# the-professor510/RSMCRT

Hardware: AMD Instinct MI355X
Metric: photon packets/sec (128^3 jmean grid, path-length deposition) (higher is better)
Workload: dtype f64

## Files before the change

### include/smcrt.h

```cpp
#ifndef SMCRT_H
#define SMCRT_H

#include <stddef.h>
#include <stdint.h>

#ifdef __cplusplus
extern "C" {
#endif

#define SMCRT_ABI_VERSION 5

typedef enum smcrt_status {
  SMCRT_OK = 0,
  SMCRT_ERR_INVALID_ARG = -1,
  SMCRT_ERR_HIP = -2,
  SMCRT_ERR_RCCL = -3,
  SMCRT_ERR_DEVICE_FAULT = -4,
  SMCRT_ERR_NO_DEVICE = -5,
  SMCRT_ERR_OOM = -6,
  SMCRT_ERR_UNSUPPORTED = -7
} smcrt_status;

typedef enum smcrt_sdf_kind {
  SMCRT_SDF_SPHERE = 1,
// ... 124 lines not shown

enum {
  SMCRT_FLAG_PATHLENGTH = 1u << 0,
  SMCRT_FLAG_SURVIVAL_BIAS = 1u << 1,
  SMCRT_FLAG_RENDER_SOURCE = 1u << 2,
  SMCRT_FLAG_TEST_KERNEL = 1u << 3,
  SMCRT_FLAG_END_EARLY = 1u << 4,
  SMCRT_FLAG_RECORD_PHOTONS = 1u << 5,
  SMCRT_FLAG_ASYNC_FOLD = 1u << 6,
  SMCRT_FLAG_OVERLAP = 1u << 7
};

typedef struct smcrt_run_config {
  uint64_t n_photons;
  uint64_t first_photon;
  uint64_t seed;
  uint32_t flags;
  int32_t reserved;
} smcrt_run_config;

enum {
  SMCRT_CTR_PHOTONS = 0,
  SMCRT_CTR_EMIT_RETRIES,
  SMCRT_CTR_SCATTERS,
  SMCRT_CTR_ABSORBED,
  SMCRT_CTR_SDF_EVALS,
  SMCRT_CTR_DEPOSITS,
  SMCRT_CTR_GRID_UPDATES,
  SMCRT_CTR_TAUINT,
  SMCRT_CTR_FRESNEL,
  SMCRT_CTR_REFLECTIONS,
  SMCRT_CTR_BOUNCE_ABORTS,
  SMCRT_CTR_FAULTS,
  SMCRT_CTR_RNG_DRAWS,
  SMCRT_CTR_DETECTOR_HITS,
  SMCRT_CTR_ESCAPED,
  SMCRT_CTR_WAVE_ITERS,
  SMCRT_NCOUNTERS = 16
};

typedef struct smcrt_photon_record {
  double pos[3];
  double dir[3];
  double weight;
  int32_t cell[3];
  int32_t layer;
  uint32_t nscatt;
  uint32_t bounces;
  uint32_t draws;
  uint32_t status;
} smcrt_photon_record;

typedef struct smcrt_tallies {
  float* jmean;
  float* absorb;
  float* emission;
  double* jmean_f64;
  double* absorb_f64;
  double* emission_f64;
  double* det_bins;
  double* nscatt;
  double* moments;
  uint64_t* counters;
  smcrt_photon_record* records;
} smcrt_tallies;

typedef struct smcrt_scene smcrt_scene;

int smcrt_abi_version(void);
int smcrt_device_count(int32_t* count);
const char* smcrt_last_error(void);

int smcrt_scene_create(const smcrt_sdf_node* nodes, int32_t n_nodes,
                       const int32_t* top, int32_t n_top,
                       const smcrt_grid* grid,
                       const smcrt_detector* dets, int32_t n_dets,
                       int32_t device, smcrt_scene** out);
void smcrt_scene_destroy(smcrt_scene* scene);

int smcrt_scene_info(const smcrt_scene* scene, smcrt_grid* grid, int32_t* n_top, int32_t* n_dets);

int smcrt_scene_det_bins(const smcrt_scene* scene, int64_t* n_doubles);

int smcrt_scene_set_optprops(smcrt_scene* scene, int32_t top_index,
                             double mus, double mua, double hgg, double n);

typedef struct smcrt_spectral {
  int64_t n_mus, n_mua, n_hgg, n_n, n_flux;
  const double* mus;
  const double* mua;
  const double* hgg;
  const double* n;
  const double* flux;
} smcrt_spectral;

typedef enum smcrt_spectral_mode {
  SMCRT_SPECTRAL_INIT = 0,
  SMCRT_SPECTRAL_UPDATE = 1,
  SMCRT_SPECTRAL_INIT_AS_WRITTEN = 2
} smcrt_spectral_mode;

typedef struct smcrt_optprops {
  double mus, mua, hgg, g2, n, kappa, albedo;
  double wavelength;
  int32_t node_flags;
  int32_t reserved;
} smcrt_optprops;

int smcrt_spectral_sample(const smcrt_spectral* sp, int32_t mode, uint64_t seed, uint64_t* draw,
                          smcrt_optprops* out);

int smcrt_scene_set_spectral(smcrt_scene* scene, int32_t top_index, const smcrt_spectral* sp, int32_t mode,
                             uint64_t seed, uint64_t* draw, smcrt_optprops* out);

int smcrt_run(smcrt_scene* scene, const smcrt_source* src, const smcrt_run_config* cfg,
              smcrt_tallies* io);

typedef struct smcrt_device_tallies {
  double* jmean;
  double* absorb;
  double* emission;
  double* det_bins;
  double* nscatt;
  double* moments;
  uint64_t* counters;
  smcrt_photon_record* records;
} smcrt_device_tallies;

int smcrt_run_device(smcrt_scene* scene, const smcrt_source* src, const smcrt_run_config* cfg,
                     smcrt_device_tallies* dev, void* stream);

int smcrt_run_origins(smcrt_scene* scene, const smcrt_source* src, const double* origins, int64_t n_origins,
                      const smcrt_run_config* cfg, double* det_totals, smcrt_tallies* io);

int smcrt_scene_classify(smcrt_scene* scene, const double* points, int64_t n, int32_t* layer, double* kappa);

int smcrt_scene_fence(smcrt_scene* scene, void* stream);

int smcrt_scene_check(smcrt_scene* scene);

typedef struct smcrt_kernel_times {
  double transport_ms;
  double deposit_ms;
  int64_t launches;
  int64_t lean_launches;
  int64_t far_steps;
  double fold_cu_ms;
  int64_t lean_hazards;
} smcrt_kernel_times;

int smcrt_scene_set_timing(smcrt_scene* scene, int32_t enable);
int smcrt_scene_kernel_times(smcrt_scene* scene, smcrt_kernel_times* out);

int smcrt_normalise_fluence(float* grid, const smcrt_grid* g, uint64_t nphotons);

typedef enum smcrt_symmetry {
  SMCRT_SYM_NONE = 0,
  SMCRT_SYM_PRISM = 1,
  SMCRT_SYM_FLIPPED = 2,
  SMCRT_SYM_UNIFORM_SLAB = 3,
  SMCRT_SYM_NONE_ROTATIONAL = 4,
  SMCRT_SYM_ROTATIONAL_360 = 5
} smcrt_symmetry;

typedef struct smcrt_escape_config {
  int32_t symmetry;
  int32_t n[3];
  double max[3];
  double pos[3];
  double dir[3];
  double rotation;
} smcrt_escape_config;

int smcrt_escape_sym_dims(const smcrt_escape_config* cfg, int32_t dims[3]);

int smcrt_escape_cells(const smcrt_escape_config* cfg, int64_t* n_cells, int32_t* cells, double* positions);

int smcrt_escape_map(const smcrt_escape_config* cfg, const smcrt_grid* grid, int32_t n_dets, const float* escape_sym,
                     float* escape);

int smcrt_escape_run(smcrt_scene* scene, const smcrt_source* src, const smcrt_escape_config* cfg,
                     const smcrt_run_config* run, float* escape_sym, float* escape, smcrt_tallies* io);

enum {
  SMCRT_INVERSE_FIND_MUS = 1u << 0,
  SMCRT_INVERSE_FIND_MUA = 1u << 1,
  SMCRT_INVERSE_FIND_G = 1u << 2,
  SMCRT_INVERSE_FIND_N = 1u << 3,
  SMCRT_INVERSE_APPLY_TRIAL = 1u << 4
};

typedef struct smcrt_inverse_config {
  int32_t layer;
  int32_t flags;
  int32_t max_steps;
  int32_t reserved;
  double max_step_size, grad_step_size, accuracy;
  uint64_t seed;
} smcrt_inverse_config;

int smcrt_scene_get_optprops(const smcrt_scene* scene, int32_t top_index, int32_t* layer, double* mus, double* mua,
                             double* hgg, double* n);

int smcrt_inverse_run(smcrt_scene* scene, const smcrt_source* src, const smcrt_inverse_config* cfg,
                      const smcrt_run_config* run, const double* targets, double* steps, smcrt_tallies* io);

enum {
  SMCRT_PACK_JMEAN = 1u << 0,
  SMCRT_PACK_ABSORB = 1u << 1,
  SMCRT_PACK_EMISSION = 1u << 2,
  SMCRT_PACK_DET_BINS = 1u << 3
};
typedef struct smcrt_pack_layout {
  int64_t n_voxels;
  int64_t n_det_bins;
  uint32_t fields;
  int32_t reserved;
} smcrt_pack_layout;

int smcrt_pack_size(const smcrt_pack_layout* layout, int64_t* n_doubles);
int smcrt_pack_host(const smcrt_pack_layout* layout, const smcrt_tallies* t, double* buf);
int smcrt_unpack_host(const smcrt_pack_layout* layout, const double* buf, smcrt_tallies* t);

#define SMCRT_UNIQUE_ID_BYTES 128
typedef struct smcrt_comm smcrt_comm;
int smcrt_comm_unique_id(uint8_t* id );
int smcrt_comm_init_rank(const uint8_t* id, int32_t n_ranks, int32_t rank, int32_t device, smcrt_comm** out);
void smcrt_comm_destroy(smcrt_comm* comm);
int smcrt_comm_info(const smcrt_comm* comm, int32_t* n_ranks, int32_t* rank, int32_t* device);
int smcrt_reduce_device_tallies(smcrt_scene* scene, smcrt_comm* comm, smcrt_device_tallies* dev, int32_t root,
                                void* stream);

typedef struct smcrt_multi smcrt_multi;
int smcrt_multi_create(const smcrt_sdf_node* nodes, int32_t n_nodes, const int32_t* top, int32_t n_top,
                       const smcrt_grid* grid, const smcrt_detector* dets, int32_t n_dets,
                       const int32_t* devices, int32_t n_devices, smcrt_multi** out);
int smcrt_multi_info(const smcrt_multi* multi, int32_t* n_devices);
smcrt_scene* smcrt_multi_scene(smcrt_multi* multi, int32_t i);
int smcrt_multi_run(smcrt_multi* multi, const smcrt_source* src, const smcrt_run_config* cfg, smcrt_tallies* io);
int smcrt_multi_accumulate(smcrt_multi* multi, const smcrt_source* src, const smcrt_run_config* cfg);
int smcrt_multi_collect(smcrt_multi* multi, smcrt_tallies* io);
int smcrt_multi_device_photons(const smcrt_multi* multi, uint64_t* photons);
void smcrt_multi_destroy(smcrt_multi* multi);


int smcrt_write_data_f32(const char* filename, const float* array, int32_t nx, int32_t ny, int32_t nz,
                         const char* metadata, const char* dect_id, int32_t overwrite,
                         char* written_path, int32_t path_cap);
int smcrt_write_data_f64(const char* filename, const double* array, int32_t nx, int32_t ny, int32_t nz,
                         const char* metadata, const char* dect_id, int32_t overwrite,
                         char* written_path, int32_t path_cap);

int smcrt_write_detector(const char* filename, const smcrt_detector* d, const double* data,
                         const char* id, int64_t nphotons);

int smcrt_write_checkpoint(const char* filename, const char* toml_filename, int64_t photons_run,
                           const float* jmean, const smcrt_grid* g, int32_t overwrite,
                           char* written_path, int32_t path_cap);

typedef struct smcrt_job smcrt_job;

typedef struct smcrt_job_desc {
  int64_t n_photons;
  int64_t seed;
  int32_t flags;
  int32_t n_nodes, n_top, n_dets;
  int32_t overwrite;
  smcrt_grid grid;
  smcrt_source source;
  char experiment[64];
  char source_name[32];
} smcrt_job_desc;

int smcrt_job_load(const char* toml_path, smcrt_job** out);
enum { SMCRT_JOB_DEFAULT = 0, SMCRT_JOB_ESCAPE = 1, SMCRT_JOB_INVERSE = 2 };
int smcrt_job_load_mode(const char* toml_path, int32_t mode, smcrt_job** out);
void smcrt_job_destroy(smcrt_job* job);
int smcrt_job_info(const smcrt_job* job, smcrt_job_desc* desc);
int smcrt_job_scene(const smcrt_job* job, smcrt_sdf_node* nodes, int32_t* top, smcrt_detector* dets);
int smcrt_job_metadata(const smcrt_job* job, char* buf, int32_t cap);
#define SMCRT_ALL_DEVICES (-1)
int smcrt_job_run(smcrt_job* job, int32_t device, const char* outdir, double* nscatt);
int smcrt_job_run_devices(smcrt_job* job, const int32_t* devices, int32_t n_devices, const char* outdir,
                          double* nscatt);

int smcrt_job_escape_config(const smcrt_job* job, smcrt_escape_config* out);
int smcrt_job_inverse_config(const smcrt_job* job, smcrt_inverse_config* out);
int smcrt_job_targets(const smcrt_job* job, double* targets);
int smcrt_job_run_escape(smcrt_job* job, int32_t device, const char* outdir);
int smcrt_job_run_inverse(smcrt_job* job, int32_t device, int32_t apply_trial, double* steps);

#ifdef __cplusplus
}
#endif
#endif
```

### rsmcrt_amd/abi.py

```python
import ctypes as C

SMCRT_ABI_VERSION = 5

OK = 0
ERR_INVALID_ARG = -1
ERR_HIP = -2
ERR_RCCL = -3
ERR_DEVICE_FAULT = -4
ERR_NO_DEVICE = -5
ERR_OOM = -6
ERR_UNSUPPORTED = -7

STATUS_NAMES = {
    OK: "OK", ERR_INVALID_ARG: "INVALID_ARG", ERR_HIP: "HIP_ERROR", ERR_RCCL: "RCCL_ERROR",
    ERR_DEVICE_FAULT: "DEVICE_FAULT", ERR_NO_DEVICE: "NO_DEVICE", ERR_OOM: "OUT_OF_MEMORY",
    ERR_UNSUPPORTED: "UNSUPPORTED",
}

SDF_SPHERE, SDF_BOX, SDF_TORUS, SDF_CYLINDER, SDF_TRIPRISM = 1, 2, 3, 4, 5
SDF_SEGMENT, SDF_CAPSULE, SDF_CONE, SDF_EGG, SDF_PLANE, SDF_MODEL = 6, 7, 8, 9, 10, 11
SDF_REVOLUTION, SDF_EXTRUDE, SDF_ONION, SDF_TWIST, SDF_BEND, SDF_ELONGATE, SDF_DISPLACEMENT = 12, 13, 14, 15, 16, 17, 18
DISP_SINE = 1

OP_UNION, OP_SMOOTH_UNION, OP_SUBTRACTION, OP_INTERSECTION = 0, 1, 2, 3
# ... 37 lines not shown
        ("first_child", C.c_int32), ("n_children", C.c_int32), ("flags", C.c_int32), ("reserved", C.c_int32 * 2),
        ("transform", C.c_double * 16), ("param", C.c_double * 12), ("k", C.c_double),
        ("mus", C.c_double), ("mua", C.c_double), ("hgg", C.c_double), ("n", C.c_double),
    ]


NODE_ALBEDO_UNGUARDED = 1

SPECTRAL_INIT = 0
SPECTRAL_UPDATE = 1
SPECTRAL_INIT_AS_WRITTEN = 2


class Spectral(C.Structure):
    _fields_ = [("n_mus", C.c_int64), ("n_mua", C.c_int64), ("n_hgg", C.c_int64), ("n_n", C.c_int64),
                ("n_flux", C.c_int64), ("mus", C.POINTER(C.c_double)), ("mua", C.POINTER(C.c_double)),
                ("hgg", C.POINTER(C.c_double)), ("n", C.POINTER(C.c_double)), ("flux", C.POINTER(C.c_double))]


class OptProps(C.Structure):
    _fields_ = [("mus", C.c_double), ("mua", C.c_double), ("hgg", C.c_double), ("g2", C.c_double),
                ("n", C.c_double), ("kappa", C.c_double), ("albedo", C.c_double), ("wavelength", C.c_double),
                ("node_flags", C.c_int32), ("reserved", C.c_int32)]


class Grid(C.Structure):
    _fields_ = [("nx", C.c_int32), ("ny", C.c_int32), ("nz", C.c_int32), ("reserved", C.c_int32),
                ("xmax", C.c_double), ("ymax", C.c_double), ("zmax", C.c_double)]


class Spectrum(C.Structure):
    _fields_ = [("kind", C.c_int32), ("reserved", C.c_int32), ("wavelength", C.c_double),
                ("n", C.c_int64), ("array", C.POINTER(C.c_double)),
                ("width", C.c_int32), ("height", C.c_int32), ("image", C.POINTER(C.c_double)),
                ("cell_width", C.c_double), ("cell_height", C.c_double)]


class Source(C.Structure):
    _fields_ = [("kind", C.c_int32), ("reserved", C.c_int32),
                ("pos", C.c_double * 3), ("dir", C.c_double * 3),
                ("p1", C.c_double * 3), ("p2", C.c_double * 3), ("p3", C.c_double * 3),
                ("beam", C.c_int32), ("reserved2", C.c_int32),
                ("radius", C.c_double), ("beam_size", C.c_double), ("focal_length", C.c_double),
                ("rlo", C.c_double), ("rhi", C.c_double), ("sigma", C.c_double),
                ("rotation", C.c_double * 3), ("spectrum", C.POINTER(Spectrum))]


class Detector(C.Structure):
    _fields_ = [
        ("kind", C.c_int32), ("nbins", C.c_int32), ("layer", C.c_int32), ("reserved", C.c_int32),
        ("pos", C.c_double * 3), ("dir", C.c_double * 3), ("e1", C.c_double * 3), ("e2", C.c_double * 3),
        ("radius", C.c_double), ("r1", C.c_double), ("r2", C.c_double),
        ("width", C.c_double), ("height", C.c_double),
        ("bin_wid", C.c_double), ("bin_wid_y", C.c_double), ("fibre", C.c_double * 11),
    ]


class RunConfig(C.Structure):
    _fields_ = [("n_photons", C.c_uint64), ("first_photon", C.c_uint64), ("seed", C.c_uint64),
                ("flags", C.c_uint32), ("reserved", C.c_int32)]


class PhotonRecord(C.Structure):
    _fields_ = [("pos", C.c_double * 3), ("dir", C.c_double * 3), ("weight", C.c_double),
                ("cell", C.c_int32 * 3), ("layer", C.c_int32), ("nscatt", C.c_uint32),
                ("bounces", C.c_uint32), ("draws", C.c_uint32), ("status", C.c_uint32)]


class Tallies(C.Structure):
    _fields_ = [
        ("jmean", C.POINTER(C.c_float)), ("absorb", C.POINTER(C.c_float)),
        ("emission", C.POINTER(C.c_float)),
        ("jmean_f64", C.POINTER(C.c_double)), ("absorb_f64", C.POINTER(C.c_double)),
        ("emission_f64", C.POINTER(C.c_double)),
        ("det_bins", C.POINTER(C.c_double)), ("nscatt", C.POINTER(C.c_double)),
        ("moments", C.POINTER(C.c_double)), ("counters", C.POINTER(C.c_uint64)),
        ("records", C.POINTER(PhotonRecord)),
    ]


class DeviceTallies(C.Structure):
    _fields_ = [
        ("jmean", C.c_void_p), ("absorb", C.c_void_p), ("emission", C.c_void_p),
        ("det_bins", C.c_void_p), ("nscatt", C.c_void_p), ("moments", C.c_void_p),
        ("counters", C.c_void_p), ("records", C.c_void_p),
    ]


def record_dtype():
    import numpy as np
    return np.dtype([("pos", "<f8", 3), ("dir", "<f8", 3), ("weight", "<f8"), ("cell", "<i4", 3),
                     ("layer", "<i4"), ("nscatt", "<u4"), ("bounces", "<u4"), ("draws", "<u4"),
                     ("status", "<u4")])


SYM_NONE, SYM_PRISM, SYM_FLIPPED, SYM_UNIFORM_SLAB, SYM_NONE_ROTATIONAL, SYM_ROTATIONAL_360 = 0, 1, 2, 3, 4, 5
SYMMETRY_KINDS = {"none": SYM_NONE, "prism": SYM_PRISM, "flipped": SYM_FLIPPED, "uniformSlab": SYM_UNIFORM_SLAB,
                  "noneRotational": SYM_NONE_ROTATIONAL, "360rotational": SYM_ROTATIONAL_360}


class EscapeConfig(C.Structure):
    _fields_ = [("symmetry", C.c_int32), ("n", C.c_int32 * 3), ("max", C.c_double * 3), ("pos", C.c_double * 3),
                ("dir", C.c_double * 3), ("rotation", C.c_double)]


INVERSE_FIND_MUS, INVERSE_FIND_MUA, INVERSE_FIND_G, INVERSE_FIND_N, INVERSE_APPLY_TRIAL = 1, 2, 4, 8, 16


class InverseConfig(C.Structure):
    _fields_ = [("layer", C.c_int32), ("flags", C.c_int32), ("max_steps", C.c_int32), ("reserved", C.c_int32),
                ("max_step_size", C.c_double), ("grad_step_size", C.c_double), ("accuracy", C.c_double),
                ("seed", C.c_uint64)]


JOB_DEFAULT, JOB_ESCAPE, JOB_INVERSE = 0, 1, 2


class JobDesc(C.Structure):
    _fields_ = [("n_photons", C.c_int64), ("seed", C.c_int64), ("flags", C.c_int32), ("n_nodes", C.c_int32),
                ("n_top", C.c_int32), ("n_dets", C.c_int32), ("overwrite", C.c_int32), ("grid", Grid),
                ("source", Source), ("experiment", C.c_char * 64), ("source_name", C.c_char * 32)]


PACK_JMEAN, PACK_ABSORB, PACK_EMISSION, PACK_DET_BINS = 1, 2, 4, 8
UNIQUE_ID_BYTES = 128
ALL_DEVICES = -1


class PackLayout(C.Structure):
    _fields_ = [("n_voxels", C.c_int64), ("n_det_bins", C.c_int64), ("fields", C.c_uint32), ("reserved", C.c_int32)]


class KernelTimes(C.Structure):
    _fields_ = [("transport_ms", C.c_double), ("deposit_ms", C.c_double), ("launches", C.c_int64),
                ("lean_launches", C.c_int64), ("far_steps", C.c_int64), ("fold_cu_ms", C.c_double),
                ("lean_hazards", C.c_int64)]


EXPORTED_SYMBOLS = [
    "smcrt_abi_version", "smcrt_device_count", "smcrt_last_error", "smcrt_scene_create",
    "smcrt_scene_destroy", "smcrt_scene_det_bins", "smcrt_scene_set_optprops", "smcrt_run",
    "smcrt_run_device", "smcrt_normalise_fluence", "smcrt_scene_set_timing", "smcrt_scene_kernel_times",
    "smcrt_write_data_f32", "smcrt_write_data_f64", "smcrt_write_detector", "smcrt_write_checkpoint",
    "smcrt_job_load", "smcrt_job_destroy", "smcrt_job_info", "smcrt_job_scene", "smcrt_job_metadata", "smcrt_job_run",
    "smcrt_scene_info", "smcrt_run_origins", "smcrt_scene_classify", "smcrt_escape_sym_dims", "smcrt_escape_cells",
    "smcrt_escape_map", "smcrt_escape_run", "smcrt_scene_get_optprops", "smcrt_inverse_run", "smcrt_job_load_mode",
    "smcrt_job_escape_config", "smcrt_job_inverse_config", "smcrt_job_targets", "smcrt_job_run_escape",
    "smcrt_job_run_inverse", "smcrt_scene_fence",
    "smcrt_pack_size", "smcrt_pack_host", "smcrt_unpack_host", "smcrt_comm_unique_id", "smcrt_comm_init_rank",
    "smcrt_comm_info", "smcrt_comm_destroy", "smcrt_reduce_device_tallies", "smcrt_multi_create", "smcrt_multi_info",
    "smcrt_multi_scene", "smcrt_multi_run", "smcrt_multi_accumulate", "smcrt_multi_collect",
    "smcrt_multi_device_photons", "smcrt_multi_destroy", "smcrt_job_run_devices",
    "smcrt_spectral_sample", "smcrt_scene_set_spectral", "smcrt_scene_check",
]
```

### rsmcrt_amd/csrc/kernel_ptrs.h

```cpp
#pragma once
#include <stddef.h>

namespace smcrt {

size_t kinst_ws_shared_bytes(int slots);
int kinst_ws_threads();
int kinst_ws_photon_lanes();
size_t kinst_ws_scratch_bytes(size_t lanes);

#define SMCRT_KINST_DECL(F, G)                                                               \
  const void* kinst_transport_##F##_##G(int xsrc, int coop);                                 \
  const void* kinst_ws_##F##_##G(int xf, int slots);                                         \
  const void* kinst_wsp_##F##_##G(int slots);                                                \
  void kinst_diag_##F##_##G(unsigned long long* d72, unsigned long long* t9, unsigned long long* c6); \
  void kinst_diagp_##F##_##G(unsigned long long* d72, unsigned long long* t9, unsigned long long* c6);
SMCRT_KINST_DECL(0, 0)
SMCRT_KINST_DECL(0, 1)
SMCRT_KINST_DECL(0, 2)
SMCRT_KINST_DECL(1, 0)
SMCRT_KINST_DECL(1, 1)
SMCRT_KINST_DECL(1, 2)
#undef SMCRT_KINST_DECL

inline const void* transport_kernel_ptr(bool lds_faces, int gm, bool xsrc, bool coop) {
  if (xsrc && coop) lds_faces = false;
  const int x = xsrc ? 1 : 0, c = coop ? 1 : 0;
  switch ((lds_faces ? 3 : 0) + gm) {
    case 0: return kinst_transport_0_0(x, c);
    case 1: return kinst_transport_0_1(x, c);
    case 2: return kinst_transport_0_2(x, c);
    case 3: return kinst_transport_1_0(x, c);
    case 4: return kinst_transport_1_1(x, c);
    default: return kinst_transport_1_2(x, c);
  }
}
inline const void* ws_kernel_ptr(bool lds_faces, int gm, bool xf, int slots) {
  const int x = xf ? 1 : 0;
  switch ((lds_faces ? 3 : 0) + gm) {
    case 0: return kinst_ws_0_0(x, slots);
    case 1: return kinst_ws_0_1(x, slots);
    case 2: return kinst_ws_0_2(x, slots);
    case 3: return kinst_ws_1_0(x, slots);
    case 4: return kinst_ws_1_1(x, slots);
    default: return kinst_ws_1_2(x, slots);
  }
}
inline void kinst_diag_gather(unsigned long long* d72, unsigned long long* t9, unsigned long long* c6) {
  for (int i = 0; i < 72; ++i) d72[i] = 0;
  for (int i = 0; i < 9; ++i) t9[i] = 0;
  for (int i = 0; i < 6; ++i) c6[i] = 0;
  kinst_diag_0_0(d72, t9, c6); kinst_diag_0_1(d72, t9, c6); kinst_diag_0_2(d72, t9, c6);
  kinst_diag_1_0(d72, t9, c6); kinst_diag_1_1(d72, t9, c6); kinst_diag_1_2(d72, t9, c6);
  kinst_diagp_0_0(d72, t9, c6); kinst_diagp_0_1(d72, t9, c6); kinst_diagp_0_2(d72, t9, c6);
  kinst_diagp_1_0(d72, t9, c6); kinst_diagp_1_1(d72, t9, c6); kinst_diagp_1_2(d72, t9, c6);
}

}
```

### rsmcrt_amd/csrc/kinst.hip

```cpp
#include "kernels.h"
#include "kernel_ptrs.h"

#if !defined(KI_F) || !defined(KI_G) || !defined(KI_P)
#error "kinst.hip is compiled with -DKI_F=<0|1> -DKI_G=<0|1|2> -DKI_P=<0|1> (rsmcrt_amd/build.py)"
#endif
#define KI_NAME3(a, f, g) a##_##f##_##g
#define KI_NAME2(a, f, g) KI_NAME3(a, f, g)
#define KI_NAME(a) KI_NAME2(a, KI_F, KI_G)

namespace smcrt {

#if KI_P == 1
const void* KI_NAME(kinst_wsp)(int slots) {
  return slots == 3 ? (const void*)ws_kernel<KI_F != 0, KI_G, false, 3> : (const void*)ws_kernel<KI_F != 0, KI_G, false, 2>;
}
#define KI_DIAG_NAME KI_NAME(kinst_diagp)
#else
const void* KI_NAME(kinst_transport)(int xsrc, int coop) {
  constexpr bool F = KI_F != 0;
  if (xsrc && coop) {
    if constexpr (!F) return (const void*)transport_kernel<false, KI_G, true, true>;
    return nullptr;
  }
  if (xsrc) return (const void*)transport_kernel<F, KI_G, true, false>;
  if (coop) return (const void*)transport_kernel<F, KI_G, false, true>;
  return (const void*)transport_kernel<F, KI_G, false, false>;
}

#if KI_F == 0 && KI_G == 0
size_t kinst_ws_shared_bytes(int slots) { return slots == 3 ? sizeof(WsSharedT<3>) : sizeof(WsSharedT<2>); }
int kinst_ws_threads() { return WS_THREADS; }
int kinst_ws_photon_lanes() { return (int)WS_NPL; }
size_t kinst_ws_scratch_bytes(size_t lanes) { return ws_scratch_bytes(lanes); }
#endif

const void* KI_NAME(kinst_ws)(int xf, int slots) {
  if (xf) return slots == 3 ? (const void*)ws_kernel<KI_F != 0, KI_G, true, 3> : (const void*)ws_kernel<KI_F != 0, KI_G, true, 2>;
  return KI_NAME(kinst_wsp)(slots);
}
#define KI_DIAG_NAME KI_NAME(kinst_diag)
#endif


void KI_DIAG_NAME(unsigned long long* d72, unsigned long long* t9, unsigned long long* c6) {
#ifdef SMCRT_DIAG
  unsigned long long h[72] = {0}, z[72] = {0};
  if (hipDeviceSynchronize() != hipSuccess) return;
  if (hipMemcpyFromSymbol(h, HIP_SYMBOL(g_diag), sizeof(h)) == hipSuccess)
    for (int i = 0; i < 72; ++i) d72[i] += (i >= 68 && i <= 69) ? 0 : h[i];
  for (int i = 68; i <= 69; ++i) d72[i] = h[i] > d72[i] ? h[i] : d72[i];
  (void)hipMemcpyToSymbol(HIP_SYMBOL(g_diag), z, sizeof(z));
  if (hipMemcpyFromSymbol(h, HIP_SYMBOL(g_diag_t), sizeof(unsigned long long) * 9) == hipSuccess)
    for (int i = 0; i < 9; ++i) t9[i] += h[i];
  (void)hipMemcpyToSymbol(HIP_SYMBOL(g_diag_t), z, sizeof(unsigned long long) * 9);
  if (hipMemcpyFromSymbol(h, HIP_SYMBOL(g_cull_diag), sizeof(unsigned long long) * 6) == hipSuccess)
    for (int i = 0; i < 6; ++i) c6[i] += h[i];
  (void)hipMemcpyToSymbol(HIP_SYMBOL(g_cull_diag), z, sizeof(unsigned long long) * 6);
#else
  (void)d72; (void)t9; (void)c6;
#endif
}

}
```

### rsmcrt_amd/csrc/sceneplan.cpp

```cpp
#include "sceneplan.h"

#include <algorithm>
#include <cmath>
#include <cstdlib>
#include <cstring>
#include <functional>
#include <string>

#include "hosterr.h"

namespace smcrt {
namespace {

int fail(int code, const std::string& msg) { return set_error(code, msg); }
bool is(const char* v, const char* s) { return v && std::strcmp(v, s) == 0; }

}

Knobs read_knobs() {
  Knobs k;
  auto num = [](const char* v, double d) { return v ? std::atof(v) : d; };
  if (const char* cm = std::getenv("SMCRT_COOP_MIN_TOPS")) k.coop_min_tops = std::max(1, std::atoi(cm));
  if (const char* cl = std::getenv("SMCRT_COOP_LANES")) k.coop_lanes = std::max(1, std::min(64, std::atoi(cl)));
  k.coop_tab = !is(std::getenv("SMCRT_COOP_TAB"), "0");
  k.cull = !is(std::getenv("SMCRT_CULL"), "0");
  k.cull_grid.cells_per_top = num(std::getenv("SMCRT_CULL_CPT"), 512.0);
  k.cull_grid.max_cells = num(std::getenv("SMCRT_CULL_MAX_CELLS"), 1 << 18);
  k.cull_grid.max_list = (int32_t)num(std::getenv("SMCRT_CULL_MAX_LIST"), 64);
  k.cull_grid.k_nearest = (int32_t)num(std::getenv("SMCRT_CULL_K"), 8);
  k.cull_grid.u_frac = num(std::getenv("SMCRT_CULL_UFRAC"), 1.0);
  k.cull_log = std::getenv("SMCRT_CULL_LOG") != nullptr;
  k.far_march = !is(std::getenv("SMCRT_FAR_MARCH"), "0");
  const char* dm = std::getenv("SMCRT_DEPOSIT");
  k.deposit_atomic = is(dm, "atomic");
  k.deposit_sorted = is(dm, "sorted");
  if (const char* pc = std::getenv("SMCRT_POOL_CAP"))
    k.pool_cap_chunks = std::max<uint64_t>(1, std::strtoull(pc, nullptr, 10) / CHUNK_RECORDS);
  const char* fp = std::getenv("SMCRT_FOLD_PRIO");
  k.fold_prio = !(fp && fp[0] == '0');
  k.fused_hist = !is(std::getenv("SMCRT_FUSED_HIST"), "0");
  const char* wsl = std::getenv("SMCRT_WS_SLOTS");
  k.ws_two_slots = wsl && wsl[0] == '2';
  const char* le = std::getenv("SMCRT_LEAN");
  k.lean_mode = le ? (is(le, "0") ? 0 : 1) : -1;
  const char* lm = std::getenv("SMCRT_DEBUG_LEAN_MARGIN");
  k.lean_debug = is(lm, "all") ? 2u : (is(lm, "0") ? 1u : 0u);
  k.verbose = std::getenv("SMCRT_VERBOSE") != nullptr;
  return k;
}

LaunchKnobs read_launch_knobs() {
  LaunchKnobs k;
#ifdef SMCRT_DIAG
  const char* dd = std::getenv("SMCRT_DIAG_DONE");
  k.diag_done = dd && dd[0] == '1';
#endif
  if (const char* wm = std::getenv("SMCRT_WATCHDOG_MS")) k.watchdog_ms = std::strtod(wm, nullptr);
  if (const char* cd = std::getenv("SMCRT_DEBUG_CLAIM_DELAY")) k.claim_delay = (uint32_t)std::strtoul(cd, nullptr, 10);
  const char* de = std::getenv("SMCRT_DEBUG_DROP_EVENT");
  k.drop_event = de && de[0] == '1';
  return k;
}

PoolKnobs read_pool_knobs() {
  PoolKnobs k;
  if (const char* ns = std::getenv("SMCRT_SLOTS")) k.slots = std::max(2, std::min(MAX_SLOTS, std::atoi(ns)));
  if (const char* dg = std::getenv("SMCRT_DEEP_SLOT_GIB")) {
    k.deep_set = true;
    k.deep_bytes = (uint64_t)std::strtoull(dg, nullptr, 10) << 30;
  }
  return k;
}

bool pool_log_knob() {
  static const bool on = std::getenv("SMCRT_POOL_LOG") != nullptr;
  return on;
}

TopProps make_props(const smcrt_sdf_node& nd) {
  TopProps p;
  p.kappa = nd.mus + nd.mua;
  if (nd.flags & SMCRT_NODE_ALBEDO_UNGUARDED) p.albedo = nd.mus / p.kappa;
  else p.albedo = (nd.mua < 1e-9) ? 1.0 : nd.mus / p.kappa;
  p.hgg = nd.hgg;
  p.n = nd.n;
  return p;
}

namespace {

int validate(const smcrt_sdf_node* nodes, int32_t n_nodes, const int32_t* top, int32_t n_top, const smcrt_grid* grid,
             const smcrt_detector* dets, int32_t n_dets) {
  if (!nodes || n_nodes < 1 || !top || n_top < 1 || !grid || n_dets < 0 || (n_dets > 0 && !dets))
    return fail(SMCRT_ERR_INVALID_ARG, "bad scene arguments");
  if (grid->nx < 1 || grid->ny < 1 || grid->nz < 1 || !(grid->xmax > 0) || !(grid->ymax > 0) ||
      !(grid->zmax > 0))
    return fail(SMCRT_ERR_INVALID_ARG, "grid dimensions must be positive");
  if ((uint64_t)grid->nx * (uint64_t)grid->ny * (uint64_t)grid->nz >= (1ull << 32))
    return fail(SMCRT_ERR_UNSUPPORTED, "grids of 2^32 or more voxels are not supported");
  for (int32_t i = 0; i < n_nodes; ++i) {
    const smcrt_sdf_node& nd = nodes[i];
    if (nd.kind < SMCRT_SDF_SPHERE || nd.kind > SMCRT_SDF_DISPLACEMENT)
      return fail(SMCRT_ERR_INVALID_ARG, "node " + std::to_string(i) + ": unknown SDF kind");
    if (nd.kind == SMCRT_SDF_MODEL) {
      if (nd.n_children < 1 || nd.first_child < 0 || nd.first_child + nd.n_children > n_nodes)
        return fail(SMCRT_ERR_INVALID_ARG, "model node " + std::to_string(i) + ": bad child range");
      if (nd.op < SMCRT_OP_UNION || nd.op > SMCRT_OP_INTERSECTION)
        return fail(SMCRT_ERR_INVALID_ARG, "model node " + std::to_string(i) + ": bad CSG op");
    } else if (composite_kind(nd.kind)) {
      if (nd.n_children != 1 || nd.first_child < 0 || nd.first_child >= n_nodes)
        return fail(SMCRT_ERR_INVALID_ARG, "modifier node " + std::to_string(i) + ": needs exactly one child");
      if (nd.kind == SMCRT_SDF_DISPLACEMENT && nd.param[0] != (double)SMCRT_DISP_SINE)
        return fail(SMCRT_ERR_INVALID_ARG, "displacement node " + std::to_string(i) + ": unknown function");
    }
  }
  std::function<int(int32_t, int)> depth_ok = [&](int32_t idx, int lvl) -> int {
    const smcrt_sdf_node& nd = nodes[idx];
    if (!composite_kind(nd.kind)) return 1;
    if (lvl >= PROG_MAX_DEPTH) return 0;
    for (int32_t c = 0; c < nd.n_children; ++c)
      if (!depth_ok(nd.first_child + c, lvl + 1)) return 0;
    return 1;
  };
  for (int32_t i = 0; i < n_top; ++i)
    if (top[i] >= 0 && top[i] < n_nodes && !depth_ok(top[i], 0))
      return fail(SMCRT_ERR_UNSUPPORTED, "top " + std::to_string(i) + ": models/modifiers nested more than " +
                                             std::to_string(PROG_MAX_DEPTH) + " levels deep are not supported");
  for (int32_t i = 0; i < n_top; ++i)
    if (top[i] < 0 || top[i] >= n_nodes) return fail(SMCRT_ERR_INVALID_ARG, "top index out of range");
  for (int32_t i = 0; i < n_dets; ++i) {
    if (dets[i].kind < SMCRT_DET_CIRCLE || dets[i].kind > SMCRT_DET_FIBRE || dets[i].nbins < 1)
      return fail(SMCRT_ERR_INVALID_ARG, "bad detector " + std::to_string(i));
  }
  return SMCRT_OK;
}

bool translate_only(const smcrt_sdf_node& nd) {
  const double* t = nd.transform;
  return t[0] == 1.0 && t[1] == 0.0 && t[2] == 0.0 && t[4] == 0.0 && t[5] == 1.0 && t[6] == 0.0 &&
         t[8] == 0.0 && t[9] == 0.0 && t[10] == 1.0;
}

void flatten(const smcrt_sdf_node* nodes, const int32_t* top, int32_t n_top, ScenePlan& p) {
  std::vector<ProgOp>& prog = p.prog;
  p.top_first.assign((size_t)n_top + 1, 0);
  for (int32_t i = 0; i < n_top; ++i) {
    const smcrt_sdf_node& nd = nodes[top[i]];
    p.top_first[i] = (int32_t)prog.size();
    if (!composite_kind(nd.kind)) {
      prog.push_back(ProgOp{top[i], PROG_TOP, i + 1, 0, 0.0, translate_only(nd), 0});
    } else if (nd.kind != SMCRT_SDF_MODEL) {
      prog.push_back(ProgOp{top[i], PROG_TOP | PROG_SUB, i + 1, 0, 0.0, 0, 0});
    } else {
      for (int32_t c = 0; c < nd.n_children; ++c) {
        const int32_t ci = nd.first_child + c;
        const bool sub = composite_kind(nodes[ci].kind);
        prog.push_back(ProgOp{ci, (c == 0 ? PROG_CHILD_FIRST : PROG_CHILD) | (sub ? PROG_SUB : 0),
                              c == nd.n_children - 1 ? i + 1 : 0, nd.op, nd.k, sub ? 0 : translate_only(nodes[ci]), 0});
      }
    }
  }
  p.n_prog = (int)prog.size();
  p.top_first[n_top] = p.n_prog;
  for (int32_t i = 0; i <= n_top; ++i)
    prog.push_back(ProgOp{p.top_first[i], PROG_TOP, 0, 0, 0.0, 0, 0});
  for (const ProgOp& op : prog) p.nested = p.nested || (op.action & PROG_SUB) != 0;
}

void plan_far_march(const smcrt_sdf_node* nodes, const int32_t* top, int32_t n_top, const smcrt_grid* grid, bool fm,
                    ScenePlan& p) {
  double ext = grid->xmax + grid->ymax + grid->zmax + 1.0;
  double scale = 0.0;
  std::function<bool(int32_t, int, double&)> far_ok = [&](int32_t idx, int lvl, double& m) -> bool {
    const smcrt_sdf_node& nd = nodes[idx];
    if (nd.kind == SMCRT_SDF_MODEL) {
      const bool op_ok = nd.op == SMCRT_OP_UNION || nd.op == SMCRT_OP_INTERSECTION || nd.op == SMCRT_OP_SUBTRACTION ||
                         (nd.op == SMCRT_OP_SMOOTH_UNION && nd.k > 0.0 && std::isfinite(nd.k));
      if (lvl >= 4 || !op_ok || nd.n_children < 1) return false;
      if (nd.op == SMCRT_OP_SMOOTH_UNION) m = std::max(m, nd.k);
      for (int32_t c = 0; c < nd.n_children; ++c)
        if (!far_ok(nd.first_child + c, lvl + 1, m)) return false;
      return true;
    }
    const int32_t kd = nd.kind;
    if (!translate_only(nd) || !(kd == SMCRT_SDF_SPHERE || kd == SMCRT_SDF_BOX || kd == SMCRT_SDF_TORUS ||
                                 kd == SMCRT_SDF_SEGMENT || kd == SMCRT_SDF_CAPSULE))
      return false;
    double mm = std::fabs(nd.transform[3]) + std::fabs(nd.transform[7]) + std::fabs(nd.transform[11]);
    for (int r = 0; r < 8; ++r) mm += std::fabs(nd.param[r]);
    if (!std::isfinite(mm)) return false;
    m = std::max(m, mm);
    return true;
  };
  for (int32_t i = 0; fm && i < n_top; ++i) {
    double m = 0.0;
    fm = far_ok(top[i], 0, m);
    scale = std::max(scale, m);
  }
  fm = fm && std::isfinite(ext);
  if (fm) {
    p.fm_err = std::ldexp(scale + ext, -44);
    p.fm_step = std::ldexp(scale + ext, -48);
  }
}

}

int plan_scene(const smcrt_sdf_node* nodes, int32_t n_nodes, const int32_t* top, int32_t n_top, const smcrt_grid* grid,
               const smcrt_detector* dets, int32_t n_dets, const Knobs& knobs, const PlanLimits& lim, ScenePlan* out) {
  if (const int st = validate(nodes, n_nodes, top, n_top, grid, dets, n_dets)) return st;
  ScenePlan& p = *out;
  p.n_nodes = n_nodes;
  p.n_top = n_top;
  p.n_dets = n_dets;
  p.grid = *grid;
  p.h_nodes.assign(nodes, nodes + n_nodes);
  p.h_top.assign(top, top + n_top);
  for (int32_t i = 0; i < n_top; ++i) p.h_props.push_back(make_props(nodes[top[i]]));
  p.h_dets.assign(dets, dets + n_dets);
  p.h_det_off.assign((size_t)n_dets + 1, 0);
  for (int32_t i = 0; i < n_dets; ++i) {
    const int64_t nb = dets[i].nbins;
    p.h_det_off[i + 1] = p.h_det_off[i] + (dets[i].kind == SMCRT_DET_CAMERA ? nb * nb : nb);
  }
  p.det_total = p.h_det_off[n_dets];
  for (int32_t i = 0; i < grid->nx + 1; ++i) p.faces.push_back((double)i * 2.0 * grid->xmax / (double)grid->nx);
  for (int32_t i = 0; i < grid->ny + 1; ++i) p.faces.push_back((double)i * 2.0 * grid->ymax / (double)grid->ny);
  for (int32_t i = 0; i < grid->nz + 2; ++i) p.faces.push_back((double)i * 2.0 * grid->zmax / (double)grid->nz);
  flatten(nodes, top, n_top, p);
  p.coop_lanes = n_top >= knobs.coop_min_tops ? std::max(1, std::min(16, n_top / ((n_top + 63) / 64 + 3))) : 0;
  if (knobs.coop_lanes && p.coop_lanes > 0) p.coop_lanes = knobs.coop_lanes;
  {
    bool ok = p.coop_lanes > 0 && n_top <= 64 && knobs.coop_tab;
    for (int32_t i = 0; ok && i < n_top; ++i) ok = !composite_kind(nodes[top[i]].kind);
    if (ok) {
      p.ctab.assign(CTAB_DOUBLES, 0.0);
      for (int32_t i = 0; i < n_top; ++i) {
        const smcrt_sdf_node& nd = nodes[top[i]];
        for (int r = 0; r < 12; ++r) p.ctab[r * 64 + i] = nd.transform[r];
        for (int r = 0; r < 8; ++r) p.ctab[(12 + r) * 64 + i] = nd.param[r];
        p.ctab[20 * 64 + i] = (double)nd.kind + (translate_only(nd) ? 16.0 : 0.0);
      }
    }
  }
  const double maxes[3] = {grid->xmax, grid->ymax, grid->zmax};
  if (p.coop_lanes > 0 && knobs.cull) p.cull = build_cull(nodes, n_nodes, top, n_top, maxes, knobs.cull_grid);
  if (!p.ctab.empty() || p.cull.enabled) plan_far_march(nodes, top, n_top, grid, knobs.far_march, p);
  for (int a = 0; a < 3; ++a) {
    int ex = 0;
    const double m = std::frexp(2.0 * maxes[a], &ex);
    p.inv2[a] = (m == 0.5 && std::isfinite(1.0 / (2.0 * maxes[a]))) ? 1.0 / (2.0 * maxes[a]) : 0.0;
  }
  {
    const bool p2 = p.inv2[0] != 0.0 && p.inv2[1] != 0.0 && p.inv2[2] != 0.0;
    const int32_t ns[3] = {grid->nx, grid->ny, grid->nz};
    bool f2 = p2;
    for (int a = 0; a < 3; ++a) {
      if ((ns[a] & (ns[a] - 1)) != 0) { f2 = false; continue; }
      int e2m = 0, en = 0;
      (void)std::frexp(2.0 * maxes[a], &e2m);
      (void)std::frexp((double)ns[a], &en);
      p.fe[a] = e2m - en;
    }
    p.grid_mode = f2 ? 2 : (p2 ? 1 : 0);
  }
  {
    const uint64_t nv = (uint64_t)grid->nx * grid->ny * grid->nz;
    const uint64_t tiles = (nv + TILE_VOXELS - 1) / TILE_VOXELS;
    p.n_tiles = (tiles <= MAX_TILES && nv < 0xFFFFFFFFull) ? (uint32_t)tiles : 0;
    p.force_atomic = knobs.deposit_atomic;
    p.pool_cap_chunks = knobs.pool_cap_chunks;
    const bool sorted = knobs.deposit_sorted || !knobs.fused_hist;
    p.bucketed = !sorted && p.n_tiles > 0 && p.n_tiles <= MAX_DIRECT_TILES;
    p.hist_tiles = (!p.bucketed && knobs.fused_hist && p.n_tiles > 0 && p.n_tiles <= MAX_FUSED_HIST_TILES) ? p.n_tiles : 0;
  }
  p.face_bytes = p.faces.size() * sizeof(double) + sizeof(TopProps) * (size_t)n_top;
  p.lds_faces = p.face_bytes <= MAX_FACE_BYTES;
  for (int32_t i = 1; i < n_top; ++i) p.fresnel = p.fresnel || p.h_props[i].n != p.h_props[0].n;
  {
    bool ok = p.bucketed && p.coop_lanes == 0 && grid->nx < (1 << 20) - 2 && grid->ny < (1 << 20) - 2 &&
              grid->nz < (1 << 20) - 2;
    p.ws_slots = (!knobs.ws_two_slots && lean_lds(p) + lim.ws_shared3 <= LDS_BYTES) ? 3 : 2;
    ok = ok && lean_lds(p) + (p.ws_slots == 3 ? lim.ws_shared3 : lim.ws_shared2) <= LDS_BYTES;
    p.lean_mode = knobs.lean_mode;
    p.lean_candidate = ok && !p.nested && (p.lean_mode == 1 || (p.lean_mode != 0 && n_dets == 0));
    p.lean_debug = knobs.lean_debug;
  }
  p.fold_prio = knobs.fold_prio;
  p.cull_log = knobs.cull_log;
  p.verbose = knobs.verbose;
  return SMCRT_OK;
}

}
```

### rsmcrt_amd/csrc/sceneplan.h

```cpp
#pragma once
#include <stdint.h>

#include <algorithm>
#include <vector>

#include "../../include/smcrt.h"
#include "transport.h"
#include "cull.h"
#include "deposit.h"

namespace smcrt {

constexpr int MAX_SLOTS = 4;
#ifndef SMCRT_DEEP_SLOT_GIB
#define SMCRT_DEEP_SLOT_GIB 24
#endif
constexpr uint64_t DEEP_SLOT_BYTES = (uint64_t)SMCRT_DEEP_SLOT_GIB << 30;

enum QueueWord : int {
  Q_STREAM0 = 0,
  Q_CALLER = MAX_SLOTS,
  Q_FAR_STEPS,
  Q_FOLD_TICKS,
  Q_LEAN_HAZARDS,
  Q_WATCHDOG,
  Q_COUNT
};
constexpr int N_QUEUES = Q_CALLER + 1;

constexpr size_t LDS_BYTES = 163840;
constexpr size_t MAX_FACE_BYTES = 40960;
constexpr uint32_t MAX_FUSED_HIST_TILES = 512;
constexpr uint64_t MAX_POOL_RECORDS = (1ull << 32) - (1ull << 28);
constexpr double POOL_SLACK = 1.15;
constexpr double DEFAULT_WATCHDOG_MS = 2000.0;

struct Knobs {
  int32_t coop_min_tops = 8;
  int32_t coop_lanes = 0;
  bool coop_tab = true;
  bool cull = true;
  CullKnobs cull_grid;
  bool cull_log = false;
  bool far_march = true;
  bool deposit_atomic = false, deposit_sorted = false;
  uint64_t pool_cap_chunks = 0;
  bool fold_prio = true;
  bool fused_hist = true;
  bool ws_two_slots = false;
  int lean_mode = -1;
  uint32_t lean_debug = 0;
  bool verbose = false;
};
struct LaunchKnobs {
  double watchdog_ms = DEFAULT_WATCHDOG_MS;
  uint32_t claim_delay = 0;
  bool drop_event = false;
  bool diag_done = false;
};
struct PoolKnobs {
  int slots = 0;
  bool deep_set = false;
  uint64_t deep_bytes = 0;
};
Knobs read_knobs();
LaunchKnobs read_launch_knobs();
PoolKnobs read_pool_knobs();
bool pool_log_knob();

struct PlanLimits {
  size_t ws_shared2 = 0, ws_shared3 = 0;
};

struct ScenePlan {
  int n_nodes = 0, n_top = 0, n_dets = 0;
  smcrt_grid grid{};
  int64_t det_total = 0;
  std::vector<smcrt_sdf_node> h_nodes;
  std::vector<int32_t> h_top;
  std::vector<TopProps> h_props;
  std::vector<smcrt_detector> h_dets;
  std::vector<int64_t> h_det_off;
  std::vector<double> faces;
  std::vector<ProgOp> prog;
  std::vector<int32_t> top_first;
  int n_prog = 0;
  bool nested = false;
  int coop_lanes = 0;
  std::vector<double> ctab;
  CullHost cull;
  double fm_err = 0.0, fm_step = 0.0;
  double inv2[3] = {0.0, 0.0, 0.0};
  int grid_mode = 0;
  int32_t fe[3] = {0, 0, 0};
  uint32_t n_tiles = 0;
  bool force_atomic = false;
  uint64_t pool_cap_chunks = 0;
  bool bucketed = false;
  uint32_t hist_tiles = 0;
  size_t face_bytes = 0;
  bool lds_faces = false;
  bool fresnel = false;
  int ws_slots = 3;
  int lean_mode = -1;
  uint32_t lean_debug = 0;
  bool lean_candidate = false;
  bool fold_prio = true, cull_log = false, verbose = false;
};

int plan_scene(const smcrt_sdf_node* nodes, int32_t n_nodes, const int32_t* top, int32_t n_top, const smcrt_grid* grid,
               const smcrt_detector* dets, int32_t n_dets, const Knobs& knobs, const PlanLimits& lim, ScenePlan* out);

TopProps make_props(const smcrt_sdf_node& nd);

inline size_t lean_lds(const ScenePlan& p) {
  return (p.lds_faces ? p.face_bytes : 0) + (size_t)2 * p.n_tiles * sizeof(uint32_t);
}
inline uint32_t dep_words(const ScenePlan& p) { return p.bucketed ? 2 * p.n_tiles : 4 * p.hist_tiles; }
inline size_t transport_lds(const ScenePlan& p, uint32_t dep_words, bool xsrc) {
  const bool ctab = !p.ctab.empty() && p.coop_lanes > 0;
  const bool faces = p.lds_faces && !(xsrc && p.coop_lanes > 0);
  return (faces ? p.face_bytes : 0) + (p.n_dets ? 3 * 256 * sizeof(double) : 0) +
         (size_t)dep_words * sizeof(uint32_t) + (ctab ? CTAB_DOUBLES * sizeof(double) : 0);
}
inline double pool_slack_records(const ScenePlan& p, int blocks) {
  const double waves = (double)blocks * 4.0;
  return p.bucketed ? (waves / 4.0 * 2.0 * p.n_tiles + waves * BUCKET_BATCH) * BUCKET_RECORDS
                    : waves * CHUNK_RECORDS;
}
inline uint64_t pool_records_for(const ScenePlan& p, int blocks, uint64_t n, double rpp) {
  const double want = (double)n * rpp * POOL_SLACK + pool_slack_records(p, blocks);
  return (uint64_t)std::min(want, (double)MAX_POOL_RECORDS);
}
inline int slot_depth(const PoolKnobs& k, bool lean_or_far, uint64_t cap_bytes, uint64_t total_mem) {
  const int want = k.slots ? k.slots : (lean_or_far ? 2 : MAX_SLOTS);
  uint64_t deep = std::max<uint64_t>(DEEP_SLOT_BYTES, (uint64_t)(0.6 * (double)total_mem) / MAX_SLOTS);
  if (k.deep_set) deep = k.deep_bytes;
  return cap_bytes <= deep ? want : 2;
}
inline bool launch_binned(const ScenePlan& p, bool has_jmean, uint32_t flags) {
  return has_jmean && (flags & SMCRT_FLAG_PATHLENGTH) && !(flags & SMCRT_FLAG_SURVIVAL_BIAS) && p.n_tiles > 0 &&
         !p.force_atomic;
}
inline bool launch_lean(bool lean_ok, bool xsrc, uint32_t bucket_tiles, uint32_t flags) {
  return !xsrc && lean_ok && bucket_tiles && (flags & SMCRT_FLAG_PATHLENGTH) && !(flags & SMCRT_FLAG_SURVIVAL_BIAS);
}
inline void lean_margins(uint32_t lean_debug, const smcrt_grid& g, double lo[3], double hi[3]) {
  const double eps = 1e-8, mf = (lean_debug & 3u) ? 0.0 : 2.0 * eps;
  const double mx = mf * (double)(g.nx + 2), my = mf * (double)(g.ny + 2), mz = mf * (double)(g.nz + 2);
  lo[0] = mx; lo[1] = my; lo[2] = mz;
  hi[0] = 2.0 * g.xmax - mx; hi[1] = 2.0 * g.ymax - my; hi[2] = 2.0 * g.zmax - mz;
}

}
```

### rsmcrt_amd/csrc/smcrt.hip

```cpp
#include <hip/hip_runtime.h>

#include <algorithm>
#include <cmath>
#include <cstdio>
#include <cstring>
#include <memory>
#include <mutex>
#include <string>
#include <vector>

#define SMCRT_FOLD_KERNELS
#include "../../include/smcrt.h"
#include "scene_internal.h"
#include "transport.h"
#include "deposit.h"
#include "devmem.h"
#include "hosterr.h"
#include "sceneplan.h"

using namespace smcrt;

#include "kernel_ptrs.h"


// ... 125 lines not shown
    float a = 0.f, b = 0.f;
    if ((err = hipEventElapsedTime(&a, e[0], e[1])) != hipSuccess) return err;
    if ((err = hipEventElapsedTime(&b, e[2], e[3])) != hipSuccess) return err;
    s->t_transport += a; s->t_deposit += b; s->t_launches += 1;
  }
  s->tev_used = 0;
  return hipSuccess;
}

static const void* transport_fn(const smcrt_scene* s, bool xsrc) {
  return transport_kernel_ptr(s->lds_faces, s->grid_mode, xsrc, s->coop_lanes > 0);
}

static uint32_t* watchdog_word(smcrt_scene* s) { return (uint32_t*)(s->d_queue + Q_WATCHDOG); }
static const char* watchdog_site(uint32_t site) {
  switch (site) {
    case WDOG_PHOTON_WAVE: return "ws_kernel photon wave (every live lane waited for an event, a segment or a slot)";
    case WDOG_RING: return "ws_kernel ring producer (the token word's previous lap was never consumed)";
    case WDOG_EVENT_QUEUE: return "ws_kernel event-queue producer (the entry's previous lap was never consumed)";
    case WDOG_BUCKET: return "bucket wait (deposit.h: the pending claim never rebased the tile word)";
    default: return "unknown site";
  }
}
static int take_watchdog(smcrt_scene* s) {
  uint32_t w = 0;
  HIPCHK(hipMemcpy(&w, watchdog_word(s), sizeof w, hipMemcpyDeviceToHost));
  if (!w) return SMCRT_OK;
  HIPCHK(hipMemset(watchdog_word(s), 0, sizeof w));
  return fail(SMCRT_ERR_DEVICE_FAULT, std::string("watchdog: a wait exceeded SMCRT_WATCHDOG_MS at ") +
                                          watchdog_site(w & 0xFFu) + " in block " + std::to_string((w >> 8) - 1u) +
                                          "; the run's tallies are incomplete");
}

extern "C" {

int smcrt_abi_version(void) { return SMCRT_ABI_VERSION; }

const char* smcrt_last_error(void) { return g_last_error.c_str(); }

int smcrt_device_count(int32_t* count) {
  if (!count) return fail(SMCRT_ERR_INVALID_ARG, "count is NULL");
  int n = 0;
  hipError_t e = hipGetDeviceCount(&n);
  if (e == hipErrorNoDevice) n = 0;
  else if (e != hipSuccess) return fail(SMCRT_ERR_HIP, hipGetErrorString(e));
  *count = n;
  return SMCRT_OK;
}

void smcrt_scene_destroy(smcrt_scene* s) {
  if (!s) return;
  (void)hipSetDevice(s->device);
  if (s->stream) (void)hipStreamSynchronize(s->stream);
  if (s->fstream) (void)hipStreamSynchronize(s->fstream);
  for (int i = 0; i < MAX_SLOTS; ++i)
    if (s->lstream[i]) (void)hipStreamSynchronize(s->lstream[i]);
  delete s;
}

static int upload_plan(smcrt_scene* s) {
  int st;
  if ((st = upload(s->d_nodes, s->h_nodes.data(), s->h_nodes.size(), "scene upload")) ||
      (st = upload(s->d_prog, s->prog.data(), s->prog.size(), "scene upload")) ||
      (st = upload(s->d_props, s->h_props.data(), s->h_props.size(), "scene upload")) ||
      (st = upload(s->d_faces, s->faces.data(), s->faces.size(), "scene upload")) ||
      (st = upload(s->d_dets, s->h_dets.data(), s->h_dets.size(), "scene upload")) ||
      (st = upload(s->d_det_off, s->h_det_off.data(), s->h_det_off.size(), "scene upload")) ||
      (!s->ctab.empty() && (st = upload(s->d_ctab, s->ctab.data(), s->ctab.size(), "scene upload"))) ||
      (st = dalloc(s->d_queue, Q_COUNT)) || (st = dalloc(s->d_cold, COLD_SLOTS)) ||
      (st = dalloc(s->d_counters, SMCRT_NCOUNTERS)) || (st = dalloc(s->d_small, (size_t)s->det_total + 1 + 24)))
    return st;
  hipError_t e = hipMemset(s->d_queue, 0, Q_COUNT * sizeof(unsigned long long));
  if (e == hipSuccess) e = hipStreamCreateWithFlags(s->stream.out(), hipStreamNonBlocking);
  for (int i = 0; i < MAX_SLOTS && e == hipSuccess; ++i) {
    e = hipStreamCreateWithFlags(s->lstream[i].out(), hipStreamNonBlocking);
    if (e == hipSuccess) e = hipEventCreateWithFlags(s->lev[i].out(), hipEventDisableTiming);
  }
  if (e == hipSuccess) e = hipEventCreateWithFlags(s->ev_in.out(), hipEventDisableTiming);
  if (e != hipSuccess) return fail(SMCRT_ERR_HIP, std::string("scene upload: ") + hipGetErrorString(e));
  return SMCRT_OK;
}

static int upload_cull(smcrt_scene* s) {
  const CullHost& cull = s->cull;
  std::vector<ProgOp> pa;
  for (int32_t t : cull.always)
    for (int32_t ip = s->top_first[t]; ip < s->top_first[t + 1]; ++ip) pa.push_back(s->prog[ip]);
  auto al = [](size_t b) { return (b + 15) & ~(size_t)15; };
  const size_t b_pa = al(pa.size() * sizeof(ProgOp)), b_off = al(cull.off.size() * 4),
               b_list = al(std::max<size_t>(1, cull.list.size()) * 4), b_lb = al(cull.lb.size() * 8),
               b_elb = al(std::max<size_t>(1, cull.elb.size()) * 4);
  std::vector<unsigned char> blob(b_pa + b_off + b_list + b_lb + b_elb, 0);
  std::memcpy(blob.data(), pa.data(), pa.size() * sizeof(ProgOp));
  std::memcpy(blob.data() + b_pa, cull.off.data(), cull.off.size() * 4);
  std::memcpy(blob.data() + b_pa + b_off, cull.list.data(), cull.list.size() * 4);
  std::memcpy(blob.data() + b_pa + b_off + b_list, cull.lb.data(), cull.lb.size() * 8);
  std::memcpy(blob.data() + b_pa + b_off + b_list + b_lb, cull.elb.data(), cull.elb.size() * 4);
  int st;
  if ((st = upload(s->d_cull_data, blob.data(), blob.size(), "cull upload"))) return st;
  const unsigned char* base = s->d_cull_data;
  CullGrid G;
  for (int a = 0; a < 3; ++a) { G.lo[a] = cull.lo[a]; G.n[a] = cull.n[a]; }
  G.cell = cull.cell;
  G.inv_cell = 1.0 / cull.cell;
  G.n_prog_always = (int32_t)pa.size();
  G.prog_always = base;
  G.off = (const uint32_t*)(base + b_pa);
  G.list = (const uint32_t*)(base + b_pa + b_off);
  G.lb = (const double*)(base + b_pa + b_off + b_list);
  G.elb = (const float*)(base + b_pa + b_off + b_list + b_lb);
  if ((st = upload(s->d_cull, &G, 1, "cull upload"))) return st;
  if (s->cull_log)
    std::fprintf(stderr, "[cull] %d tops, %zu always, %d x %d x %d cells of %.4g, %.1f tops per cell\n",
                 s->n_top, cull.always.size(), cull.n[0], cull.n[1], cull.n[2], cull.cell, cull.mean_list);
  s->cull.off = {}; s->cull.list = {}; s->cull.elb = {}; s->cull.lb = {};
  return SMCRT_OK;
}

static int create_fold_state(smcrt_scene* s) {
  int st;
  if ((st = dalloc(s->d_tile_count, s->n_tiles)) || (st = dalloc(s->d_tile_start, s->n_tiles))) return st;
  for (int i = 0; i < MAX_SLOTS; ++i)
    if ((st = dalloc(s->d_dep_ctl[i], 8)) || (st = dalloc(s->d_bin_counts[i], (size_t)s->n_tiles * BIN_BLOCKS))) return st;
  s->scatter_lds = scatter_lds_bytes(s->n_tiles);
  if (hipFuncSetAttribute((const void*)bin_scatter, hipFuncAttributeMaxDynamicSharedMemorySize,
                          (int)s->scatter_lds) != hipSuccess)
    return fail(SMCRT_ERR_HIP, "bin_scatter LDS attribute");
  int prio_least = 0, prio_greatest = 0;
  const bool fold_prio = s->fold_prio &&
                         hipDeviceGetStreamPriorityRange(&prio_least, &prio_greatest) == hipSuccess &&
                         prio_greatest != prio_least;
  bool ok = s->h_ctl.alloc(8 * MAX_SLOTS) == hipSuccess &&
            hipEventCreateWithFlags(s->ev_t.out(), hipEventDisableTiming) == hipSuccess &&
            (fold_prio ? hipStreamCreateWithPriority(s->fstream.out(), hipStreamNonBlocking, prio_greatest)
                       : hipStreamCreateWithFlags(s->fstream.out(), hipStreamNonBlocking)) == hipSuccess;
  for (int i = 0; ok && i < MAX_SLOTS; ++i)
    ok = hipEventCreateWithFlags(s->ctl_ev[i].out(), hipEventDisableTiming) == hipSuccess &&
         hipEventCreateWithFlags(s->ev_f[i].out(), hipEventDisableTiming) == hipSuccess;
  if (!ok) return fail(SMCRT_ERR_HIP, "pinned/event/stream allocation failed");
  std::memset(s->h_ctl, 0, 8 * MAX_SLOTS * sizeof(uint32_t));
  return SMCRT_OK;
}

static void size_grids(smcrt_scene* s) {
  int per_cu = 0, cus = 0;
  if (hipDeviceGetAttribute(&cus, hipDeviceAttributeMultiprocessorCount, s->device) != hipSuccess || cus < 1) cus = 256;
  s->n_cus = cus;
  int khz = 0;
  if (hipDeviceGetAttribute(&khz, hipDeviceAttributeWallClockRate, s->device) == hipSuccess && khz > 0) s->wall_khz = khz;
  s->lean_ok = s->lean_candidate;
  const bool xf = s->fresnel || s->n_dets > 0;
  if (s->lean_ok) {
    hipError_t oe = hipOccupancyMaxActiveBlocksPerMultiprocessor(
        &per_cu, ws_kernel_ptr(s->lds_faces, s->grid_mode, xf, s->ws_slots), kinst_ws_threads(), lean_lds(*s));
    if (oe != hipSuccess || per_cu < 1) per_cu = 1;
    s->grid_blocks_ws = cus * per_cu;
    if (xf) {
      s->lscratch_stride = (kinst_ws_scratch_bytes((size_t)s->grid_blocks_ws * kinst_ws_photon_lanes()) + 255) & ~(size_t)255;
      if (s->d_lscratch.alloc(s->lscratch_stride * N_QUEUES) != hipSuccess) {
        (void)hipGetLastError();
        s->lean_ok = false;
      }
    }
  }
  if (s->verbose)
    std::fprintf(stderr, "[smcrt] scene: lean %d (ws slots %d, blocks/CU %d, static LDS %zu + dynamic %zu B), transport grid %d\n",
                 (int)s->lean_ok, s->ws_slots, s->grid_blocks_ws / std::max(1, cus), kinst_ws_shared_bytes(s->ws_slots), lean_lds(*s),
                 s->grid_blocks);
  for (int x = 0; x < 2; ++x) {
    hipError_t oe = hipOccupancyMaxActiveBlocksPerMultiprocessor(&per_cu, transport_fn(s, x == 1), 256,
                                                                 transport_lds(*s, dep_words(*s), x == 1));
    if (oe != hipSuccess || per_cu < 1) per_cu = 1;
    (x ? s->grid_blocks_x : s->grid_blocks) = cus * per_cu;
  }
}

int smcrt_scene_create(const smcrt_sdf_node* nodes, int32_t n_nodes, const int32_t* top, int32_t n_top,
                       const smcrt_grid* grid, const smcrt_detector* dets, int32_t n_dets, int32_t device,
                       smcrt_scene** out) {
  g_last_error.clear();
  if (!out) return fail(SMCRT_ERR_INVALID_ARG, "out is NULL");
  *out = nullptr;
  const PlanLimits lim{kinst_ws_shared_bytes(2), kinst_ws_shared_bytes(3)};
  ScenePlan plan;
  int st = plan_scene(nodes, n_nodes, top, n_top, grid, dets, n_dets, read_knobs(), lim, &plan);
  if (st) return st;
  int ndev = 0;
  if (hipGetDeviceCount(&ndev) != hipSuccess || ndev == 0) return fail(SMCRT_ERR_NO_DEVICE, "no HIP device");
  if (device < 0 || device >= ndev) return fail(SMCRT_ERR_INVALID_ARG, "device ordinal out of range");
  std::unique_ptr<smcrt_scene, void (*)(smcrt_scene*)> s(new smcrt_scene(), smcrt_scene_destroy);
  static_cast<ScenePlan&>(*s) = std::move(plan);
  s->device = device;
  if (hipSetDevice(device) != hipSuccess) return fail(SMCRT_ERR_HIP, "hipSetDevice failed");
  if ((st = upload_plan(s.get())) || (s->cull.enabled && (st = upload_cull(s.get()))) ||
      (s->n_tiles && (st = create_fold_state(s.get()))))
    return st;
  size_grids(s.get());
  *out = s.release();
  return SMCRT_OK;
}

int smcrt_scene_det_bins(const smcrt_scene* s, int64_t* n) {
  if (!s || !n) return fail(SMCRT_ERR_INVALID_ARG, "NULL argument");
  *n = s->det_total;
  return SMCRT_OK;
}

int smcrt_scene_set_optprops(smcrt_scene* s, int32_t i, double mus, double mua, double hgg, double n) {
  return smcrt::scene_set_node_props(s, i, mus, mua, hgg, n, 0);
}

int smcrt_scene_get_optprops(const smcrt_scene* s, int32_t i, int32_t* layer, double* mus, double* mua, double* hgg,
                             double* n) {
  if (!s || i < 0 || i >= s->n_top) return fail(SMCRT_ERR_INVALID_ARG, "bad scene or index");
  const smcrt_sdf_node& nd = s->h_nodes[s->h_top[i]];
  if (layer) *layer = nd.layer;
  if (mua) *mua = nd.mua;
  if (mus) *mus = s->h_props[i].kappa - nd.mua;
  if (hgg) *hgg = nd.hgg;
  if (n) *n = nd.n;
  return SMCRT_OK;
}

}

int smcrt::scene_node_optprops(const smcrt_scene* s, int32_t i, double out[4]) {
  if (!s || i < 0 || i >= s->n_top) return fail(SMCRT_ERR_INVALID_ARG, "bad scene or index");
  const smcrt_sdf_node& nd = s->h_nodes[s->h_top[i]];
  out[0] = nd.mus; out[1] = nd.mua; out[2] = nd.hgg; out[3] = nd.n;
  return SMCRT_OK;
}

int smcrt::scene_set_node_props(smcrt_scene* s, int32_t i, double mus, double mua, double hgg, double n,
                                int32_t flags) {
  if (!s || i < 0 || i >= s->n_top) return fail(SMCRT_ERR_INVALID_ARG, "bad scene or index");
  std::lock_guard<std::mutex> g(s->mu);
  smcrt_sdf_node& nd = s->h_nodes[s->h_top[i]];
  nd.mus = mus; nd.mua = mua; nd.hgg = hgg; nd.n = n;
  nd.flags = flags;
  s->h_props[i] = make_props(nd);
  HIPCHK(hipSetDevice(s->device));
  HIPCHK(hipMemcpyAsync(s->d_props + i, &s->h_props[i], sizeof(TopProps), hipMemcpyHostToDevice, s->stream));
  HIPCHK(hipStreamSynchronize(s->stream));
  return SMCRT_OK;
}

int smcrt::scene_node_flags(const smcrt_scene* s, int32_t i, int32_t* flags) {
  if (!s || i < 0 || i >= s->n_top) return fail(SMCRT_ERR_INVALID_ARG, "bad scene or index");
  *flags = s->h_nodes[s->h_top[i]].flags;
  return SMCRT_OK;
}

int smcrt::scene_device(const smcrt_scene* s) { return s->device; }
void* smcrt::scene_stream(const smcrt_scene* s) { return (void*)s->stream; }

int smcrt::scene_inflight(smcrt_scene* s) {
  std::lock_guard<std::mutex> g(s->mu);
  int n = 0;
  for (int i = 0; i < MAX_SLOTS; ++i) {
    if (s->lpending[i] && hipEventQuery(s->lev[i]) == hipSuccess) s->lpending[i] = false;
    n += s->lpending[i] ? 1 : 0;
  }
  return n;
}
int smcrt::scene_depth(const smcrt_scene* s) { return s->n_slots; }

int smcrt::scene_det_size(const smcrt_scene* s, int32_t d, int64_t* n) {
  if (!s || d < 0 || d >= s->n_dets) return fail(SMCRT_ERR_INVALID_ARG, "bad scene or detector");
  *n = (d + 1 < s->n_dets ? s->h_det_off[d + 1] : s->det_total) - s->h_det_off[d];
  return SMCRT_OK;
}

extern "C" {

static void refine_rpp(smcrt_scene* s) {
  for (int i = 0; i < s->n_slots; ++i) {
    const int sl = s->last_slot < 0 ? i : (s->last_slot + 1 + i) % s->n_slots;
    if (s->ctl_pending[sl] && hipEventQuery(s->ctl_ev[sl]) == hipSuccess) {
      s->ctl_pending[sl] = false;
      const uint32_t* h = s->h_ctl + 8 * sl;
      if (pool_log_knob())
        std::fprintf(stderr, "[pool] slot %d: %u photons, %u records, %u overflowed, %u of %llu chunks\n", sl, h[4],
                     h[3], h[1], h[0], (unsigned long long)s->pool_chunks);
      if (h[4] > 0) {
        const double rpp = (double)(h[3] + h[1]) / (double)h[4];
        s->rpp_est = std::max(1.0, rpp);
        s->rpp_measured = true;
      }
    }
  }
}

static hipError_t drain_folds(smcrt_scene* s) {
  if (!s->fstream) return hipSuccess;
  const hipError_t e = hipStreamSynchronize(s->fstream);
  for (bool& f : s->f_pending) f = false;
  return e;
}

static int transport_blocks(const smcrt_scene* s) { return std::max(s->grid_blocks, s->grid_blocks_x); }

static bool ensure_pool(smcrt_scene* s, uint64_t records) {
  uint64_t chunks = (records + CHUNK_RECORDS - 1) / CHUNK_RECORDS;
  if (s->pool_cap_chunks) chunks = std::min(chunks, s->pool_cap_chunks);
  if (chunks <= s->pool_chunks) return true;
  chunks = std::min<uint64_t>(chunks + chunks / 4, MAX_POOL_RECORDS / CHUNK_RECORDS);
  if (s->pool_cap_chunks) chunks = std::min(chunks, s->pool_cap_chunks);
  (void)hipDeviceSynchronize();
  (void)drain_folds(s);
  auto release = [&]() {
    s->d_sorted.reset(); s->d_pieces.reset(); s->d_order.reset();
    for (int i = 0; i < MAX_SLOTS; ++i) { s->d_pool[i].reset(); s->d_chunk_fill[i].reset(); s->d_bucket_tile[i].reset(); }
    s->pool_chunks = 0;
  };
  release();
  const uint64_t cap = chunks * CHUNK_RECORDS;
  size_t mfree = 0, mtotal = 0;
  if (hipMemGetInfo(&mfree, &mtotal) != hipSuccess) mtotal = 0;
  s->n_slots = slot_depth(read_pool_knobs(), s->lean_ok || s->fm_err > 0.0, cap * 8, mtotal);
  s->slot = 0;
  s->lturn = 0;
  s->last_slot = -1;
  const uint64_t pieces = std::min<uint64_t>(cap / MIN_PIECE_RECORDS, REDUCE_PIECES + 1) + s->n_tiles + 1;
  const uint64_t buckets = cap / BUCKET_RECORDS;
  bool ok = s->d_pieces.alloc(pieces) == hipSuccess;
  for (int i = 0; ok && i < s->n_slots; ++i) {
    ok = s->d_pool[i].alloc(cap) == hipSuccess;
    if (ok && s->bucketed)
      ok = s->d_chunk_fill[i].alloc(buckets) == hipSuccess && s->d_bucket_tile[i].alloc(buckets) == hipSuccess;
    else if (ok)
      ok = s->d_chunk_fill[i].alloc(chunks) == hipSuccess;
  }
  if (ok && s->bucketed)
    ok = s->d_order.alloc(buckets) == hipSuccess;
  else if (ok)
    ok = s->d_sorted.alloc(cap) == hipSuccess;
  if (!ok) {
    (void)hipGetLastError();
    release();
    return false;
  }
  s->pool_chunks = chunks;
  s->max_pieces = pieces;
  return true;
}


static int next_timing_events(smcrt_scene* s, Event** ev) {
  *ev = nullptr;
  if (!s->timing) return SMCRT_OK;
  if (s->tev_used == MAX_TIMED) HIPCHK(harvest_times(s));
  while (4 * (s->tev_used + 1) > s->tev.size()) {
    Event e;
    HIPCHK(hipEventCreate(e.out()));
    s->tev.push_back(std::move(e));
  }
  *ev = &s->tev[4 * s->tev_used++];
  return SMCRT_OK;
}

static int enqueue_transport(smcrt_scene* s, const KParams& K, KCold Ch, bool xsrc, bool lean, hipStream_t stream,
                             int sl, int qi, Event** ev_out) {
  const bool binned = K.rec_pool != nullptr;
  if (binned && s->f_pending[sl]) HIPCHK(hipStreamWaitEvent(stream, s->ev_f[sl], 0));
  Ch.queue = s->d_queue + qi;
  Ch.lane_scratch = s->d_lscratch ? (double*)(s->d_lscratch + (size_t)qi * s->lscratch_stride) : nullptr;
  HIPCHK(hipMemsetAsync(Ch.queue, 0, sizeof(unsigned long long), stream));
  const KCold* C = s->d_cold + (size_t)qi * COLD_PER_STREAM + (s->cold_seq[qi]++ % COLD_PER_STREAM);
  HIPCHK(hipMemcpyAsync((void*)C, &Ch, sizeof(KCold), hipMemcpyHostToDevice, stream));
  if (binned) {
    HIPCHK(hipMemsetAsync(s->d_dep_ctl[sl], 0, 8 * sizeof(uint32_t), stream));
    if (K.bucket_tiles)
      HIPCHK(hipMemsetAsync(s->d_bin_counts[sl], 0, (size_t)s->n_tiles * sizeof(uint32_t), stream));
    else if (K.hist_tiles)
      HIPCHK(hipMemsetAsync(s->d_bin_counts[sl], 0, (size_t)s->n_tiles * BIN_BLOCKS * sizeof(uint32_t), stream));
  }
  if (const int st = next_timing_events(s, ev_out)) return st;
  Event* ev = *ev_out;
  if (ev) HIPCHK(hipEventRecord(ev[0], stream));
  const uint64_t waves_needed = (Ch.n_photons + 63) / 64;
  const uint64_t blocks_needed = (waves_needed + 3) / 4;
  const uint64_t ws_needed = (Ch.n_photons + kinst_ws_photon_lanes() - 1) / kinst_ws_photon_lanes();
  const int blocks = (int)std::min<uint64_t>(
      (uint64_t)(lean ? s->grid_blocks_ws : (xsrc ? s->grid_blocks_x : s->grid_blocks)),
      std::max<uint64_t>(1, lean ? ws_needed : blocks_needed));
  const smcrt_sdf_node* a_nodes = K.nodes;
  const ProgOp* a_prog = K.prog;
  if (lean) {
    ++s->lean_launches;
    void* args[] = {(void*)&K, (void*)&a_nodes, (void*)&a_prog, (void*)&C};
    HIPCHK(hipLaunchKernel(ws_kernel_ptr(s->lds_faces, s->grid_mode, s->d_lscratch != nullptr, s->ws_slots), dim3(blocks),
                           dim3(kinst_ws_threads()), args, lean_lds(*s), stream));
  } else {
    const smcrt_detector* a_dets = K.dets;
    const int64_t* a_off = K.det_off;
    void* args[] = {(void*)&K, (void*)&a_nodes, (void*)&a_prog, (void*)&a_dets, (void*)&a_off, (void*)&C};
    HIPCHK(hipLaunchKernel(transport_fn(s, xsrc), dim3(blocks), dim3(256), args, transport_lds(*s, dep_words(*s), xsrc), stream));
  }
  HIPCHK(hipGetLastError());
  if (ev) HIPCHK(hipEventRecord(ev[1], stream));
  return SMCRT_OK;
}

static int enqueue_fold(smcrt_scene* s, const KParams& K, double* jmean, hipStream_t stream, int sl, Event* ev) {
  if (!K.rec_pool) {
    if (ev) {
      HIPCHK(hipEventRecord(ev[2], stream));
      HIPCHK(hipEventRecord(ev[3], stream));
    }
    return SMCRT_OK;
  }
  hipStream_t fs = s->fstream;
  HIPCHK(hipEventRecord(s->ev_t, stream));
  HIPCHK(hipStreamWaitEvent(fs, s->ev_t, 0));
  if (ev) HIPCHK(hipEventRecord(ev[2], fs));
  const uint32_t nch = (uint32_t)s->pool_chunks;
  const uint64_t nv = (uint64_t)s->grid.nx * s->grid.ny * s->grid.nz;
  if (K.bucket_tiles) {
    hipLaunchKernelGGL(bk_scan, dim3(1), dim3(1024), 0, fs, s->d_bin_counts[sl], s->n_tiles, s->d_tile_start,
                       s->d_tile_count, s->d_pieces, s->d_dep_ctl[sl]);
    hipLaunchKernelGGL(bk_place, dim3(BIN_BLOCKS), dim3(BIN_THREADS), 0, fs, s->d_bucket_tile[sl], s->d_dep_ctl[sl],
                       K.n_buckets, s->n_tiles, s->d_tile_count, s->d_order);
#ifndef SMCRT_ABL_NO_FOLD
    hipLaunchKernelGGL(bk_reduce, dim3(1024), dim3(RED_THREADS), 0, fs, s->d_pool[sl], s->d_order, s->d_chunk_fill[sl],
                       s->d_pieces, s->d_dep_ctl[sl], nv, jmean, s->d_queue + Q_FOLD_TICKS);
#endif
  } else {
    if (!K.hist_tiles)
      hipLaunchKernelGGL(bin_hist, dim3(BIN_BLOCKS), dim3(BIN_THREADS), 0, fs, s->d_pool[sl], s->d_chunk_fill[sl],
                         s->d_dep_ctl[sl], nch, s->n_tiles, s->d_bin_counts[sl]);
    hipLaunchKernelGGL(bin_rowscan, dim3(s->n_tiles), dim3(BIN_BLOCKS), 0, fs, s->d_bin_counts[sl],
                       s->d_tile_count);
    hipLaunchKernelGGL(bin_scan, dim3(1), dim3(1024), 0, fs, s->d_tile_count, s->n_tiles, s->d_tile_start,
                       s->d_pieces, s->d_dep_ctl[sl]);
    hipLaunchKernelGGL(bin_scatter, dim3(BIN_BLOCKS), dim3(BIN_THREADS), s->scatter_lds, fs, s->d_pool[sl],
                       s->d_chunk_fill[sl], s->d_dep_ctl[sl], nch, s->n_tiles, s->d_tile_start, s->d_bin_counts[sl],
                       s->d_sorted, (uint64_t)s->pool_chunks * CHUNK_RECORDS);
    hipLaunchKernelGGL(bin_reduce, dim3(1024), dim3(1024), 0, fs, s->d_sorted, s->d_pieces, s->d_dep_ctl[sl], nv,
                       jmean);
  }
  HIPCHK(hipGetLastError());
  HIPCHK(hipMemcpyAsync(s->h_ctl + 8 * sl, s->d_dep_ctl[sl], 4 * sizeof(uint32_t), hipMemcpyDeviceToHost, fs));
  HIPCHK(hipMemcpyAsync(s->h_ctl + 8 * sl + 5, s->d_dep_ctl[sl] + 5, 2 * sizeof(uint32_t), hipMemcpyDeviceToHost, fs));
  HIPCHK(hipEventRecord(s->ctl_ev[sl], fs));
  s->ctl_pending[sl] = true;
  if (ev) HIPCHK(hipEventRecord(ev[3], fs));
  HIPCHK(hipEventRecord(s->ev_f[sl], fs));
  s->f_pending[sl] = true;
  s->last_slot = sl;
  return SMCRT_OK;
}

#ifdef SMCRT_DIAG
static int diag_report(hipStream_t stream, bool lean) {
  unsigned long long h[72], ht[9], hc[6];
  HIPCHK(hipStreamSynchronize(stream));
  kinst_diag_gather(h, ht, hc);
  if (lean) {
    const double wi = (double)std::max(1ull, h[20]), pt = (double)std::max(1ull, h[24]);
    std::fprintf(stderr, "[diag-ws] walker iters %llu: idle %.3f, busy lanes/iter %.1f, pending lanes/iter %.1f | "
                 "photon trips %llu: sleep %.3f, idle lanes %.1f, sync-waiting %.2f, slot-blocked %.2f, EVAL lanes "
                 "%.1f, pushes %.2f, P7 runs %.3f (lanes/run %.1f), event-waiting %.2f | producer waits %llu | event "
                 "iters %llu, lanes/iter %.1f\n",
                 h[20], h[21] / wi, h[22] / wi, h[23] / wi, h[24], h[25] / pt, h[30] / pt, h[27] / pt, h[26] / pt,
                 h[31] / pt, h[32] / pt, h[28] / pt, (double)h[29] / (double)std::max(1ull, h[28]), h[36] / pt, h[33],
                 h[34], (double)h[35] / (double)std::max(1ull, h[34]));
    const char* np[8] = {"fetch", "poll", "eval", "p3p4", "handout", "p5p6", "p7", "p8"};
    double tp = 0, tw = 0, te = 0;
    for (int i = 0; i < 8; ++i) tp += (double)h[37 + i];
    for (int i = 0; i < 4; ++i) tw += (double)h[45 + i];
    te = (double)h[49] + (double)h[50];
    std::fprintf(stderr, "[diag-ws-time] photon:");
    for (int i = 0; i < 8; ++i) std::fprintf(stderr, " %s=%.3f", np[i], (double)h[37 + i] / std::max(1.0, tp));
    std::fprintf(stderr, " | walker: claim=%.3f idle=%.3f walk=%.3f finish=%.3f | event: run=%.3f idle=%.3f | "
                 "ticks photon/walker/event %.3g/%.3g/%.3g\n", h[45] / std::max(1.0, tw), h[46] / std::max(1.0, tw),
                 h[47] / std::max(1.0, tw), h[48] / std::max(1.0, tw), h[49] / std::max(1.0, te),
                 h[50] / std::max(1.0, te), tp, tw, te);
  }
  unsigned long long lt = 0;
  for (int i = 0; i < 64; ++i) lt += h[i];
  std::fprintf(stderr, "[diag] waves %llu, longest wave %llu trips %llu ticks\n", h[70], h[68], h[69]);
  std::fprintf(stderr, "[diag] trips %llu dda %llu eval %llu p7 %llu | lane-trips %llu:", h[64], h[65], h[66],
               h[67], lt);
  for (int i = 0; i < 64; ++i)
    if (h[i]) std::fprintf(stderr, " %s%d=%.3f", i >= 32 ? "seg:" : "", i & 31, (double)h[i] / (double)lt);
  std::fprintf(stderr, "\n");

  double tt = 0;
  for (int i = 1; i < 9; ++i) tt += (double)ht[i];
  const char* nm_t[9] = {"", "fetch", "eval", "p3", "p4", "dda", "p5p6", "p7", "p8"};
  const char* nm_l[9] = {"", "fetch", "eval", "p3p4", "push", "walk", "p5p6", "p7", "p8"};
  const char* const* nm = lean ? nm_l : nm_t;
  std::fprintf(stderr, "[diag-time]");
  for (int i = 1; i < 9; ++i) std::fprintf(stderr, " %s=%.3f", nm[i], (double)ht[i] / tt);
  std::fprintf(stderr, "\n");

  if (hc[0] + hc[2])
    std::fprintf(stderr, "[diag-cull] culled lane-EVALs %llu, bound fallbacks %llu (%.4f), capture/outside %llu, "
                 "mean list %.1f, wave-EVALs %llu with a full fallback %.3f\n", hc[0], hc[1],
                 (double)hc[1] / (double)std::max(1ull, hc[0]), hc[2], (double)hc[3] / (double)std::max(1ull, hc[0]),
                 hc[4], (double)hc[5] / (double)std::max(1ull, hc[4]));
  return SMCRT_OK;
}
#endif

static int launch_one(smcrt_scene* s, const KParams& K, const KCold& Ch, bool xsrc, hipStream_t stream, int sl, int qi) {
  const bool lean = launch_lean(s->lean_ok, xsrc, K.bucket_tiles, K.flags);
  Event* ev = nullptr;
  int st = enqueue_transport(s, K, Ch, xsrc, lean, stream, sl, qi, &ev);
  if (!st) st = enqueue_fold(s, K, Ch.jmean, stream, sl, ev);
#ifdef SMCRT_DIAG
  if (!st) st = diag_report(stream, lean);
#endif
  return st;
}

struct OriginRun {
  const double* d_origins;
  double* d_totals;
  uint64_t per_origin, first;
};

static int fill_params(smcrt_scene* s, const smcrt_source* src, const smcrt_run_config* cfg,
                       const smcrt_device_tallies& dt, const SrcPlan& plan, hipStream_t stream, bool diag_done_ok,
                       KParams& K, KCold& Ch) {
  const LaunchKnobs knobs = read_launch_knobs();
  K.nodes = s->d_nodes;
  K.prog = s->d_prog;
  K.n_prog = s->n_prog;
  K.coop_lanes = s->coop_lanes;
  K.cull = s->d_cull;
  K.ctab = s->d_ctab;
  const bool far = s->fm_err > 0.0 && (cfg->flags & SMCRT_FLAG_PATHLENGTH);
  K.fm_err = far ? s->fm_err : 0.0;
  K.fm_step = s->fm_step;
  K.inv2x = s->inv2[0]; K.inv2y = s->inv2[1]; K.inv2z = s->inv2[2];
  K.fex = s->fe[0]; K.fey = s->fe[1]; K.fez = s->fe[2];
  K.props = s->d_props;
  K.xface = s->d_faces;
  K.yface = s->d_faces + (s->grid.nx + 1);
  K.zface = s->d_faces + (s->grid.nx + 1) + (s->grid.ny + 1);
  K.dets = s->d_dets;
  K.det_off = s->d_det_off;
  K.n_top = s->n_top;
  K.n_dets = s->n_dets;
  K.nx = s->grid.nx; K.ny = s->grid.ny; K.nz = s->grid.nz;
  K.xmax = s->grid.xmax; K.ymax = s->grid.ymax; K.zmax = s->grid.zmax;
  K.flags = cfg->flags;
  Ch.src = *src;
  Ch.plan = plan;
  K.key0 = (uint32_t)cfg->seed;
  K.key1 = (uint32_t)(cfg->seed >> 32);
  Ch.jmean = dt.jmean; Ch.absorb = dt.absorb; Ch.emission = dt.emission;
  Ch.chunk_fill = nullptr; Ch.dep_ctl = nullptr; Ch.bin_counts = nullptr;
  Ch.bucket_tile = nullptr; Ch.bucket_fill = nullptr; Ch.tile_nb = nullptr;
  Ch.det_bins = dt.det_bins; Ch.nscatt = dt.nscatt; Ch.moments = dt.moments;
  Ch.counters = (unsigned long long*)dt.counters;
  Ch.queue = nullptr;
  Ch.far_steps = s->d_queue + Q_FAR_STEPS;
  Ch.lean_hazards = s->d_queue + Q_LEAN_HAZARDS;
  Ch.lane_scratch = nullptr;
  Ch.watchdog = watchdog_word(s);
#ifdef SMCRT_DIAG
  Ch.done_time = nullptr;
  Ch.done_base = cfg->first_photon;
  if (knobs.diag_done && diag_done_ok) {
    s->n_done = cfg->n_photons;
    HIPCHK(s->d_done.alloc(s->n_done));
    HIPCHK(hipMemsetAsync(s->d_done, 0, sizeof(unsigned long long) * s->n_done, stream));
    Ch.done_time = s->d_done;
  }
#else
  (void)stream; (void)diag_done_ok;
#endif
  Ch.watchdog_ticks = knobs.watchdog_ms > 0.0 ? (uint64_t)(knobs.watchdog_ms * (double)s->wall_khz) : 0ull;
  K.rec_pool = nullptr; K.n_chunks = 0; K.hist_tiles = 0; K.bucket_tiles = 0; K.n_buckets = 0;
  K.claim_delay = knobs.claim_delay;
  K.lean_debug = s->lean_debug | (knobs.drop_event ? 4u : 0u);
  lean_margins(K.lean_debug, s->grid, K.lean_lo, K.lean_hi);
  return SMCRT_OK;
}

static int launch(smcrt_scene* s, const smcrt_source* src, const smcrt_run_config* cfg,
                  const smcrt_device_tallies& dt, hipStream_t stream, const OriginRun* orun = nullptr) {
  if (src->kind < SMCRT_SRC_POINT || src->kind > SMCRT_SRC_APERTURE) return fail(SMCRT_ERR_INVALID_ARG, "bad source kind");
  if (cfg->n_photons == 0) return SMCRT_OK;
  const bool xsrc = src_needs_plan(src) || orun || s->nested;
  SrcPlan plan;
  std::memset(&plan, 0, sizeof plan);
  if (xsrc) {
    std::vector<double> px, py, pc;
    const char* perr = "";
    const int pst = build_src_plan(src, &s->grid, &plan, px, py, pc, &perr);
    if (pst) return fail(pst, perr);
    std::vector<double> tab;
    tab.reserve(px.size() + py.size() + pc.size());
    tab.insert(tab.end(), px.begin(), px.end());
    tab.insert(tab.end(), py.begin(), py.end());
    tab.insert(tab.end(), pc.begin(), pc.end());
    if (!tab.empty()) {
      if (tab != s->h_spec) {
        HIPCHK(hipStreamSynchronize(stream));
        if (s->stream != stream) HIPCHK(hipStreamSynchronize(s->stream));
        if (tab.size() > s->spec_cap) {
          s->spec_cap = 0;
          HIPCHK(s->d_spec.alloc(tab.size()));
          s->spec_cap = tab.size();
        }
        HIPCHK(hipMemcpy(s->d_spec, tab.data(), tab.size() * sizeof(double), hipMemcpyHostToDevice));
        s->h_spec = tab;
      }
      plan.spec_x = px.empty() ? nullptr : s->d_spec;
      plan.spec_y = py.empty() ? nullptr : s->d_spec + px.size();
      plan.cdf = s->d_spec + px.size() + py.size();
    }
    if (orun) {
      plan.origins = orun->d_origins;
      plan.det_totals = orun->d_totals;
      plan.per_origin = orun->per_origin;
      plan.first = orun->first;
    }
  }
  KParams K;
  KCold Ch;
  if (const int st = fill_params(s, src, cfg, dt, plan, stream, !orun, K, Ch)) return st;
  const bool binned = launch_binned(*s, dt.jmean != nullptr, cfg->flags);
  const bool overlap = (cfg->flags & SMCRT_FLAG_OVERLAP) != 0;
  if (overlap) {
    HIPCHK(hipEventRecord(s->ev_in, stream));
    for (int i = 0; i < MAX_SLOTS; ++i) HIPCHK(hipStreamWaitEvent(s->lstream[i], s->ev_in, 0));
  } else {
    for (int i = 0; i < MAX_SLOTS; ++i)
      if (s->lpending[i]) HIPCHK(hipStreamWaitEvent(stream, s->lev[i], 0));
  }
  for (int i = 0; i < MAX_SLOTS; ++i)
    if (s->lpending[i] && hipEventQuery(s->lev[i]) == hipSuccess) s->lpending[i] = false;
  for (uint64_t done = 0; done < cfg->n_photons;) {
    refine_rpp(s);
    uint64_t n = cfg->n_photons - done;
    K.rec_pool = nullptr; K.n_chunks = 0; K.hist_tiles = 0; K.bucket_tiles = 0; K.n_buckets = 0;
    bool calibrate = false;
    if (binned) {
      if (!s->rpp_measured && n > CALIB_PHOTONS) { n = CALIB_PHOTONS; calibrate = true; }
      const uint64_t want = pool_records_for(*s, transport_blocks(s), n, s->rpp_est);
      if (!ensure_pool(s, want)) (void)ensure_pool(s, want / 4);
      if (s->pool_chunks) {
        const double usable = (double)(s->pool_chunks * CHUNK_RECORDS) - pool_slack_records(*s, transport_blocks(s));
        n = std::min<uint64_t>(n, (uint64_t)std::max(65536.0, usable / (s->rpp_est * POOL_SLACK)));
        K.rec_pool = s->d_pool[s->slot];
        Ch.chunk_fill = s->d_chunk_fill[s->slot];
        Ch.dep_ctl = s->d_dep_ctl[s->slot];
        Ch.bin_counts = s->d_bin_counts[s->slot];
        K.n_chunks = (uint32_t)s->pool_chunks;
        K.hist_tiles = s->hist_tiles;
        if (s->bucketed) {
          Ch.bucket_fill = s->d_chunk_fill[s->slot];
          Ch.bucket_tile = s->d_bucket_tile[s->slot];
          Ch.tile_nb = s->d_bin_counts[s->slot];
          K.bucket_tiles = s->n_tiles;
          K.n_buckets = (uint32_t)(s->pool_chunks * (CHUNK_RECORDS / BUCKET_RECORDS));
        }
      }
    }
    Ch.n_photons = n;
    Ch.first_photon = orun ? done : cfg->first_photon + done;
    Ch.records = dt.records ? dt.records + done : nullptr;
    const int sl = s->slot;
    if (K.rec_pool) {
      if (s->ctl_pending[sl]) { HIPCHK(hipEventSynchronize(s->ctl_ev[sl])); refine_rpp(s); }
      s->h_ctl[8 * sl + 4] = (uint32_t)std::min<uint64_t>(n, 0xFFFFFFFFull);
    }
    int st;
    if (overlap) {
      const int q = s->lturn;
      s->lturn = (s->lturn + 1) % s->n_slots;
      st = launch_one(s, K, Ch, xsrc, s->lstream[q], sl, q);
      if (!st && hipEventRecord(s->lev[q], s->lstream[q]) != hipSuccess) st = fail(SMCRT_ERR_HIP, "event record failed");
      s->lpending[q] = true;
    } else {
      st = launch_one(s, K, Ch, xsrc, stream, sl, Q_CALLER);
    }
    if (st) return st;
    if (K.rec_pool) s->slot = (s->slot + 1) % s->n_slots;
    if (calibrate && K.rec_pool) {
      HIPCHK(hipEventSynchronize(s->ctl_ev[sl]));
      refine_rpp(s);
    }
    done += n;
  }
  if (!(cfg->flags & (SMCRT_FLAG_ASYNC_FOLD | SMCRT_FLAG_OVERLAP)) && s->last_slot >= 0 && s->f_pending[s->last_slot])
    HIPCHK(hipStreamWaitEvent(stream, s->ev_f[s->last_slot], 0));
  return SMCRT_OK;
}

int smcrt_run_device(smcrt_scene* s, const smcrt_source* src, const smcrt_run_config* cfg,
                     smcrt_device_tallies* dev, void* stream) {
  g_last_error.clear();
  if (!s || !src || !cfg || !dev) return fail(SMCRT_ERR_INVALID_ARG, "NULL argument");
  std::lock_guard<std::mutex> g(s->mu);
  HIPCHK(hipSetDevice(s->device));
  return launch(s, src, cfg, *dev, (hipStream_t)stream);
}

}

static int run_sync(smcrt_scene* s, const smcrt_source* src, const smcrt_run_config* cfg_in, smcrt_tallies* io,
                    const OriginRun* orun) {
  smcrt_run_config cfg_local = *cfg_in;
  cfg_local.flags &= ~(uint32_t)(SMCRT_FLAG_ASYNC_FOLD | SMCRT_FLAG_OVERLAP);
  const smcrt_run_config* cfg = &cfg_local;
  const int64_t nv = (int64_t)s->grid.nx * s->grid.ny * s->grid.nz;
  const bool want[3] = {io->jmean || io->jmean_f64, io->absorb || io->absorb_f64, io->emission || io->emission_f64};
  if (!s->d_grids && (want[0] || want[1] || want[2])) {
    int st = dalloc(s->d_grids, (size_t)nv * 3);
    if (st) return st;
  }
  const bool rec = (cfg->flags & SMCRT_FLAG_RECORD_PHOTONS) && io->records;
  if (rec && s->records_cap < cfg->n_photons) {
    s->records_cap = 0;
    int st = dalloc(s->d_records, cfg->n_photons);
    if (st) return st;
    s->records_cap = cfg->n_photons;
  }
  smcrt_device_tallies dt{};
  for (int t = 0; t < 3; ++t) {
    if (!want[t]) continue;
    double* p = s->d_grids + (size_t)t * nv;
    HIPCHK(hipMemsetAsync(p, 0, sizeof(double) * nv, s->stream));
    if (t == 0) dt.jmean = p;
    if (t == 1) dt.absorb = p;
    if (t == 2) dt.emission = p;
// ... 51 lines not shown

int smcrt_run_origins(smcrt_scene* s, const smcrt_source* src, const double* origins, int64_t n_origins,
                      const smcrt_run_config* cfg, double* det_totals, smcrt_tallies* io) {
  g_last_error.clear();
  if (!s || !cfg || !io || (n_origins > 0 && !origins)) return fail(SMCRT_ERR_INVALID_ARG, "NULL argument");
  if (n_origins < 0) return fail(SMCRT_ERR_INVALID_ARG, "n_origins < 0");
  if (cfg->flags & SMCRT_FLAG_RECORD_PHOTONS) return fail(SMCRT_ERR_INVALID_ARG, "photon records are not kept for batched origins");
  if (n_origins > 0xFFFFFFFFll) return fail(SMCRT_ERR_INVALID_ARG, "more than 2^32 origins");
  if (n_origins == 0 || cfg->n_photons == 0) return SMCRT_OK;
  if (cfg->n_photons > UINT64_MAX / (uint64_t)n_origins) return fail(SMCRT_ERR_INVALID_ARG, "photon count overflows");
  std::lock_guard<std::mutex> g(s->mu);
  HIPCHK(hipSetDevice(s->device));
  smcrt_source p;
  if (src) p = *src;
  else std::memset(&p, 0, sizeof p);
  p.kind = SMCRT_SRC_POINT;
  const size_t nt = (size_t)n_origins * (size_t)std::max(s->n_dets, 1);
  DevBuf<double> d_org, d_tot;
  int st = dalloc(d_org, (size_t)n_origins * 3);
  if (!st) st = dalloc(d_tot, nt);
  if (!st) {
    OriginRun orun{d_org, s->n_dets ? d_tot : nullptr, cfg->n_photons, cfg->first_photon};
    smcrt_run_config c = *cfg;
    c.n_photons = cfg->n_photons * (uint64_t)n_origins;
    hipError_t e = hipMemcpy(d_org, origins, sizeof(double) * 3 * (size_t)n_origins, hipMemcpyHostToDevice);
    if (e == hipSuccess) e = hipMemset(d_tot, 0, sizeof(double) * nt);
    if (e != hipSuccess) st = fail(SMCRT_ERR_HIP, std::string("origin upload: ") + hipGetErrorString(e));
    if (!st) st = run_sync(s, &p, &c, io, &orun);
    if (!st && det_totals && s->n_dets) {
      std::vector<double> h(nt);
      e = hipMemcpy(h.data(), d_tot, sizeof(double) * nt, hipMemcpyDeviceToHost);
      if (e != hipSuccess) st = fail(SMCRT_ERR_HIP, std::string("totals: ") + hipGetErrorString(e));
      else for (size_t i = 0; i < nt; ++i) det_totals[i] += h[i];
    }
  }
  return st;
}

#ifdef SMCRT_DIAG
int smcrt_diag_read(unsigned long long* out) {
  HIPCHK(hipDeviceSynchronize());
  unsigned long long hc[6];
  kinst_diag_gather(out, out + 72, hc);
  return SMCRT_OK;
}
int smcrt_diag_done_times(smcrt_scene* s, unsigned long long* out, uint64_t n, int32_t* khz) {
  if (!s || !out || !s->d_done || n > s->n_done) return fail(SMCRT_ERR_INVALID_ARG, "no completion times");
  HIPCHK(hipDeviceSynchronize());
  HIPCHK(hipMemcpy(out, s->d_done, sizeof(unsigned long long) * n, hipMemcpyDeviceToHost));
  if (khz) *khz = s->wall_khz;
  return SMCRT_OK;
}
#endif

int smcrt_scene_info(const smcrt_scene* s, smcrt_grid* grid, int32_t* n_top, int32_t* n_dets) {
  if (!s) return fail(SMCRT_ERR_INVALID_ARG, "scene is NULL");
  if (grid) *grid = s->grid;
  if (n_top) *n_top = s->n_top;
  if (n_dets) *n_dets = s->n_dets;
  return SMCRT_OK;
}

int smcrt_scene_classify(smcrt_scene* s, const double* points, int64_t n, int32_t* layer, double* kappa) {
  g_last_error.clear();
  if (!s || (n > 0 && (!points || !layer))) return fail(SMCRT_ERR_INVALID_ARG, "NULL argument");
  if (n <= 0) return SMCRT_OK;
  std::lock_guard<std::mutex> g(s->mu);
  HIPCHK(hipSetDevice(s->device));
  DevBuf<double> d_pts;
  DevBuf<int32_t> d_lay;
  int st = dalloc(d_pts, (size_t)n * 3);
  if (!st) st = dalloc(d_lay, (size_t)n);
  if (!st) {
    hipError_t e = hipMemcpy(d_pts, points, sizeof(double) * 3 * (size_t)n, hipMemcpyHostToDevice);
    if (e == hipSuccess) {
      const int blocks = (int)std::min<int64_t>((n + 255) / 256, 65535);
      hipLaunchKernelGGL(classify_kernel, dim3(blocks), dim3(256), 0, s->stream, (const smcrt_sdf_node*)s->d_nodes,
                         (const ProgOp*)s->d_prog, (int32_t)s->n_prog, (const double*)d_pts, n, d_lay);
      e = hipGetLastError();
    }
    if (e == hipSuccess) e = hipStreamSynchronize(s->stream);
    if (e == hipSuccess) e = hipMemcpy(layer, d_lay, sizeof(int32_t) * (size_t)n, hipMemcpyDeviceToHost);
    if (e != hipSuccess) st = fail(SMCRT_ERR_HIP, std::string("classify: ") + hipGetErrorString(e));
  }
  if (!st && kappa)
    for (int64_t i = 0; i < n; ++i) kappa[i] = layer[i] > 0 ? s->h_props[layer[i] - 1].kappa : 0.0;
  return st;
}

int smcrt_scene_fence(smcrt_scene* s, void* stream) {
  g_last_error.clear();
  if (!s) return fail(SMCRT_ERR_INVALID_ARG, "scene is NULL");
  std::lock_guard<std::mutex> g(s->mu);
  HIPCHK(hipSetDevice(s->device));
  for (int i = 0; i < MAX_SLOTS; ++i)
    if (s->lpending[i]) HIPCHK(hipStreamWaitEvent((hipStream_t)stream, s->lev[i], 0));
  if (s->last_slot >= 0 && s->f_pending[s->last_slot])
    HIPCHK(hipStreamWaitEvent((hipStream_t)stream, s->ev_f[s->last_slot], 0));
  return SMCRT_OK;
}

int smcrt_scene_check(smcrt_scene* s) {
  g_last_error.clear();
  if (!s) return fail(SMCRT_ERR_INVALID_ARG, "scene is NULL");
  std::lock_guard<std::mutex> g(s->mu);
  HIPCHK(hipSetDevice(s->device));
  for (int i = 0; i < MAX_SLOTS; ++i)
    if (s->lstream[i]) {
      const hipError_t e = hipStreamSynchronize(s->lstream[i]);
      if (e != hipSuccess) return fail(SMCRT_ERR_DEVICE_FAULT, std::string("transport kernel: ") + hipGetErrorString(e));
    }
  for (hipStream_t st : {(hipStream_t)s->stream, (hipStream_t)s->fstream})
    if (st) {
      const hipError_t e = hipStreamSynchronize(st);
      if (e != hipSuccess) return fail(SMCRT_ERR_DEVICE_FAULT, std::string("transport kernel: ") + hipGetErrorString(e));
    }
  return take_watchdog(s);
}

int smcrt_scene_set_timing(smcrt_scene* s, int32_t enable) {
  if (!s) return fail(SMCRT_ERR_INVALID_ARG, "scene is NULL");
  std::lock_guard<std::mutex> g(s->mu);
  s->timing = enable != 0;
  return SMCRT_OK;
}

int smcrt_scene_kernel_times(smcrt_scene* s, smcrt_kernel_times* out) {
  if (!s || !out) return fail(SMCRT_ERR_INVALID_ARG, "NULL argument");
  std::lock_guard<std::mutex> g(s->mu);
  HIPCHK(hipSetDevice(s->device));
  HIPCHK(harvest_times(s));
  out->transport_ms = s->t_transport;
  out->deposit_ms = s->t_deposit;
  out->launches = s->t_launches;
  out->lean_launches = s->lean_launches;
  s->lean_launches = 0;
  unsigned long long far = 0;
  HIPCHK(hipMemcpy(&far, s->d_queue + Q_FAR_STEPS, sizeof(far), hipMemcpyDeviceToHost));
  out->far_steps = (int64_t)(far - s->far_reported);
  s->far_reported = far;
  unsigned long long ticks = 0;
  HIPCHK(hipMemcpy(&ticks, s->d_queue + Q_FOLD_TICKS, sizeof(ticks), hipMemcpyDeviceToHost));
  out->fold_cu_ms = (double)(ticks - s->fold_ticks_reported) / (double)s->wall_khz / (double)s->n_cus;
  s->fold_ticks_reported = ticks;
  unsigned long long hz = 0;
  HIPCHK(hipMemcpy(&hz, s->d_queue + Q_LEAN_HAZARDS, sizeof(hz), hipMemcpyDeviceToHost));
  out->lean_hazards = (int64_t)(hz - s->hazards_reported);
  s->hazards_reported = hz;
  s->t_transport = s->t_deposit = 0.0;
  s->t_launches = 0;
  return SMCRT_OK;
}

int smcrt_normalise_fluence(float* g, const smcrt_grid* grid, uint64_t nphotons) {
  if (!g || !grid || nphotons == 0) return fail(SMCRT_ERR_INVALID_ARG, "bad arguments");
  const double xmax = grid->xmax, ymax = grid->ymax, zmax = grid->zmax;
  const double f = (2.0 * xmax * 2.0 * ymax * 2.0 * zmax) /
                   ((double)nphotons * (2.0 * xmax / grid->nx) * (2.0 * ymax / grid->ny) * (2.0 * zmax / grid->nz));
  const int64_t nv = (int64_t)grid->nx * grid->ny * grid->nz;
  for (int64_t i = 0; i < nv; ++i) g[i] = (float)((double)g[i] * f);
  return SMCRT_OK;
}

}
```

### rsmcrt_amd/csrc/transport.h

```cpp
#pragma once
#include <hip/hip_runtime.h>
#include <stdint.h>

#include "../../include/smcrt.h"
#include "detmath.h"
#include "geometry.h"
#include "srcplan.h"
#include "cull.h"

namespace smcrt {

constexpr int64_t MAX_EMIT_TRIES = 100000;
constexpr int64_t MAX_HOP_ITERS = 1000000;
constexpr int64_t MAX_MARCH_ITERS = 10000000;
constexpr int64_t MAX_GLANCE_ITERS = 100000;
constexpr int64_t MAX_DDA_ITERS = 10000000;
constexpr int MAX_RENORM_ITERS = 64;
constexpr int64_t MAX_INTERACTIONS = 100000000;

#define SMCRT_DDA_PER_ITER 3
#define SMCRT_FETCH_CHUNK 64
#define SMCRT_EVENT_LANES 16

struct TopProps {
  double kappa, albedo, hgg, n;
};

struct KCold {
  smcrt_source src;
  uint64_t n_photons, first_photon;
  double* absorb;
  double* emission;
  double* det_bins;
  double* nscatt;
  double* moments;
  unsigned long long* counters;
  smcrt_photon_record* records;
  unsigned long long* queue;
  double* jmean;
  uint32_t* chunk_fill;
  uint32_t* dep_ctl;
  uint32_t* bin_counts;
  uint32_t* bucket_tile;
  uint32_t* bucket_fill;
  uint32_t* tile_nb;
  unsigned long long* far_steps;
  unsigned long long* lean_hazards;
  double* lane_scratch;
  uint32_t* watchdog;
  uint64_t watchdog_ticks;
#ifdef SMCRT_DIAG
  unsigned long long* done_time;
  uint64_t done_base;
#endif
  SrcPlan plan;
};

enum : uint32_t {
  WDOG_PHOTON_WAVE = 1,
  WDOG_RING = 2,
  WDOG_EVENT_QUEUE = 3,
  WDOG_BUCKET = 4
};
__device__ __forceinline__ bool watchdog_expired(const KCold* __restrict__ C, uint64_t t0, uint32_t site) {
  const uint64_t budget = C->watchdog_ticks;
  if (budget == 0 || __builtin_amdgcn_s_memrealtime() - t0 <= budget) return false;
  atomicCAS(C->watchdog, 0u, site | ((blockIdx.x + 1u) << 8));
  return true;
}

struct KParams {
  const smcrt_sdf_node* __restrict__ nodes;
  const ProgOp* __restrict__ prog;
  const TopProps* __restrict__ props;
  const double* __restrict__ xface;
  const double* __restrict__ yface;
  const double* __restrict__ zface;
  const smcrt_detector* __restrict__ dets;
  const int64_t* __restrict__ det_off;
  int32_t n_prog, n_top, n_dets;
  int32_t coop_lanes;
  int32_t nx, ny, nz;
  uint32_t flags;
  double xmax, ymax, zmax;
  double inv2x, inv2y, inv2z;
  int32_t fex, fey, fez;
  uint32_t key0, key1;
  unsigned long long* rec_pool;
  uint32_t n_chunks;
  uint32_t hist_tiles;
  uint32_t bucket_tiles, n_buckets;
  uint32_t claim_delay;
  uint32_t lean_debug;
  double lean_lo[3], lean_hi[3];
  const CullGrid* __restrict__ cull;
  const double* __restrict__ ctab;
  double fm_err, fm_step;
};

template <int GM>
__device__ __forceinline__ double cell_floor(double p, int32_t n, double max, double inv, int32_t fe) {
  if constexpr (GM == 2) return floor(ldexp(p, -fe));
  const double a = (double)n * p;
  return floor(GM >= 1 ? a * inv : (inv != 0.0 ? a * inv : a / (2.0 * max)));
}
__device__ __forceinline__ int32_t cvt_sat_i32(double f) {
  int32_t r;
  asm("v_cvt_i32_f64 %0, %1" : "=v"(r) : "v"(f));
  return r;
}
template <int GM>
__device__ __forceinline__ int32_t cell_of(double p, int32_t n, double max, double inv, int32_t fe) {
  const double f = cell_floor<GM>(p, n, max, inv, fe);
  if (!(f >= 0.0 && f < (double)n)) return -1;
  return (int32_t)f + 1;
}
template <int GM>
__device__ __forceinline__ int32_t vox_of(double p, int32_t n, double max, double inv, int32_t fe) {
  return cell_of<GM>(p + max, n, max, inv, fe);
}

template <int GM>
__device__ __forceinline__ double face(const double* __restrict__ f, int32_t k, int32_t ex) {
  if constexpr (GM == 2) return ldexp((double)k, ex);
  else return f[k];
}

__device__ __forceinline__ void atomic_add_nr(double* p, double v) {
  __hip_atomic_fetch_add(p, v, __ATOMIC_RELAXED, __HIP_MEMORY_SCOPE_AGENT);
}

__device__ __forceinline__ bool intersect_circle(V3 n, V3 p0, double radius, V3 l0, V3 l, double& t, double& d2) {
  t = 0.0;
  const double denom = dot(n, l);
  if (denom > 1e-6) {
    const V3 p0l0 = p0 - l0;
    double tt = dot(p0l0, n);
    tt = tt / denom;
    t = tt;
    if (tt > -1e-6) {
      const V3 p = l0 + mul(l, tt);
      const V3 v = p - p0;
      d2 = sqrt(dot(v, v));
      if (d2 <= radius) return true;
    }
  }
  return false;
}

__device__ __forceinline__ int64_t f_nint(double x) {
  if (!(fabs(x) < 4.0e18)) return x > 0 ? (int64_t)4e18 : -(int64_t)4e18;
  return (int64_t)round(x);
}
__device__ __forceinline__ int64_t f_int(double x) {
  if (!(fabs(x) < 4.0e18)) return x > 0 ? (int64_t)4e18 : -(int64_t)4e18;
  return (int64_t)x;
}

__device__ __forceinline__ uint32_t record_hits(const KParams& K, double* det_bins,
                                                const smcrt_detector* __restrict__ dets,
                                                const int64_t* __restrict__ det_off, V3 start, V3 dir,
                                                double pointSep, int32_t layer, double weight,
                                                double* totals = nullptr) {
  uint32_t hits = 0;
  double value1D = (double)layer;
  for (int32_t di = 0; di < K.n_dets; ++di) {
    const smcrt_detector* D = dets + di;
    const V3 dpos = v3(D->pos[0], D->pos[1], D->pos[2]);
    const V3 ddir = v3(D->dir[0], D->dir[1], D->dir[2]);
    double* data = det_bins ? det_bins + det_off[di] : nullptr;
    double t;
    int64_t bin = -1;
    double w = weight;
    if (D->kind == SMCRT_DET_CIRCLE || D->kind == SMCRT_DET_ANNULUS) {
      const double den = dot(ddir, dir);
      const double num = dot(dpos - start, ddir);
      if (!(den > 1e-6) || !(num > 0.0) || num > pointSep * den * (1.0 + 1e-9)) continue;
    }
    if (D->kind == SMCRT_DET_CIRCLE) {
      bool hit = intersect_circle(ddir, dpos, D->radius, start, dir, t, value1D);
      if (hit && (t <= 0.0 || t > pointSep)) hit = false;
      if (hit) {
        int64_t idx = f_nint(value1D / D->bin_wid) + 1;
        if (idx > D->nbins) idx = D->nbins;
        if (idx >= 1) bin = idx - 1;
      }
    } else if (D->kind == SMCRT_DET_ANNULUS) {
      const bool h1 = intersect_circle(ddir, dpos, D->r1, start, dir, t, value1D);
      const bool h2 = intersect_circle(ddir, dpos, D->r2, start, dir, t, value1D);
      bool hit = false;
      if (!h1 && h2) hit = !(t <= 0.0 || t > pointSep);
      value1D = value1D - D->r1;
      if (hit) {
        int64_t idx = f_nint(value1D / D->bin_wid) + 1;
        if (idx > D->nbins) idx = D->nbins;
        if (idx >= 1) bin = idx - 1;
      }
    } else if (D->kind == SMCRT_DET_CAMERA) {
      const V3 e1 = v3(D->e1[0], D->e1[1], D->e1[2]), e2 = v3(D->e2[0], D->e2[1], D->e2[2]);
      const double tt = dot(dpos - start, ddir) / dot(dir, ddir);
      if (tt >= 0.0) {
        const V3 v = (start + smul(tt, dir)) - dpos;
        const double proj1 = dot(v, e1) / D->width;
        const double proj2 = dot(v, e2) / D->height;
        if ((proj1 < D->width && proj1 > 0.0) && (proj2 < D->height && proj2 > 0.0)) {
          const double x = start.z + D->pos[0];
          const double y = start.y + D->pos[1];
          int64_t idx = f_int(x / D->bin_wid) + 1;
          int64_t idy = f_int(y / D->bin_wid_y) + 1;
          if (idx > D->nbins) idx = D->nbins;
          if (idy > D->nbins) idy = D->nbins;
          if (idx < 1) idx = D->nbins;
          if (idy < 1) idy = D->nbins;
          bin = (idx - 1) + (int64_t)D->nbins * (idy - 1);
          w = 1.0;
        }
      }
    } else if (D->kind == SMCRT_DET_FIBRE) {
      const double* F = D->fibre;
      bool hit = intersect_circle(ddir, dpos + mul(ddir, F[4]), F[2], start, dir, t, value1D);
      if (hit && (t <= 0.0 || t > pointSep)) hit = false;
      if (hit) {
        double costt = dot(ddir, dir);
        if (costt > 1.0) costt = 1.0;
        const double sintt = sqrt(1.0 - costt * costt);
        double gradient = sintt / costt;
        double radius = value1D;
        gradient = -radius / F[0] + gradient;
        radius = radius + gradient * F[6];
        if (radius > F[8]) {
          hit = false;
        } else {
          radius = radius + gradient * F[7];
          if (radius > F[3]) {
            hit = false;
          } else {
            gradient = -radius / F[1] + gradient;
            radius = radius + gradient * F[5];
            const double angle = fabs(det_atan(gradient)) * 360.0 / 6.283185307179586;
            if (angle > F[9] || radius > (F[10] / 2.0)) hit = false;
            value1D = fabs(radius);
          }
        }
      }
      if (hit) {
        int64_t idx = f_nint(value1D / D->bin_wid) + 1;
// ... 1108 lines not shown
```

### rsmcrt_amd/csrc/ws.h

```cpp
#pragma once
#include <hip/hip_runtime.h>
#include <stdint.h>

#include "lean.h"

namespace smcrt {

#ifndef SMCRT_WS_PHOTON_WAVES
#define SMCRT_WS_PHOTON_WAVES 8
#endif
#ifndef SMCRT_WS_EVENT_WAVES
#define SMCRT_WS_EVENT_WAVES 1
#endif
#ifndef SMCRT_WS_DDA
#define SMCRT_WS_DDA 2
#endif
#ifndef SMCRT_WS_WAVES
#define SMCRT_WS_WAVES 16
#endif
#ifndef SMCRT_WS_KBOUNDS_PLAIN
#define SMCRT_WS_KBOUNDS_PLAIN 0
#endif
#ifndef SMCRT_WS_START_CELLS
#define SMCRT_WS_START_CELLS 1
#endif
constexpr int WS_WAVES = SMCRT_WS_WAVES;
constexpr int WS_THREADS = 64 * WS_WAVES;
constexpr int WS_PW = SMCRT_WS_PHOTON_WAVES;
constexpr int WS_EW = SMCRT_WS_EVENT_WAVES;
static_assert(WS_PW >= 1 && WS_EW >= 1 && WS_PW + WS_EW < WS_WAVES, "a block needs all three roles");
constexpr uint32_t WS_NPL = 64u * WS_PW;
constexpr uint32_t ws_pow2(uint32_t v) { return v <= 1 ? 1 : 2 * ws_pow2((v + 1) / 2); }
constexpr uint32_t WS_EQ = ws_pow2(WS_NPL);
constexpr uint32_t WS_CONSUMED = 1u << 12;
constexpr uint32_t WS_SEQ_MASK = 0xFFFFF000u;
__device__ __forceinline__ uint32_t ws_tick(uint32_t t) { return ((t + 1u) & 0x7FFFFu) << 13; }

enum : int { SG_OX = 0, SG_OY, SG_OZ, SG_DX, SG_DY, SG_DZ, SG_LEN, SG_N };
template <uint32_t SL>
struct WsSharedT {
  static constexpr uint32_t SLOTS = SL;
  static constexpr uint32_t RING = ws_pow2(WS_NPL * SL);
  static_assert(SL >= 1 && SL <= 4, "two slot bits in a meta word");
  static_assert(RING >= WS_NPL * SL && RING < (1u << 18), "ring bound");
  double seg[SL][SG_N][WS_NPL];
  uint32_t meta[RING];
  unsigned long long pcell[WS_NPL][SL];
  uint32_t busy[WS_NPL];
  uint32_t lu[3][WS_NPL];
  uint32_t wctr[WS_WAVES][LC_N];
  double ev_dir[3][WS_NPL];
  double ev_cached[WS_NPL];
  double ev_tau[WS_NPL];
  uint32_t ev_pid[2][WS_NPL];
  uint32_t ev_draws[WS_NPL];
  uint32_t ev_code[WS_NPL];
  uint32_t evq[WS_EQ];
  uint32_t head, tail;
  uint32_t ev_head, ev_tail;
  uint32_t alive;
  uint32_t abort_;
};
constexpr uint32_t WS_EV_INTERACT = 1u, WS_EV_TAU = 2u, WS_EV_EMIT = 3u, WS_EV_FRESNEL = 4u;

enum : int { WX_ENTRY = 0, WX_START = 6, WX_SSP = 9, WX_ND = 12 };
enum : int { WXI_NEWL = 0, WXI_BOUNCES, WXI_N };
__host__ __device__ constexpr size_t ws_scratch_bytes(size_t lanes) {
  return lanes * (WX_ND * sizeof(double) + WXI_N * sizeof(uint32_t));
}

template <class S>
__device__ __forceinline__ void ws_count(S* sh, int c) {
  const uint64_t m = __ballot(1);
  if ((int)(threadIdx.x & 63) == __builtin_ctzll(m)) atomicAdd(&sh->wctr[threadIdx.x >> 6][c], (uint32_t)__popcll(m));
}

template <class S>
__device__ __forceinline__ uint32_t ws_busy(S* sh, uint32_t pl) {
  return __hip_atomic_load(&sh->busy[pl], __ATOMIC_ACQUIRE, __HIP_MEMORY_SCOPE_WORKGROUP);
}

__device__ __forceinline__ uint32_t ws_load(uint32_t* p) {
  return __hip_atomic_load(p, __ATOMIC_RELAXED, __HIP_MEMORY_SCOPE_WORKGROUP);
}


#ifdef SMCRT_ASM_MARKERS
#define WS_MARK(i) asm volatile("; @@LPHASE " #i)
#else
#define WS_MARK(i) do {} while (0)
#endif
#ifdef SMCRT_DIAG
enum : int { WD_WITERS = 20, WD_WIDLE, WD_WBUSY, WD_WPEND, WD_PTRIPS, WD_PSLEEP, WD_PBLOCKED, WD_PWAIT, WD_P7,
             WD_P7LANES, WD_PIDLE, WD_ELANES, WD_PUSH, WD_PRODWAIT, WD_EITERS, WD_ELANESRUN, WD_PEVQ,
             WD_TP_FETCH, WD_TP_POLL, WD_TP_EVAL, WD_TP_P34, WD_TP_HAND, WD_TP_P56, WD_TP_P7, WD_TP_P8,
             WD_TW_CLAIM, WD_TW_IDLE, WD_TW_WALK, WD_TW_FIN, WD_TE_RUN, WD_TE_IDLE, WD_N };
static_assert(WD_N <= 64, "g_diag[64..] belongs to transport_kernel");
#define WSDIAG(i, v) (wd[(i) - WD_WITERS] += (uint64_t)(v))
#define WST(i)                                                \
  do {                                                        \
    const uint64_t now_ = __builtin_amdgcn_s_memtime();       \
    wd[(i) - WD_WITERS] += now_ - tprev;                      \
    tprev = now_;                                             \
  } while (0)
#else
#define WSDIAG(i, v) do {} while (0)
#define WST(i) do {} while (0)
#endif

template <bool LDS_FACES, int GM, bool XF, uint32_t SL>
__global__ __launch_bounds__(WS_THREADS) __attribute__((amdgpu_waves_per_eu(4))) void ws_kernel(
    KParams K, const smcrt_sdf_node* __restrict__ nodes, const ProgOp* __restrict__ prog,
    const KCold* __restrict__ C) {
  using WsShared = WsSharedT<SL>;
  constexpr uint32_t WS_SLOTS = SL, WS_RING = WsShared::RING;
  __shared__ WsShared shm;
  WsShared* sh = &shm;
  const double eps = 1e-8;
  const int lane_id = threadIdx.x & 63;
  const int wv = threadIdx.x >> 6;

  extern __shared__ double sh_dyn[];
  const TopProps* props = K.props;
  const double* xf = K.xface;
  const double* yf = K.yface;
  const double* zf = K.zface;
  int dyn_off = 0;
  if constexpr (LDS_FACES) {
    const int np = 4 * K.n_top;
    const double* gp = (const double*)K.props;
    for (int i = threadIdx.x; i < np; i += blockDim.x) sh_dyn[i] = gp[i];
    const int nf = (K.nx + 1) + (K.ny + 1) + (K.nz + 2);
    double* sh_faces = sh_dyn + np;
    for (int i = threadIdx.x; i < nf; i += blockDim.x) sh_faces[i] = K.xface[i];
    props = (const TopProps*)sh_dyn;
    xf = sh_faces;
    yf = sh_faces + (K.nx + 1);
    zf = yf + (K.ny + 1);
    dyn_off = np + nf;
  }
  unsigned long long* const bstate = (unsigned long long*)(sh_dyn + dyn_off);
  init_buckets(K, C, bstate);
  for (int c = lane_id; c < LC_N; c += 64) sh->wctr[wv][c] = 0;
  for (uint32_t i = threadIdx.x; i < WS_NPL; i += WS_THREADS) {
    sh->busy[i] = 0;
    sh->lu[0][i] = sh->lu[1][i] = sh->lu[2][i] = 0;
  }
  for (uint32_t i = threadIdx.x; i < WS_RING; i += WS_THREADS) sh->meta[i] = 0;
  for (uint32_t i = threadIdx.x; i < WS_EQ; i += WS_THREADS) sh->evq[i] = 0;
  if (threadIdx.x == 0) {
    sh->head = sh->tail = 0;
    sh->ev_head = sh->ev_tail = 0;
    sh->alive = WS_PW;
    sh->abort_ = 0;
  }
  __syncthreads();

  uint32_t w_iters = 0, w_sdf = 0, w_dep = 0, hazards = 0;
  uint32_t r_upd = 0, r_scat = 0, r_tau = 0, r_abs = 0;
#ifdef SMCRT_DIAG
  uint64_t wd[WD_N - WD_WITERS] = {};
  uint64_t tprev = __builtin_amdgcn_s_memtime();
#endif
  if (wv < WS_PW) {
    WS_MARK(1);
    const bool test_kernel = (K.flags & SMCRT_FLAG_TEST_KERNEL) != 0;
    const bool records_on = (K.flags & SMCRT_FLAG_RECORD_PHOTONS) != 0 && C->records != nullptr;
    const uint32_t pl = threadIdx.x;
#define WLU(f) (sh->lu[(f)][pl])
    const double mf = (K.lean_debug & 3u) ? 0.0 : 2.0 * eps;
    const double mx0 = mf * (double)(K.nx + 2), my0 = mf * (double)(K.ny + 2), mz0 = mf * (double)(K.nz + 2);
    const double ex0 = 2.0 * K.xmax - mx0, ey0 = 2.0 * K.ymax - my0, ez0 = 2.0 * K.zmax - mz0;
    const bool defer_all = (K.lean_debug & 3u) == 2u;
    bool drop_event = (K.lean_debug & 4u) && blockIdx.x == 0 && pl == 0;
    uint64_t wait_t0 = 0;
    const size_t xs = (size_t)gridDim.x * WS_NPL;
    double* const X = XF ? C->lane_scratch + (size_t)blockIdx.x * WS_NPL + pl : nullptr;
    uint32_t* const XI = XF ? (uint32_t*)(C->lane_scratch + WX_ND * xs) + (size_t)blockIdx.x * WS_NPL + pl
                                         : nullptr;
    LeanPhoton P;
    P.st = ST_FETCH; P.f = LF_CELLS;
    P.pos = P.dir = v3(0.0, 0.0, 0.0);
    P.tau = P.taurun = P.d = P.minabs = 0.0;
    P.layer = P.xcell = P.ycell = P.zcell = 0;
    P.hop = P.loopc = P.seq = 0;
    P.rng.init(0);
    uint64_t chunk_base = 0;
    uint32_t chunk_left = 0;
    bool more = true;
    auto t2_entry = [&]() {
      if constexpr (XF) {
        X[(WX_ENTRY + 0) * xs] = P.pos.x; X[(WX_ENTRY + 1) * xs] = P.pos.y; X[(WX_ENTRY + 2) * xs] = P.pos.z;
        X[(WX_ENTRY + 3) * xs] = P.dir.x; X[(WX_ENTRY + 4) * xs] = P.dir.y; X[(WX_ENTRY + 5) * xs] = P.dir.z;
        X[(WX_START + 0) * xs] = P.pos.x; X[(WX_START + 1) * xs] = P.pos.y; X[(WX_START + 2) * xs] = P.pos.z;
      }
    };

    auto p8 = [&]() {
      if (!(P.f & (LF_REQ | LF_WAIT | LF_PEND)) && P.st == ST_H0) {
        if (!(P.taurun <= P.tau)) P.st = ST_T2END;
        else if (++P.hop > (uint32_t)MAX_HOP_ITERS) { P.set(LF_FAULT | LF_TFLAG); P.st = ST_T2END; }
        else P.set(LF_PEND);
      }
    };
    for (;; ++w_iters) {
      {
        uint64_t need = __ballot(P.st == ST_FETCH);
        while (need && more) {
          if (chunk_left == 0) {
            unsigned long long base = 0;
            if (lane_id == 0) base = atomicAdd(C->queue, (unsigned long long)SMCRT_FETCH_CHUNK);
            chunk_base = __shfl(base, 0, 64);
            const uint64_t n_photons = C->n_photons;
            chunk_left = (chunk_base < n_photons)
                             ? (uint32_t)((n_photons - chunk_base) < SMCRT_FETCH_CHUNK ? (n_photons - chunk_base)
                                                                                         : SMCRT_FETCH_CHUNK)
                             : 0u;
            if (chunk_left == 0) { more = false; break; }
          }
          const uint32_t n = __popcll(need);
          const uint32_t take = n < chunk_left ? n : chunk_left;
          const uint64_t rank = __popcll(need & ((1ull << lane_id) - 1ull));
          if (P.st == ST_FETCH && rank < take) {
            P.rng.init(C->first_photon + chunk_base + rank);
            sh->ev_pid[0][pl] = P.rng.pid_lo; sh->ev_pid[1][pl] = P.rng.pid_hi;
            P.st = ST_EMIT;
          }
          chunk_base += take;
          chunk_left -= take;
          need = __ballot(P.st == ST_FETCH);
        }
        if (!more && P.st == ST_FETCH) P.st = ST_IDLE;
        const uint64_t live = __ballot(P.st != ST_IDLE);
        if (live == 0) break;
      }
      WST(WD_TP_FETCH);
      if (P.has(LF_EVQ)) {
        const uint32_t code = __hip_atomic_load(&sh->ev_code[pl], __ATOMIC_ACQUIRE, __HIP_MEMORY_SCOPE_WORKGROUP);
        if (code & EV_DONE) {
          P.clr(LF_EVQ);
          P.rng.draws = sh->ev_draws[pl];
          P.rng.cached = sh->ev_cached[pl];
          if (P.st == ST_EMIT) {
            P.pos = v3(sh->seg[P.seq][SG_OX][pl], sh->seg[P.seq][SG_OY][pl], sh->seg[P.seq][SG_OZ][pl]);
            P.dir = v3(sh->ev_dir[0][pl], sh->ev_dir[1][pl], sh->ev_dir[2][pl]);
            P.clr(LF_TFLAG);
            P.layer = (int32_t)(code & 0xFFFFu);
            P.xcell = vox_of<GM>(P.pos.x, K.nx, K.xmax, K.inv2x, K.fex);
            P.ycell = vox_of<GM>(P.pos.y, K.ny, K.ymax, K.inv2y, K.fey);
            P.zcell = vox_of<GM>(P.pos.z, K.nz, K.zmax, K.inv2z, K.fez);
            P.set(LF_CELLS);
            if (code & EV_RUNAWAY) { P.set(LF_FAULT); P.st = ST_DONE; }
            else { P.st = ST_LAYER; P.set(LF_PEND); }
          } else if (XF && P.st == ST_F0) {
            if (code & EV_RUNAWAY) {
              P.set(LF_FAULT | LF_TFLAG); P.st = ST_T2END;
            } else if (code & EV_FR_REFLECT) {
              X[WX_START * xs] = P.pos.x; X[(WX_START + 1) * xs] = P.pos.y; X[(WX_START + 2) * xs] = P.pos.z;
              const uint32_t nb = XI[WXI_BOUNCES * xs] + 1u;
              XI[WXI_BOUNCES * xs] = nb;
              if (nb > 1000u) {
                ws_count(sh, LC_BABORT);
                P.pos = v3(X[WX_ENTRY * xs], X[(WX_ENTRY + 1) * xs], X[(WX_ENTRY + 2) * xs]);
                P.dir = v3(X[(WX_ENTRY + 3) * xs], X[(WX_ENTRY + 4) * xs], X[(WX_ENTRY + 5) * xs]);
                P.st = ST_INTERACT;
              } else {
                P.dir = v3(sh->ev_dir[0][pl], sh->ev_dir[1][pl], sh->ev_dir[2][pl]);
                P.st = ST_H0;
                p8();
              }
            } else {
              X[WX_SSP * xs] = sh->seg[P.seq][SG_DX][pl];
              X[(WX_SSP + 1) * xs] = sh->seg[P.seq][SG_DY][pl];
              X[(WX_SSP + 2) * xs] = sh->seg[P.seq][SG_DZ][pl];
              P.dir = v3(sh->ev_dir[0][pl], sh->ev_dir[1][pl], sh->ev_dir[2][pl]);
              P.layer = (int32_t)XI[WXI_NEWL * xs];
              P.st = ST_X1;
              P.set(LF_REQ | LF_SSP);
            }
          } else if (code & EV_ABSORB) {
            P.set(LF_TFLAG);
            P.st = ST_ABSORB;
          } else {
            if (code & EV_RUNAWAY) P.set(LF_FAULT | LF_TFLAG);
            P.dir = v3(sh->ev_dir[0][pl], sh->ev_dir[1][pl], sh->ev_dir[2][pl]);
            P.tau = sh->ev_tau[pl];
            P.taurun = 0.0;
            P.hop = 0;
            P.st = ST_H0;
            t2_entry();
            p8();
          }
        }
      }
      WSDIAG(WD_PTRIPS, 1);
      WSDIAG(WD_PIDLE, __popcll(__ballot(P.st == ST_IDLE)));
      WSDIAG(WD_PWAIT, __popcll(__ballot(P.has(LF_WAIT))));
      WSDIAG(WD_PEVQ, __popcll(__ballot(P.has(LF_EVQ))));

      WST(WD_TP_POLL);
      const bool have = (P.f & (LF_PEND | LF_REQ | LF_WAIT)) == LF_PEND;
      EvalOut R;
      R.minabs = R.minv = R.va = R.vb = 0.0; R.maxloc = 0;
      if (__ballot(have)) {
        const bool mask_le = test_kernel && P.st == ST_LAYER;
        const V3 q = (P.st == ST_H1 || P.st == ST_G0) ? P.pos + smul(P.d, P.dir) : P.pos;
        R = eval_sdfs(nodes, prog, K.n_prog, q, mask_le, 0, 0);
        const bool counted = P.st == ST_H0 || P.st == ST_H1 || P.st == ST_H3 || P.st == ST_M1 || P.st == ST_G0;
        w_sdf += __popcll(__ballot(have && counted)) * (uint32_t)K.n_top;
        WSDIAG(WD_ELANES, __popcll(__ballot(have)));
        if (have) P.clr(LF_PEND);
      }

      WST(WD_TP_EVAL);
      if (have && (P.st == ST_H0 || P.st == ST_H3 || P.st == ST_M1)) {
        const uint32_t st0 = P.st;
        P.minabs = R.minabs;
        const bool small = st0 == ST_H0 && R.minabs < eps;
        const bool out = st0 != ST_H0 && R.minv > 0.0;
        if (out) P.set(LF_TFLAG);
        if (st0 == ST_H0) P.loopc = 0;
        const bool done = P.taurun >= P.tau || P.has(LF_TFLAG);
        P.d = small ? R.minabs + 2.0 * eps : R.minabs;
        uint32_t ns = st0 == ST_M1 ? (out ? (uint32_t)ST_B0 : (uint32_t)ST_M0) : (done ? (uint32_t)ST_T2END : (uint32_t)ST_M0);
        if (small) { ns = ST_H1; P.set(LF_PEND); }
        P.st = ns;
      } else if (have) {
        switch (P.st) {
          case ST_LAYER:
            P.layer = R.maxloc;
            if (P.layer == 0) { P.set(LF_FAULT); P.st = ST_DONE; }
            else P.st = ST_T2;
            break;
          case ST_H1: {
            const double kap = props[P.layer - 1].kappa;
            const double t = P.d * kap;
            if (R.maxloc == P.layer) {
              if (P.taurun + t < P.tau) { P.set(LF_MOVE_FWD); P.taurun = P.taurun + t; }
              else { P.d = (P.tau - P.taurun) / kap; P.taurun = P.taurun + t; }
            } else {
              if (P.taurun + t < P.tau) { P.set(LF_MOVE_BACK); P.taurun = P.taurun + t; }
              else { P.d = (P.tau - P.taurun) / kap; P.set(LF_MOVE_BACK); }
            }
            P.st = ST_H2;
            P.set(LF_REQ);
            break;
          }
          case ST_G0: {
            const int32_t new_layer = R.maxloc;
            if (new_layer == P.layer && R.minabs < eps) {
              if (++P.loopc > (uint32_t)MAX_GLANCE_ITERS) { P.set(LF_FAULT | LF_TFLAG); P.st = ST_T2END; break; }
              P.d = P.d + eps;
              P.set(LF_PEND);
              break;
            }
            if (new_layer == 0) { P.set(LF_TFLAG); P.st = ST_T2END; break; }
            if (XF && props[P.layer - 1].n != props[new_layer - 1].n) {
              XI[WXI_NEWL * xs] = (uint32_t)new_layer;
              P.st = ST_F0;
              break;
            }
            P.layer = new_layer;
            P.st = ST_X1;
            P.set(LF_REQ);
            break;
          }
          default:
            break;
        }
      }

      if (!(P.f & (LF_REQ | LF_WAIT)) && P.st == ST_M0) {
        if (!(P.d >= eps)) {
          P.st = ST_B0;
        } else if (++P.loopc > (uint32_t)MAX_MARCH_ITERS) {
          P.set(LF_FAULT | LF_TFLAG); P.st = ST_B0;
        } else {
          const double kap = props[P.layer - 1].kappa;
          const double t = P.d * kap;
          if (P.taurun + t < P.tau) {
            P.taurun = P.taurun + t;
            P.st = ST_M1; P.set(LF_PEND);
          } else {
            P.d = (P.tau - P.taurun) / kap;
            P.taurun = P.tau;
            P.st = ST_B0;
          }
          P.set(LF_REQ | LF_MOVE_FWD);
        }
      }

      WST(WD_TP_P34);
      if (__ballot(P.has(LF_REQ))) {
        bool push = false, sync = false;
        V3 old = v3(0.0, 0.0, 0.0);
        const uint32_t slot = P.seq;
        if (P.has(LF_REQ) && !(ws_busy(sh, pl) & (1u << slot))) {
          ++r_upd;
          old = v3(P.pos.x + K.xmax, P.pos.y + K.ymax, P.pos.z + K.zmax);
          const int32_t ci = cell_of<GM>(old.x, K.nx, K.xmax, K.inv2x, K.fex),
                        cj = cell_of<GM>(old.y, K.ny, K.ymax, K.inv2y, K.fey),
                        ck = cell_of<GM>(old.z, K.nz, K.zmax, K.inv2z, K.fez);
          if (P.has(LF_MOVE_FWD)) P.pos = P.pos + smul(P.d, P.dir);
          else if (P.has(LF_MOVE_BACK)) P.pos = P.pos - smul(P.d, P.dir);
          P.clr(LF_REQ | LF_MOVE_FWD | LF_MOVE_BACK);
          if (ci == -1 || cj == -1 || ck == -1) {
            P.set(LF_TFLAG | LF_CELLS);
            P.xcell = ci; P.ycell = cj; P.zcell = ck;
          } else {
            const double len = P.d;
            const V3 e = v3(old.x + P.dir.x * len, old.y + P.dir.y * len, old.z + P.dir.z * len);
            constexpr bool KB = XF || SMCRT_WS_KBOUNDS_PLAIN;
            const double mx = KB ? K.lean_lo[0] : mx0, my = KB ? K.lean_lo[1] : my0, mz = KB ? K.lean_lo[2] : mz0;
            const double ex = KB ? K.lean_hi[0] : ex0, ey = KB ? K.lean_hi[1] : ey0, ez = KB ? K.lean_hi[2] : ez0;
            const bool inside = old.x >= mx && old.x <= ex && old.y >= my && old.y <= ey && old.z >= mz &&
                                old.z <= ez && e.x >= mx && e.x <= ex && e.y >= my && e.y <= ey && e.z >= mz &&
                                e.z <= ez;
            push = true;
            sync = !inside && !defer_all;
#if SMCRT_WS_START_CELLS
            sh->pcell[pl][slot] = lean_pack(ci, cj, ck);
#endif
            if constexpr (GM != 2) {
              const bool in_cell = face<GM>(xf, ci - 1, K.fex) <= old.x && old.x <= face<GM>(xf, ci, K.fex) &&
                                   face<GM>(yf, cj - 1, K.fey) <= old.y && old.y <= face<GM>(yf, cj, K.fey) &&
                                   face<GM>(zf, ck - 1, K.fez) <= old.z && old.z <= face<GM>(zf, ck, K.fez);
              if (!in_cell) sync = true;
            }
          }
        }
        const uint64_t pm = __ballot(push);
        WSDIAG(WD_PUSH, __popcll(pm));
        WSDIAG(WD_PBLOCKED, __popcll(__ballot(P.has(LF_REQ))));
        if (pm) {
          const int first = __builtin_ctzll(pm);
          uint32_t base = 0;
          if (lane_id == first) base = atomicAdd(&sh->tail, (uint32_t)__popcll(pm));
          base = __builtin_amdgcn_readlane(base, first);
          if (push) {
            const uint32_t rank = __builtin_amdgcn_mbcnt_hi((uint32_t)(pm >> 32), __builtin_amdgcn_mbcnt_lo((uint32_t)pm, 0u));
            const uint32_t t = base + rank;
            const uint32_t ix = t & (WS_RING - 1);
            double* const sg = &sh->seg[slot][0][pl];
            sg[SG_OX * WS_NPL] = old.x; sg[SG_OY * WS_NPL] = old.y; sg[SG_OZ * WS_NPL] = old.z;
            sg[SG_DX * WS_NPL] = P.dir.x; sg[SG_DY * WS_NPL] = P.dir.y; sg[SG_DZ * WS_NPL] = P.dir.z;
            sg[SG_LEN * WS_NPL] = P.d;
            atomicOr(&sh->busy[pl], 1u << slot);
            const uint32_t prev = t < WS_RING ? 0u : (ws_tick(t - WS_RING) | WS_CONSUMED);
            uint64_t t0 = 0;
            while (__hip_atomic_load(&sh->meta[ix], __ATOMIC_RELAXED, __HIP_MEMORY_SCOPE_WORKGROUP) != prev) {
              WSDIAG(WD_PRODWAIT, 1);
              __builtin_amdgcn_s_sleep(1);
              if (!t0) t0 = __builtin_amdgcn_s_memrealtime();
              else if (watchdog_expired(C, t0, WDOG_RING)) break;
            }
            __hip_atomic_store(&sh->meta[ix], pl | (slot << 9) | (sync ? (1u << 11) : 0u) | ws_tick(t),
                               __ATOMIC_RELEASE, __HIP_MEMORY_SCOPE_WORKGROUP);
            P.seq = P.seq + 1 == WS_SLOTS ? 0u : P.seq + 1;
            P.clr(LF_CELLS);
            if (sync) P.set(LF_WAIT);
          }
        }
      }

      WST(WD_TP_HAND);
      if (P.has(LF_WAIT) && !(ws_busy(sh, pl) & (1u << ((P.seq + WS_SLOTS - 1) % WS_SLOTS)))) {
        const unsigned long long w = sh->pcell[pl][(P.seq + WS_SLOTS - 1) % WS_SLOTS];
        P.xcell = lean_cell(w, 0); P.ycell = lean_cell(w, 1); P.zcell = lean_cell(w, 2);
        P.set(LF_CELLS);
        if (w & LEAN_TFLAG) P.set(LF_TFLAG);
        if (w & LEAN_FAULT) P.set(LF_FAULT);
        P.clr(LF_WAIT);
      }
      const bool free_ = !(P.f & (LF_REQ | LF_WAIT));
      if (free_ && (P.st == ST_H2 || P.st == ST_B0 || P.st == ST_X1)) {
        if (P.st == ST_X1) {
          P.taurun = P.taurun + P.d * props[P.layer - 1].kappa;
          if (XF && P.has(LF_SSP)) P.pos = v3(X[WX_SSP * xs], X[(WX_SSP + 1) * xs], X[(WX_SSP + 2) * xs]);
          else P.pos = P.pos + smul(P.d, P.dir);
          P.clr(LF_SSP);
        }
        if (XF && K.n_dets) {
          const V3 st = v3(X[WX_START * xs], X[(WX_START + 1) * xs], X[(WX_START + 2) * xs]);
          const double sep = pointsep(P.pos, st);
          X[WX_START * xs] = P.pos.x; X[(WX_START + 1) * xs] = P.pos.y; X[(WX_START + 2) * xs] = P.pos.z;
          const uint32_t hits = record_hits(K, C->det_bins, K.dets, K.det_off, st, P.dir, sep, P.layer, 1.0);
          if (hits) atomicAdd(&sh->wctr[wv][LC_HITS], hits);
        }
        if (P.st == ST_H2) {
          P.st = ST_H3; P.set(LF_PEND);
        } else if (P.st == ST_X1) {
          P.st = P.has(LF_TFLAG) ? ST_T2END : ST_H0;
        } else if (P.taurun >= P.tau || P.has(LF_TFLAG)) {
          P.st = ST_T2END;
        } else {
          P.d = P.minabs + 2.0 * eps;
          P.loopc = 0;
          P.st = ST_G0; P.set(LF_PEND);
        }
      }

      if (free_ && P.st == ST_T2END) {
        if (fabs(P.pos.x) > K.xmax) P.set(LF_TFLAG);
        if (fabs(P.pos.y) > K.ymax) P.set(LF_TFLAG);
        if (fabs(P.pos.z) > K.zmax) P.set(LF_TFLAG);
        P.st = ST_INTERACT;
      }
      if (!P.has(LF_CELLS) && (P.st == ST_ABSORB || (records_on && P.st == ST_DONE)) && ws_busy(sh, pl) == 0) {
        const unsigned long long w = sh->pcell[pl][(P.seq + WS_SLOTS - 1) % WS_SLOTS];
        P.xcell = lean_cell(w, 0); P.ycell = lean_cell(w, 1); P.zcell = lean_cell(w, 2);
        P.set(LF_CELLS);
      }
      if (P.st == ST_ABSORB && P.has(LF_CELLS)) {
        if (P.xcell < 1 || P.xcell > K.nx || P.ycell < 1 || P.ycell > K.ny || P.zcell < 1 || P.zcell > K.nz)
          P.set(LF_FAULT);
        else if (C->absorb) atomic_add_nr(C->absorb + lin(K, P.xcell, P.ycell, P.zcell), 1.0);
        P.st = ST_DONE;
      }

      WST(WD_TP_P56);
      {
        bool qev = free_ && !P.has(LF_EVQ) &&
                   ((!test_kernel && ((P.st == ST_INTERACT && !(P.f & (LF_TFLAG | LF_FAULT)) &&
                                     WLU(LL_INTER) + 1u <= (uint32_t)MAX_INTERACTIONS) ||
                                    P.st == ST_T2 || (P.st == ST_EMIT && !(ws_busy(sh, pl) & (1u << P.seq))))) ||
                    (XF && P.st == ST_F0 && !(ws_busy(sh, pl) & (1u << P.seq))));
        if (drop_event && qev) {
          drop_event = qev = false;
          __hip_atomic_store(&sh->ev_code[pl], 0u, __ATOMIC_RELAXED, __HIP_MEMORY_SCOPE_WORKGROUP);
          P.set(LF_EVQ);
        }
        const uint64_t qm = __ballot(qev);
        if (qm) {
          const int first = __builtin_ctzll(qm);
          uint32_t base = 0;
          if (lane_id == first) base = atomicAdd(&sh->ev_tail, (uint32_t)__popcll(qm));
          base = __builtin_amdgcn_readlane(base, first);
          if (qev) {
            const uint32_t t = base + __builtin_amdgcn_mbcnt_hi((uint32_t)(qm >> 32), __builtin_amdgcn_mbcnt_lo((uint32_t)qm, 0u));
            const uint32_t ix = t & (WS_EQ - 1);
            const uint32_t prev = t < WS_EQ ? 0u : (ws_tick(t - WS_EQ) | WS_CONSUMED);
            uint64_t t0 = 0;
            while (__hip_atomic_load(&sh->evq[ix], __ATOMIC_ACQUIRE, __HIP_MEMORY_SCOPE_WORKGROUP) != prev) {
              __builtin_amdgcn_s_sleep(1);
              if (!t0) t0 = __builtin_amdgcn_s_memrealtime();
              else if (watchdog_expired(C, t0, WDOG_EVENT_QUEUE)) break;
            }
            sh->ev_dir[0][pl] = P.dir.x; sh->ev_dir[1][pl] = P.dir.y; sh->ev_dir[2][pl] = P.dir.z;
            sh->ev_cached[pl] = P.rng.cached;
            sh->ev_draws[pl] = P.rng.draws;
            if (XF && P.st == ST_F0) {
              sh->seg[P.seq][SG_OX][pl] = P.pos.x; sh->seg[P.seq][SG_OY][pl] = P.pos.y;
              sh->seg[P.seq][SG_OZ][pl] = P.pos.z; sh->seg[P.seq][SG_LEN][pl] = P.d;
              sh->ev_tau[pl] = (double)XI[WXI_NEWL * xs];
            }
            if (P.st == ST_EMIT) {
              P.clr(LF_FAULT); P.layer = 0;
              WLU(LL_STATUS) = 0; WLU(LL_NSCATT) = 0; WLU(LL_INTER) = 0;
              if constexpr (XF) XI[WXI_BOUNCES * xs] = 0;
            }
            sh->ev_code[pl] = (uint32_t)P.layer |
                              ((P.st == ST_INTERACT ? WS_EV_INTERACT
                                : (P.st == ST_T2 ? WS_EV_TAU : (P.st == ST_EMIT ? WS_EV_EMIT : WS_EV_FRESNEL))) << 16) |
                              (P.seq << 19);
            __hip_atomic_store(&sh->evq[ix], pl | ws_tick(t), __ATOMIC_RELEASE, __HIP_MEMORY_SCOPE_WORKGROUP);
            P.set(LF_EVQ);
          }
        }
      }
      {
        const bool ev = free_ && !P.has(LF_EVQ) &&
                        (P.st == ST_INTERACT || P.st == ST_T2 || P.st == ST_EMIT || P.st == ST_DONE);
        const uint64_t evm = __ballot(ev);
        const uint64_t busy = __ballot(P.st != ST_IDLE && P.st != ST_FETCH && !P.has(LF_EVQ));
        const uint32_t nev = __popcll(evm);
        const uint32_t batch = test_kernel ? (uint32_t)SMCRT_LEAN_EVENT_LANES : 4u;
        const bool run_ev = nev && (nev >= batch || evm == busy);
        WSDIAG(WD_P7, run_ev ? 1 : 0);
        WSDIAG(WD_P7LANES, run_ev ? nev : 0);
        if (run_ev) {
          if (ev && P.st == ST_INTERACT) {
            if (P.f & (LF_TFLAG | LF_FAULT)) {
              P.st = ST_DONE;
            } else if (WLU(LL_INTER) + 1u > (uint32_t)MAX_INTERACTIONS) {
              ++WLU(LL_INTER);
              P.set(LF_FAULT); P.st = ST_DONE;
            } else {
              const double ran = P.rng.next(K.key0, K.key1);
              const TopProps pr = props[P.layer - 1];
              const bool sc = ran < pr.albedo;
              ++WLU(LL_INTER);
              if (!sc) {
                P.set(LF_TFLAG); WLU(LL_STATUS) = 1; ++r_abs;
                P.st = test_kernel ? ST_DONE : ST_ABSORB;
              } else {
                Lane L;
                L.dir = P.dir; L.rng = P.rng; L.fault = false; L.tflag = false;
                scatter(K, L, pr.hgg);
                P.dir = L.dir; P.rng = L.rng;
                if (L.fault) P.set(LF_FAULT | LF_TFLAG);
                const uint32_t st = ++WLU(LL_NSCATT);
                ++r_scat;
                if (test_kernel) {
                  if (st >= 1 && st <= 4) {
                    double* const moments = C->moments;
                    if (moments) {
                      double* m = moments + 3 * (st - 1);
                      double* m2 = moments + 12 + 3 * (st - 1);
                      atomic_add_nr(m + 0, P.pos.x); atomic_add_nr(m + 1, P.pos.y); atomic_add_nr(m + 2, P.pos.z);
                      atomic_add_nr(m2 + 0, P.pos.x * P.pos.x);
                      atomic_add_nr(m2 + 1, P.pos.y * P.pos.y);
                      atomic_add_nr(m2 + 2, P.pos.z * P.pos.z);
                    }
                  } else if (K.flags & SMCRT_FLAG_END_EARLY) {
                    P.set(LF_TFLAG);
                    WLU(LL_STATUS) = 4;
                  }
                }
                P.st = ST_T2;
              }
            }
          }
          if (ev && P.st == ST_T2) {
            ++r_tau;
            t2_entry();
            P.tau = -det_log(P.rng.next(K.key0, K.key1));
            P.taurun = 0.0;
            P.hop = 0;
            P.st = ST_H0;
          }
          if (ev && P.st == ST_EMIT) {
            P.clr(LF_FAULT); P.layer = 0;
            WLU(LL_STATUS) = 0; WLU(LL_NSCATT) = 0; WLU(LL_INTER) = 0;
            if constexpr (XF) XI[WXI_BOUNCES * xs] = 0;
            Lane L;
            L.rng = P.rng; L.xcell = L.ycell = L.zcell = 0; L.layer = 0; L.tflag = false;
            emit<GM, false>(K, C, L, 0u);
            if (!test_kernel) {
              int64_t tries = 0;
              while (cell_out(K, L)) {
                if (++tries > MAX_EMIT_TRIES) { P.set(LF_FAULT); break; }
                ws_count(sh, LC_RETRIES);
                emit<GM, false>(K, C, L, 0u);
              }
            }
            P.pos = L.pos; P.dir = L.dir; P.rng = L.rng; P.clr(LF_TFLAG);
            P.layer = L.layer;
            P.xcell = L.xcell; P.ycell = L.ycell; P.zcell = L.zcell;
            P.set(LF_CELLS);
            if (!test_kernel && !P.has(LF_FAULT) && (K.flags & SMCRT_FLAG_RENDER_SOURCE) && C->emission)
              atomic_add_nr(C->emission + lin(K, P.xcell, P.ycell, P.zcell), 1.0);
            if (P.has(LF_FAULT)) P.st = ST_DONE;
            else { P.st = ST_LAYER; P.set(LF_PEND); }
          }
          if (ev && P.st == ST_DONE && (P.has(LF_CELLS) || !records_on)) {
            if (P.has(LF_FAULT)) { WLU(LL_STATUS) = 3; ws_count(sh, LC_FAULTS); }
            else if (WLU(LL_STATUS) == 0) { WLU(LL_STATUS) = 2; ws_count(sh, LC_ESCAPED); }
            ws_count(sh, LC_PHOTONS);
            atomicAdd(&sh->wctr[wv][LC_DRAWS], P.rng.draws);
#ifdef SMCRT_DIAG
            if (C->done_time)
              C->done_time[(((uint64_t)P.rng.pid_hi << 32) | P.rng.pid_lo) - C->done_base] = __builtin_amdgcn_s_memrealtime();
#endif
            if (records_on) {
              const uint64_t pid = ((uint64_t)P.rng.pid_hi << 32) | P.rng.pid_lo;
              smcrt_photon_record* r = C->records + (pid - C->first_photon);
              r->pos[0] = P.pos.x; r->pos[1] = P.pos.y; r->pos[2] = P.pos.z;
              r->dir[0] = P.dir.x; r->dir[1] = P.dir.y; r->dir[2] = P.dir.z;
              r->weight = 1.0;
              r->cell[0] = P.xcell; r->cell[1] = P.ycell; r->cell[2] = P.zcell;
              r->layer = P.layer;
              r->nscatt = WLU(LL_NSCATT);
              r->bounces = XF ? XI[WXI_BOUNCES * xs] : 0u;
              r->draws = P.rng.draws;
              r->status = WLU(LL_STATUS);
            }
            P.clr(LF_TFLAG | LF_FAULT);
            P.st = ST_FETCH;
          }
        }
      }

      WST(WD_TP_P7);
      p8();
      if (__ballot(P.st != ST_IDLE && !(P.has(LF_WAIT) || P.has(LF_REQ) || P.has(LF_EVQ) ||
                                        (P.st == ST_ABSORB && !P.has(LF_CELLS)))) == 0) {
        WSDIAG(WD_PSLEEP, 1);
        __builtin_amdgcn_s_sleep(1);
        if (!wait_t0) {
          wait_t0 = __builtin_amdgcn_s_memrealtime();
        } else if (ws_load(&sh->abort_) || watchdog_expired(C, wait_t0, WDOG_PHOTON_WAVE)) {
          if (lane_id == 0) __hip_atomic_store(&sh->abort_, 1u, __ATOMIC_RELAXED, __HIP_MEMORY_SCOPE_WORKGROUP);
          break;
        }
      } else {
        wait_t0 = 0;
      }
      WST(WD_TP_P8);
    }
#undef WLU
    if (lane_id == 0) atomicSub(&sh->alive, 1u);
  } else if (wv < WS_PW + WS_EW) {
    WS_MARK(2);
    __builtin_amdgcn_s_setprio(3);
    bool pend = false;
    uint32_t tk = 0;
    for (;; ++w_iters) {
      const uint64_t cm = __ballot(!pend);
      if (cm) {
        const int first = __builtin_ctzll(cm);
        uint32_t base = 0;
        if (lane_id == first) base = atomicAdd(&sh->ev_head, (uint32_t)__popcll(cm));
        base = __builtin_amdgcn_readlane(base, first);
        if (!pend) {
          tk = base + __builtin_amdgcn_mbcnt_hi((uint32_t)(cm >> 32), __builtin_amdgcn_mbcnt_lo((uint32_t)cm, 0u));
          pend = true;
        }
      }
      bool run = false;
      uint32_t o = 0;
      if (pend) {
        const uint32_t ix = tk & (WS_EQ - 1);
        const uint32_t m = __hip_atomic_load(&sh->evq[ix], __ATOMIC_ACQUIRE, __HIP_MEMORY_SCOPE_WORKGROUP);
        if ((m & WS_SEQ_MASK) == ws_tick(tk)) {
          o = m & 511u;
          __hip_atomic_store(&sh->evq[ix], ws_tick(tk) | WS_CONSUMED, __ATOMIC_RELEASE, __HIP_MEMORY_SCOPE_WORKGROUP);
          run = true;
          pend = false;
        }
      }
      if (!__ballot(run)) {
        if (ws_load(&sh->abort_)) break;
        if (ws_load(&sh->alive) == 0) {
          const uint32_t T = ws_load(&sh->ev_tail);
          if (pend && (int32_t)(tk - T) >= 0) pend = false;
          if (!__ballot(pend) && (int32_t)(ws_load(&sh->ev_head) - T) >= 0) break;
        }
        __builtin_amdgcn_s_sleep(2);
        WST(WD_TE_IDLE);
        continue;
      }
      WSDIAG(WD_EITERS, 1);
      WSDIAG(WD_ELANESRUN, __popcll(__ballot(run)));
      if (run) {
        Rng rg;
        rg.pid_lo = sh->ev_pid[0][o]; rg.pid_hi = sh->ev_pid[1][o];
        rg.draws = sh->ev_draws[o]; rg.cached = sh->ev_cached[o];
        const uint32_t code = sh->ev_code[o];
        const int32_t layer = (int32_t)(code & 0xFFFFu);
        uint32_t res = 0;
        const uint32_t kind = (code >> 16) & 7u;
        bool tau_entry = kind == WS_EV_TAU;
        if (kind == WS_EV_EMIT) {
          Lane L;
          L.rng = rg; L.xcell = L.ycell = L.zcell = 0; L.layer = 0; L.tflag = false;
          emit<GM, false>(K, C, L, 0u);
          int64_t tries = 0;
          bool fault = false;
          while (cell_out(K, L)) {
            if (++tries > MAX_EMIT_TRIES) { fault = true; break; }
            ws_count(sh, LC_RETRIES);
            emit<GM, false>(K, C, L, 0u);
          }
          rg = L.rng;
          const uint32_t es = (code >> 19) & 3u;
          sh->seg[es][SG_OX][o] = L.pos.x; sh->seg[es][SG_OY][o] = L.pos.y; sh->seg[es][SG_OZ][o] = L.pos.z;
          sh->ev_dir[0][o] = L.dir.x; sh->ev_dir[1][o] = L.dir.y; sh->ev_dir[2][o] = L.dir.z;
          if (!fault && (K.flags & SMCRT_FLAG_RENDER_SOURCE) && C->emission)
            atomic_add_nr(C->emission + lin(K, L.xcell, L.ycell, L.zcell), 1.0);
          res = (fault ? EV_RUNAWAY : 0u) | ((uint32_t)L.layer & 0xFFFFu);
        } else if (XF && kind == WS_EV_FRESNEL) {
          const uint32_t es = (code >> 19) & 3u;
          const V3 pos = v3(sh->seg[es][SG_OX][o], sh->seg[es][SG_OY][o], sh->seg[es][SG_OZ][o]);
          const V3 dir0 = v3(sh->ev_dir[0][o], sh->ev_dir[1][o], sh->ev_dir[2][o]);
          const int32_t new_layer = (int32_t)sh->ev_tau[o];
          const V3 ssp = pos + smul(sh->seg[es][SG_LEN][o], dir0);
          const EvalOut R0 = eval_sdfs(nodes, prog, K.n_prog, pos, false, new_layer, layer);
          const EvalOut R1 = eval_sdfs(nodes, prog, K.n_prog, ssp, false, new_layer, layer);
          const double ds_new = R0.va, ds_old = R0.vb, dn_new = R1.va, dn_old = R1.vb;
          int32_t ls = 0;
          if (dn_new < 0.0 && ds_new >= 0.0) ls = new_layer;
          else if (dn_old >= 0.0 && ds_old < 0.0) ls = layer;
          else if (dn_new < 0.0 && dn_old < 0.0) ls = new_layer;
          else if (ds_old >= 0.0 && dn_old >= 0.0) ls = layer;
          if (ls == 0) {
            res = EV_RUNAWAY;
          } else {
            const double t = 1e-6;
            const double e1 = eval_sdfs(nodes, prog, K.n_prog, pos + mul(v3(1.0, -1.0, -1.0), t), false, ls, 0).va;
            const double e2 = eval_sdfs(nodes, prog, K.n_prog, pos + mul(v3(-1.0, -1.0, 1.0), t), false, ls, 0).va;
            const double e3 = eval_sdfs(nodes, prog, K.n_prog, pos + mul(v3(-1.0, 1.0, -1.0), t), false, ls, 0).va;
            const double e4 = eval_sdfs(nodes, prog, K.n_prog, pos + mul(v3(1.0, 1.0, 1.0), t), false, ls, 0).va;
            const V3 xyy = v3(1.0, -1.0, -1.0), yyx = v3(-1.0, -1.0, 1.0), yxy = v3(-1.0, 1.0, -1.0),
                     xxx = v3(1.0, 1.0, 1.0);
            const V3 nn = ((mul(xyy, e1) + mul(yyx, e2)) + mul(yxy, e3)) + mul(xxx, e4);
            const double ln = len(nn);
            const V3 N = v3(nn.x / ln, nn.y / ln, nn.z / ln);
            const double n1 = props[layer - 1].n, n2 = props[new_layer - 1].n;
            ws_count(sh, LC_FRES);
            const double Rf = fresnel(dir0, N, n1, n2);
            V3 dn;
            if (rg.next(K.key0, K.key1) <= Rf) {
              const double s2 = 2.0 * dot(N, dir0);
              dn = dir0 - smul(s2, N);
              ws_count(sh, LC_REFL);
              res = EV_FR_REFLECT;
            } else {
              sh->seg[es][SG_DX][o] = ssp.x; sh->seg[es][SG_DY][o] = ssp.y; sh->seg[es][SG_DZ][o] = ssp.z;
              const double eta = n1 / n2;
              V3 Nt = N;
              double c1 = dot(Nt, dir0);
              if (c1 < 0.0) c1 = -c1;
              else Nt = smul(-1.0, N);
              const double c2 = sqrt(1.0 - (eta * eta) * (1.0 - c1 * c1));
              dn = smul(eta, dir0) + smul(eta * c1 - c2, Nt);
            }
            sh->ev_dir[0][o] = dn.x; sh->ev_dir[1][o] = dn.y; sh->ev_dir[2][o] = dn.z;
          }
        } else if (kind == WS_EV_INTERACT) {
          const TopProps pr = props[layer - 1];
          const double ran = rg.next(K.key0, K.key1);
          ++sh->lu[LL_INTER][o];
          if (!(ran < pr.albedo)) {
            sh->lu[LL_STATUS][o] = 1;
            ++r_abs;
            res = EV_ABSORB;
          } else {
            Lane L;
            L.dir = v3(sh->ev_dir[0][o], sh->ev_dir[1][o], sh->ev_dir[2][o]);
            L.rng = rg; L.fault = false; L.tflag = false;
            scatter(K, L, pr.hgg);
            rg = L.rng;
            if (L.fault) res = EV_RUNAWAY;
            ++sh->lu[LL_NSCATT][o];
            ++r_scat;
            sh->ev_dir[0][o] = L.dir.x; sh->ev_dir[1][o] = L.dir.y; sh->ev_dir[2][o] = L.dir.z;
            tau_entry = true;
          }
        }
        if (tau_entry) {
          ++r_tau;
          sh->ev_tau[o] = -det_log(rg.next(K.key0, K.key1));
        }
        sh->ev_draws[o] = rg.draws;
        sh->ev_cached[o] = rg.cached;
        __hip_atomic_store(&sh->ev_code[o], res | EV_DONE, __ATOMIC_RELEASE, __HIP_MEMORY_SCOPE_WORKGROUP);
      }
      WST(WD_TE_RUN);
    }
  } else {
    WS_MARK(10);
    WalkSeg W;
    W.old = v3(0.0, 0.0, 0.0);
    W.sd = W.slen = 0.0;
    W.xcell = W.ycell = W.zcell = 0;
    W.dda_it = 0;
    W.seg = W.tflag = W.fault = false;
    V3 wdir = v3(0.0, 0.0, 0.0);
    V3 wrcp = v3(0.0, 0.0, 0.0);
    uint32_t wmeta = 0;
    BucketLog WB;
    WB.next = WB.end = 0;
    uint32_t overflow = 0;
    bool pend = false;
    uint32_t tk = 0;
    for (;; ++w_iters) {
      WS_MARK(11);
      const uint64_t cm = __ballot(!W.seg && !pend);
      if (cm) {
        const int first = __builtin_ctzll(cm);
        uint32_t base = 0;
        if (lane_id == first) base = atomicAdd(&sh->head, (uint32_t)__popcll(cm));
        base = __builtin_amdgcn_readlane(base, first);
        if (!W.seg && !pend) {
          tk = base + __builtin_amdgcn_mbcnt_hi((uint32_t)(cm >> 32), __builtin_amdgcn_mbcnt_lo((uint32_t)cm, 0u));
          pend = true;
        }
      }
      if (pend) {
        const uint32_t ix = tk & (WS_RING - 1);
        const uint32_t m = __hip_atomic_load(&sh->meta[ix], __ATOMIC_ACQUIRE, __HIP_MEMORY_SCOPE_WORKGROUP);
        if ((m & WS_SEQ_MASK) == ws_tick(tk)) {
          __hip_atomic_store(&sh->meta[ix], ws_tick(tk) | WS_CONSUMED, __ATOMIC_RELAXED, __HIP_MEMORY_SCOPE_WORKGROUP);
          const double* const sg = &sh->seg[(m >> 9) & 3u][0][m & 511u];
          const V3 o = v3(sg[SG_OX * WS_NPL], sg[SG_OY * WS_NPL], sg[SG_OZ * WS_NPL]);
          const V3 dd = v3(sg[SG_DX * WS_NPL], sg[SG_DY * WS_NPL], sg[SG_DZ * WS_NPL]);
          const double l = sg[SG_LEN * WS_NPL];
          W.old = o;
          wdir = dd;
          wrcp = v3(ieee_rcp_f64(dd.x), ieee_rcp_f64(dd.y), ieee_rcp_f64(dd.z));
          W.slen = l;
          wmeta = m;
#if SMCRT_WS_START_CELLS
          {
            const unsigned long long cw = sh->pcell[m & 511u][(m >> 9) & 3u];
            W.xcell = lean_cell(cw, 0); W.ycell = lean_cell(cw, 1); W.zcell = lean_cell(cw, 2);
          }
#else
          W.xcell = cell_of<GM>(W.old.x, K.nx, K.xmax, K.inv2x, K.fex);
          W.ycell = cell_of<GM>(W.old.y, K.ny, K.ymax, K.inv2y, K.fey);
          W.zcell = cell_of<GM>(W.old.z, K.nz, K.zmax, K.inv2z, K.fez);
#endif
          W.sd = 0.0; W.dda_it = 0;
          W.seg = true; W.tflag = false; W.fault = false;
          pend = false;
        }
      }
      const uint64_t am = __ballot(W.seg);
      WSDIAG(WD_WITERS, 1);
      WSDIAG(WD_WIDLE, am ? 0 : 1);
      WSDIAG(WD_WBUSY, __popcll(am));
      WSDIAG(WD_WPEND, __popcll(__ballot(pend)));
      WST(WD_TW_CLAIM);
      if (!am) {
        if (ws_load(&sh->abort_)) break;
        if (ws_load(&sh->alive) == 0) {
          const uint32_t T = ws_load(&sh->tail);
          if (pend && (int32_t)(tk - T) >= 0) pend = false;
          if (!__ballot(pend) && (int32_t)(ws_load(&sh->head) - T) >= 0) break;
        }
        __builtin_amdgcn_s_sleep(2);
        WST(WD_TW_IDLE);
        continue;
      }
      WS_MARK(12);
#pragma unroll
      for (int k = 0; k < SMCRT_WS_DDA; ++k) {
        if (k > 0 && !__ballot(W.seg)) break;
        bool dep = false;
        uint32_t vox = 0;
        double val = 0.0;
        if (W.seg) dda_step_r<GM>(K, W, wdir, wrcp, xf, yf, zf, dep, vox, val, 1.0);
        w_dep += __popcll(__ballot(dep));
        WS_MARK(13);
        emit_bucketed(K, C, WB, dep, vox, val, overflow, bstate);
      }
      WS_MARK(14);
      WST(WD_TW_WALK);
      if ((am >> lane_id & 1ull) && !W.seg) {
        const uint32_t owner = wmeta & 511u, slot = (wmeta >> 9) & 3u;
        const bool sync = (wmeta & (1u << 11)) != 0;
        if (!sync && (W.tflag || W.fault)) ++hazards;
        sh->pcell[owner][slot] = lean_pack(W.xcell, W.ycell, W.zcell) | (W.tflag ? LEAN_TFLAG : 0ull) |
                                 (W.fault ? LEAN_FAULT : 0ull);
        __hip_atomic_fetch_and(&sh->busy[owner], ~(1u << slot), __ATOMIC_RELEASE, __HIP_MEMORY_SCOPE_WORKGROUP);
      }
      WST(WD_TW_FIN);
    }
    WS_MARK(15);
    close_buckets(K, C, WB, w_dep - overflow, overflow);
  }
  WS_MARK(16);
  {
    unsigned long long* const counters = C->counters;
    const uint32_t hz = wave_sum_u32(hazards);
    const uint32_t n_upd = wave_sum_u32(r_upd), n_scat = wave_sum_u32(r_scat), n_tau = wave_sum_u32(r_tau),
                   n_abs = wave_sum_u32(r_abs);
    if (lane_id == 0) {
      if (hz) {
        atomicAdd(C->dep_ctl + 5, hz);
        atomicAdd(C->lean_hazards, (unsigned long long)hz);
      }
      if (C->dep_ctl && n_upd) atomicAdd(C->dep_ctl + 6, n_upd);
      if (counters) {
        const uint32_t* c = sh->wctr[wv];
        const uint32_t v[SMCRT_NCOUNTERS] = {c[LC_PHOTONS], c[LC_RETRIES], n_scat,        n_abs,          w_sdf,
                                             w_dep,         n_upd,         n_tau,          c[LC_FRES],     c[LC_REFL],
                                             c[LC_BABORT],  c[LC_FAULTS] + hz, c[LC_DRAWS], c[LC_HITS],   c[LC_ESCAPED],
                                             w_iters};
        for (int i = 0; i < SMCRT_NCOUNTERS; ++i)
          if (v[i]) atomicAdd(counters + i, (unsigned long long)v[i]);
      }
      double* const nscatt = C->nscatt;
      if (nscatt && n_scat) atomic_add_nr(nscatt, (double)n_scat);
    }
  }
#ifdef SMCRT_DIAG
  if (lane_id == 0)
    for (int i = 0; i < WD_N - WD_WITERS; ++i)
      if (wd[i]) atomicAdd(&::g_diag[WD_WITERS + i], (unsigned long long)wd[i]);
#endif
  __syncthreads();
  close_block_buckets(K, C, bstate);
}

}
```

### rsmcrt_amd/engine.py

```python
from __future__ import annotations

import ctypes as C
import os
import threading

import numpy as np

from . import abi
from .scene import detector_array
from .tallies import Result

LIB_PATH = os.environ.get("SMCRT_LIB") or os.path.join(os.path.dirname(os.path.abspath(__file__)), "libsmcrt.so")
_lock = threading.Lock()
_lib = None


class SmcrtError(RuntimeError):
    pass


def load_library(path: str = LIB_PATH):
    global _lib
    with _lock:
        if _lib is not None:
# ... 67 lines not shown
        return L


def _check(st: int):
    if st != abi.OK:
        msg = load_library().smcrt_last_error().decode(errors="replace")
        raise SmcrtError(f"{abi.STATUS_NAMES.get(st, st)}: {msg}")


def device_count() -> int:
    n = C.c_int32()
    _check(load_library().smcrt_device_count(C.byref(n)))
    return n.value


class Engine:

    def __init__(self, scene, grid, dets=(), device: int = 0):
        L = load_library()
        self.scene, self.grid, self.dets, self.device = scene, grid, list(dets), device
        self._nodes = scene.node_array()
        self._top = scene.top_array()
        self._darr = detector_array(self.dets)
        h = C.c_void_p()
        _check(L.smcrt_scene_create(self._nodes, len(scene.nodes), self._top, scene.n_top, C.byref(grid),
                                    self._darr, len(self.dets), device, C.byref(h)))
        self._h = h

    def close(self):
        if getattr(self, "_h", None):
            load_library().smcrt_scene_destroy(self._h)
            self._h = None

    def __del__(self):
        try:
            self.close()
        except Exception:
            pass

    def __enter__(self):
        return self

    def __exit__(self, *exc):
        self.close()

    def set_spectral(self, top_index: int, sp, mode: int = abi.SPECTRAL_UPDATE) -> float:
        from .spectral import _lib
        d = C.c_uint64(sp.draw)
        out = abi.OptProps()
        _check(_lib().smcrt_scene_set_spectral(self._h, top_index, C.byref(sp.struct()), int(mode), sp.seed,
                                               C.byref(d), C.byref(out)))
        sp.draw, sp.props = d.value, out
        return out.wavelength

    def set_optprops(self, top_index: int, mus, mua, hgg, n):
        _check(load_library().smcrt_scene_set_optprops(self._h, top_index, mus, mua, hgg, n))

    @staticmethod
    def config(n_photons, seed=123456789, flags=abi.FLAG_PATHLENGTH, first_photon=0) -> abi.RunConfig:
        cfg = abi.RunConfig()
        cfg.n_photons, cfg.first_photon, cfg.seed, cfg.flags = int(n_photons), int(first_photon), int(seed), int(flags)
        return cfg

    def run(self, source, n_photons, seed=123456789, flags=abi.FLAG_PATHLENGTH, first_photon=0,
            records=False, result: Result | None = None) -> Result:
        res = result if result is not None else Result(self.grid, self.dets, n_photons, records)
        res.n_photons += int(n_photons)
        cfg = self.config(n_photons, seed, flags | (abi.FLAG_RECORD_PHOTONS if records else 0), first_photon)
        t = res.tallies()
        _check(load_library().smcrt_run(self._h, C.byref(source), C.byref(cfg), C.byref(t)))
        return res

    def run_origins(self, origins, n_photons, source=None, seed=123456789, flags=abi.FLAG_PATHLENGTH,
                    first_photon=0, result: Result | None = None):
        org = np.ascontiguousarray(origins, dtype=np.float64).reshape(-1, 3)
        k = len(org)
        res = result if result is not None else Result(self.grid, self.dets, 0)
        res.n_photons += int(n_photons) * k
        tot = np.zeros((k, max(1, len(self.dets))))
        cfg = self.config(n_photons, seed, flags, first_photon)
        t = res.tallies()
        _check(load_library().smcrt_run_origins(self._h, C.byref(source) if source is not None else None,
                                                org.ctypes.data_as(C.POINTER(C.c_double)), k, C.byref(cfg),
                                                tot.ctypes.data_as(C.POINTER(C.c_double)), C.byref(t)))
        return tot[:, :len(self.dets)], res

    def classify(self, points):
        pts = np.ascontiguousarray(points, dtype=np.float64).reshape(-1, 3)
        lay = np.zeros(len(pts), dtype=np.int32)
        kap = np.zeros(len(pts))
        _check(load_library().smcrt_scene_classify(self._h, pts.ctypes.data_as(C.POINTER(C.c_double)), len(pts),
                                                   lay.ctypes.data_as(C.POINTER(C.c_int32)),
                                                   kap.ctypes.data_as(C.POINTER(C.c_double))))
        return lay, kap

    def escape(self, cfg: abi.EscapeConfig, n_photons, source=None, seed=123456789, flags=abi.FLAG_PATHLENGTH,
               result: Result | None = None):
        from .escape import sym_dims
        n0, n1, n2 = sym_dims(cfg)
        nd = len(self.dets)
        es = np.zeros((n2, n1, n0, max(nd, 1)), dtype=np.float32)
        e = np.zeros((self.grid.nz, self.grid.ny, self.grid.nx, max(nd, 1)), dtype=np.float32)
        res = result if result is not None else Result(self.grid, self.dets, 0)
        rc = self.config(n_photons, seed, flags, 0)
        t = res.tallies()
        _check(load_library().smcrt_escape_run(self._h, C.byref(source) if source is not None else None, C.byref(cfg),
                                               C.byref(rc), es.ctypes.data_as(C.POINTER(C.c_float)),
                                               e.ctypes.data_as(C.POINTER(C.c_float)), C.byref(t)))
        return es.transpose(3, 2, 1, 0)[:nd], e.transpose(3, 2, 1, 0)[:nd], res

    def get_optprops(self, top_index: int):
        lay = C.c_int32()
        v = [C.c_double() for _ in range(4)]
        _check(load_library().smcrt_scene_get_optprops(self._h, top_index, C.byref(lay), *[C.byref(x) for x in v]))
        return (lay.value, *[x.value for x in v])

    def inverse(self, source, cfg: abi.InverseConfig, n_photons, targets, seed=123456789,
                flags=abi.FLAG_PATHLENGTH, result: Result | None = None):
        m = cfg.max_steps
        out = np.zeros((5, m))
        tg = np.ascontiguousarray(targets, dtype=np.float64)
        rc = self.config(n_photons, seed, flags, 0)
        t = result.tallies() if result is not None else None
        _check(load_library().smcrt_inverse_run(self._h, C.byref(source), C.byref(cfg), C.byref(rc),
                                                tg.ctypes.data_as(C.POINTER(C.c_double)),
                                                out.ctypes.data_as(C.POINTER(C.c_double)),
                                                C.byref(t) if t is not None else None))
        return out.T.copy()

    def run_device(self, source, cfg: abi.RunConfig, dev: abi.DeviceTallies, stream: int = 0):
        _check(load_library().smcrt_run_device(self._h, C.byref(source), C.byref(cfg), C.byref(dev),
                                               C.c_void_p(stream)))

    def reduce_device_tallies(self, comm: "Comm", dev: abi.DeviceTallies, root: int = -1, stream: int = 0):
        _check(load_library().smcrt_reduce_device_tallies(self._h, comm._h, C.byref(dev), int(root),
                                                          C.c_void_p(stream)))

    def fence(self, stream: int = 0):
        _check(load_library().smcrt_scene_fence(self._h, C.c_void_p(stream)))

    def check(self):
        _check(load_library().smcrt_scene_check(self._h))

    def set_timing(self, enable: bool = True):
        _check(load_library().smcrt_scene_set_timing(self._h, 1 if enable else 0))

    def kernel_times(self) -> dict:
        t = abi.KernelTimes()
        _check(load_library().smcrt_scene_kernel_times(self._h, C.byref(t)))
        return {"transport_ms": t.transport_ms, "deposit_ms": t.deposit_ms, "launches": t.launches,
                "lean_launches": t.lean_launches, "far_steps": t.far_steps,
                "fold_cu_ms": t.fold_cu_ms, "lean_hazards": t.lean_hazards}


def pack_layout(grid, n_det_bins: int, fields: int) -> abi.PackLayout:
    lay = abi.PackLayout()
    lay.n_voxels, lay.n_det_bins, lay.fields = grid.nx * grid.ny * grid.nz, int(n_det_bins), int(fields)
    return lay


def pack_result(res: Result, fields: int) -> np.ndarray:
    L = load_library()
    lay = pack_layout(res.grid, sum(res.det_sizes), fields)
    n = C.c_int64()
    _check(L.smcrt_pack_size(C.byref(lay), C.byref(n)))
    buf = np.zeros(n.value)
    t = res.tallies()
    _check(L.smcrt_pack_host(C.byref(lay), C.byref(t), buf.ctypes.data_as(C.POINTER(C.c_double))))
    return buf


def unpack_into(res: Result, buf: np.ndarray, fields: int) -> Result:
    L = load_library()
    lay = pack_layout(res.grid, sum(res.det_sizes), fields)
    b = np.ascontiguousarray(buf, dtype=np.float64)
    t = res.tallies()
    _check(L.smcrt_unpack_host(C.byref(lay), b.ctypes.data_as(C.POINTER(C.c_double)), C.byref(t)))
    return res


class Comm:

    @staticmethod
    def unique_id() -> bytes:
        buf = (C.c_uint8 * abi.UNIQUE_ID_BYTES)()
        _check(load_library().smcrt_comm_unique_id(buf))
        return bytes(buf)

    def __init__(self, uid: bytes, n_ranks: int, rank: int, device: int):
        buf = (C.c_uint8 * abi.UNIQUE_ID_BYTES).from_buffer_copy(uid)
        h = C.c_void_p()
        _check(load_library().smcrt_comm_init_rank(buf, int(n_ranks), int(rank), int(device), C.byref(h)))
        self._h = h

    def info(self) -> dict:
        n, r, d = C.c_int32(), C.c_int32(), C.c_int32()
        _check(load_library().smcrt_comm_info(self._h, C.byref(n), C.byref(r), C.byref(d)))
        return {"n_ranks": n.value, "rank": r.value, "device": d.value}

    @property
    def n_ranks(self) -> int:
        return self.info()["n_ranks"]

    def close(self):
        if getattr(self, "_h", None):
            load_library().smcrt_comm_destroy(self._h)
            self._h = None

    def __del__(self):
        try:
            self.close()
        except Exception:
            pass


class MultiEngine:

    def __init__(self, scene, grid, dets=(), devices=None):
        L = load_library()
        self.scene, self.grid, self.dets = scene, grid, list(dets)
        self._nodes = scene.node_array()
        self._top = scene.top_array()
        self._darr = detector_array(self.dets)
        devs = None if devices is None else (C.c_int32 * len(devices))(*devices)
        h = C.c_void_p()
        _check(L.smcrt_multi_create(self._nodes, len(scene.nodes), self._top, scene.n_top, C.byref(grid),
                                    self._darr, len(self.dets), devs, len(devices) if devices else 0, C.byref(h)))
        self._h = h
        n = C.c_int32()
        _check(L.smcrt_multi_info(h, C.byref(n)))
        self.n_devices = n.value
        self._pending = 0

    def close(self):
        if getattr(self, "_h", None):
            load_library().smcrt_multi_destroy(self._h)
            self._h = None

    def __del__(self):
        try:
            self.close()
        except Exception:
            pass

    def __enter__(self):
        return self

    def __exit__(self, *exc):
        self.close()

    def run(self, source, n_photons, seed=123456789, flags=abi.FLAG_PATHLENGTH, first_photon=0,
            result: Result | None = None) -> Result:
        res = result if result is not None else Result(self.grid, self.dets, n_photons)
        res.n_photons += int(n_photons) + self._pending
        self._pending = 0
        cfg = Engine.config(n_photons, seed, flags, first_photon)
        t = res.tallies()
        _check(load_library().smcrt_multi_run(self._h, C.byref(source), C.byref(cfg), C.byref(t)))
        return res

    def accumulate(self, source, n_photons, seed=123456789, flags=abi.FLAG_PATHLENGTH, first_photon=0):
        cfg = Engine.config(n_photons, seed, flags, first_photon)
        try:
            _check(load_library().smcrt_multi_accumulate(self._h, C.byref(source), C.byref(cfg)))
        except SmcrtError:
            self._pending = 0
            raise
        self._pending += int(n_photons)

    def device_photons(self):
        out = (C.c_uint64 * self.n_devices)()
        _check(load_library().smcrt_multi_device_photons(self._h, out))
        return list(out)

    def collect(self, result: Result | None = None) -> Result:
        res = result if result is not None else Result(self.grid, self.dets, 0)
        held = sum(self.device_photons())
        if held != self._pending:
            raise SmcrtError(f"multi-device photon count mismatch: the devices hold {held} photons, "
                             f"{self._pending} were accumulated since the last collect")
        res.n_photons += held
        self._pending = 0
        t = res.tallies()
        _check(load_library().smcrt_multi_collect(self._h, C.byref(t)))
        return res
```

Before: 262.3 million.

## Add in-voxel fast path accumulating path length locally in work-stealing kernel

Adds a per-lane fast path to the lean work-stealing kernel. When a path-length segment provably stays inside the current voxel, its length is added to a lane-local accumulator instead of going through the shared deposit slot and event machinery. The accumulator is flushed with an atomic add when the voxel changes or the photon finishes. This targets deposit queue traffic and slot-busy stalls. In exchange it adds a conservative geometry test with an epsilon margin, rounds each segment length to float before summing, and doubles the kernel instantiations. It is enabled by default for the non-Fresnel kernels.

New measurement: 272.7 million (median of 6 runs). +3.9%, better.

```diff
diff --git a/include/smcrt.h b/include/smcrt.h
--- a/include/smcrt.h
+++ b/include/smcrt.h
@@ -300,6 +300,8 @@
 int smcrt_scene_set_timing(smcrt_scene* scene, int32_t enable);
 int smcrt_scene_kernel_times(smcrt_scene* scene, smcrt_kernel_times* out);
 
+int smcrt_scene_invoxel_segments(smcrt_scene* scene, int64_t* out);
+
 int smcrt_normalise_fluence(float* grid, const smcrt_grid* g, uint64_t nphotons);
 
 typedef enum smcrt_symmetry {
diff --git a/rsmcrt_amd/abi.py b/rsmcrt_amd/abi.py
--- a/rsmcrt_amd/abi.py
+++ b/rsmcrt_amd/abi.py
@@ -213,4 +213,5 @@
     "smcrt_multi_scene", "smcrt_multi_run", "smcrt_multi_accumulate", "smcrt_multi_collect",
     "smcrt_multi_device_photons", "smcrt_multi_destroy", "smcrt_job_run_devices",
     "smcrt_spectral_sample", "smcrt_scene_set_spectral", "smcrt_scene_check",
+    "smcrt_scene_invoxel_segments",
 ]
diff --git a/rsmcrt_amd/csrc/invoxel.h b/rsmcrt_amd/csrc/invoxel.h
--- /dev/null
+++ b/rsmcrt_amd/csrc/invoxel.h
@@ -0,0 +1,26 @@
+#pragma once
+
+#if defined(__HIPCC__) || defined(__CUDACC__)
+#define SMCRT_INVOXEL_HD __host__ __device__ inline
+#else
+#define SMCRT_INVOXEL_HD inline
+#endif
+
+namespace smcrt {
+
+SMCRT_INVOXEL_HD bool invoxel_axis(double f, double o, double dir, double len) {
+  if (dir == 0.0) return true;
+  const double ad = dir < 0.0 ? -dir : dir;
+  const double n = f - o;
+  const double sn = dir < 0.0 ? -n : n;
+  const double rhs = (len * ad) * (1.0 + 0x1.0p-41);
+  return ad >= 0x1.0p-500 && sn > rhs;
+}
+
+SMCRT_INVOXEL_HD bool invoxel_segment(double ox, double oy, double oz, double dx, double dy, double dz, double len,
+                                      double fx, double fy, double fz) {
+  if (!(len >= 0x1.0p-400 && len < 100000.0)) return false;
+  return invoxel_axis(fx, ox, dx, len) && invoxel_axis(fy, oy, dy, len) && invoxel_axis(fz, oz, dz, len);
+}
+
+}
diff --git a/rsmcrt_amd/csrc/kernel_ptrs.h b/rsmcrt_amd/csrc/kernel_ptrs.h
--- a/rsmcrt_amd/csrc/kernel_ptrs.h
+++ b/rsmcrt_amd/csrc/kernel_ptrs.h
@@ -34,8 +34,8 @@
     default: return kinst_transport_1_2(x, c);
   }
 }
-inline const void* ws_kernel_ptr(bool lds_faces, int gm, bool xf, int slots) {
-  const int x = xf ? 1 : 0;
+inline const void* ws_kernel_ptr(bool lds_faces, int gm, bool xf, int slots, bool iv) {
+  const int x = xf ? (iv ? 2 : 1) : 0;
   switch ((lds_faces ? 3 : 0) + gm) {
     case 0: return kinst_ws_0_0(x, slots);
     case 1: return kinst_ws_0_1(x, slots);
diff --git a/rsmcrt_amd/csrc/kinst.hip b/rsmcrt_amd/csrc/kinst.hip
--- a/rsmcrt_amd/csrc/kinst.hip
+++ b/rsmcrt_amd/csrc/kinst.hip
@@ -12,7 +12,8 @@
 
 #if KI_P == 1
 const void* KI_NAME(kinst_wsp)(int slots) {
-  return slots == 3 ? (const void*)ws_kernel<KI_F != 0, KI_G, false, 3> : (const void*)ws_kernel<KI_F != 0, KI_G, false, 2>;
+  return slots == 3 ? (const void*)ws_kernel<KI_F != 0, KI_G, false, 3, true>
+                    : (const void*)ws_kernel<KI_F != 0, KI_G, false, 2, true>;
 }
 #define KI_DIAG_NAME KI_NAME(kinst_diagp)
 #else
@@ -35,7 +36,12 @@
 #endif
 
 const void* KI_NAME(kinst_ws)(int xf, int slots) {
-  if (xf) return slots == 3 ? (const void*)ws_kernel<KI_F != 0, KI_G, true, 3> : (const void*)ws_kernel<KI_F != 0, KI_G, true, 2>;
+  if (xf == 2)
+    return slots == 3 ? (const void*)ws_kernel<KI_F != 0, KI_G, true, 3, true>
+                      : (const void*)ws_kernel<KI_F != 0, KI_G, true, 2, true>;
+  if (xf)
+    return slots == 3 ? (const void*)ws_kernel<KI_F != 0, KI_G, true, 3, false>
+                      : (const void*)ws_kernel<KI_F != 0, KI_G, true, 2, false>;
   return KI_NAME(kinst_wsp)(slots);
 }
 #define KI_DIAG_NAME KI_NAME(kinst_diag)
diff --git a/rsmcrt_amd/csrc/sceneplan.cpp b/rsmcrt_amd/csrc/sceneplan.cpp
--- a/rsmcrt_amd/csrc/sceneplan.cpp
+++ b/rsmcrt_amd/csrc/sceneplan.cpp
@@ -41,6 +41,8 @@
   k.fused_hist = !is(std::getenv("SMCRT_FUSED_HIST"), "0");
   const char* wsl = std::getenv("SMCRT_WS_SLOTS");
   k.ws_two_slots = wsl && wsl[0] == '2';
+  const char* wi = std::getenv("SMCRT_WS_INVOXEL");
+  k.ws_invoxel = wi ? (is(wi, "0") ? 0 : 1) : -1;
   const char* le = std::getenv("SMCRT_LEAN");
   k.lean_mode = le ? (is(le, "0") ? 0 : 1) : -1;
   const char* lm = std::getenv("SMCRT_DEBUG_LEAN_MARGIN");
@@ -285,6 +287,7 @@
     p.lean_mode = knobs.lean_mode;
     p.lean_candidate = ok && !p.nested && (p.lean_mode == 1 || (p.lean_mode != 0 && n_dets == 0));
     p.lean_debug = knobs.lean_debug;
+    p.ws_invoxel = knobs.ws_invoxel;
   }
   p.fold_prio = knobs.fold_prio;
   p.cull_log = knobs.cull_log;
diff --git a/rsmcrt_amd/csrc/sceneplan.h b/rsmcrt_amd/csrc/sceneplan.h
--- a/rsmcrt_amd/csrc/sceneplan.h
+++ b/rsmcrt_amd/csrc/sceneplan.h
@@ -24,6 +24,7 @@
   Q_FOLD_TICKS,
   Q_LEAN_HAZARDS,
   Q_WATCHDOG,
+  Q_INVOXEL,
   Q_COUNT
 };
 constexpr int N_QUEUES = Q_CALLER + 1;
@@ -48,6 +49,7 @@
   bool fold_prio = true;
   bool fused_hist = true;
   bool ws_two_slots = false;
+  int ws_invoxel = -1;
   int lean_mode = -1;
   uint32_t lean_debug = 0;
   bool verbose = false;
@@ -104,6 +106,7 @@
   int ws_slots = 3;
   int lean_mode = -1;
   uint32_t lean_debug = 0;
+  int ws_invoxel = -1;
   bool lean_candidate = false;
   bool fold_prio = true, cull_log = false, verbose = false;
 };
@@ -145,6 +148,7 @@
 inline bool launch_lean(bool lean_ok, bool xsrc, uint32_t bucket_tiles, uint32_t flags) {
   return !xsrc && lean_ok && bucket_tiles && (flags & SMCRT_FLAG_PATHLENGTH) && !(flags & SMCRT_FLAG_SURVIVAL_BIAS);
 }
+inline bool ws_invoxel_on(int knob, bool xf) { return knob < 0 ? !xf : knob != 0; }
 inline void lean_margins(uint32_t lean_debug, const smcrt_grid& g, double lo[3], double hi[3]) {
   const double eps = 1e-8, mf = (lean_debug & 3u) ? 0.0 : 2.0 * eps;
   const double mx = mf * (double)(g.nx + 2), my = mf * (double)(g.ny + 2), mz = mf * (double)(g.nz + 2);
diff --git a/rsmcrt_amd/csrc/smcrt.hip b/rsmcrt_amd/csrc/smcrt.hip
--- a/rsmcrt_amd/csrc/smcrt.hip
+++ b/rsmcrt_amd/csrc/smcrt.hip
@@ -301,7 +301,8 @@
   const bool xf = s->fresnel || s->n_dets > 0;
   if (s->lean_ok) {
     hipError_t oe = hipOccupancyMaxActiveBlocksPerMultiprocessor(
-        &per_cu, ws_kernel_ptr(s->lds_faces, s->grid_mode, xf, s->ws_slots), kinst_ws_threads(), lean_lds(*s));
+        &per_cu, ws_kernel_ptr(s->lds_faces, s->grid_mode, xf, s->ws_slots, ws_invoxel_on(s->ws_invoxel, xf)),
+        kinst_ws_threads(), lean_lds(*s));
     if (oe != hipSuccess || per_cu < 1) per_cu = 1;
     s->grid_blocks_ws = cus * per_cu;
     if (xf) {
@@ -538,8 +539,9 @@
   if (lean) {
     ++s->lean_launches;
     void* args[] = {(void*)&K, (void*)&a_nodes, (void*)&a_prog, (void*)&C};
-    HIPCHK(hipLaunchKernel(ws_kernel_ptr(s->lds_faces, s->grid_mode, s->d_lscratch != nullptr, s->ws_slots), dim3(blocks),
-                           dim3(kinst_ws_threads()), args, lean_lds(*s), stream));
+    const bool xf = s->d_lscratch != nullptr;
+    HIPCHK(hipLaunchKernel(ws_kernel_ptr(s->lds_faces, s->grid_mode, xf, s->ws_slots, ws_invoxel_on(s->ws_invoxel, xf)),
+                           dim3(blocks), dim3(kinst_ws_threads()), args, lean_lds(*s), stream));
   } else {
     const smcrt_detector* a_dets = K.dets;
     const int64_t* a_off = K.det_off;
@@ -708,6 +710,7 @@
   Ch.queue = nullptr;
   Ch.far_steps = s->d_queue + Q_FAR_STEPS;
   Ch.lean_hazards = s->d_queue + Q_LEAN_HAZARDS;
+  Ch.invoxel_segs = s->d_queue + Q_INVOXEL;
   Ch.lane_scratch = nullptr;
   Ch.watchdog = watchdog_word(s);
 #ifdef SMCRT_DIAG
@@ -726,6 +729,7 @@
   K.rec_pool = nullptr; K.n_chunks = 0; K.hist_tiles = 0; K.bucket_tiles = 0; K.n_buckets = 0;
   K.claim_delay = knobs.claim_delay;
   K.lean_debug = s->lean_debug | (knobs.drop_event ? 4u : 0u);
+  K.ws_invoxel = ws_invoxel_on(s->ws_invoxel, s->d_lscratch != nullptr) ? 1u : 0u;
   lean_margins(K.lean_debug, s->grid, K.lean_lo, K.lean_hi);
   return SMCRT_OK;
 }
@@ -1083,6 +1087,16 @@
   return SMCRT_OK;
 }
 
+int smcrt_scene_invoxel_segments(smcrt_scene* s, int64_t* out) {
+  if (!s || !out) return fail(SMCRT_ERR_INVALID_ARG, "NULL argument");
+  std::lock_guard<std::mutex> g(s->mu);
+  HIPCHK(hipSetDevice(s->device));
+  unsigned long long n = 0;
+  HIPCHK(hipMemcpy(&n, s->d_queue + Q_INVOXEL, sizeof(n), hipMemcpyDeviceToHost));
+  *out = (int64_t)n;
+  return SMCRT_OK;
+}
+
 int smcrt_normalise_fluence(float* g, const smcrt_grid* grid, uint64_t nphotons) {
   if (!g || !grid || nphotons == 0) return fail(SMCRT_ERR_INVALID_ARG, "bad arguments");
   const double xmax = grid->xmax, ymax = grid->ymax, zmax = grid->zmax;
diff --git a/rsmcrt_amd/csrc/transport.h b/rsmcrt_amd/csrc/transport.h
--- a/rsmcrt_amd/csrc/transport.h
+++ b/rsmcrt_amd/csrc/transport.h
@@ -46,6 +46,7 @@
   uint32_t* tile_nb;
   unsigned long long* far_steps;
   unsigned long long* lean_hazards;
+  unsigned long long* invoxel_segs;
   double* lane_scratch;
   uint32_t* watchdog;
   uint64_t watchdog_ticks;
@@ -92,6 +93,7 @@
   uint32_t bucket_tiles, n_buckets;
   uint32_t claim_delay;
   uint32_t lean_debug;
+  uint32_t ws_invoxel;
   double lean_lo[3], lean_hi[3];
   const CullGrid* __restrict__ cull;
   const double* __restrict__ ctab;
diff --git a/rsmcrt_amd/csrc/ws.h b/rsmcrt_amd/csrc/ws.h
--- a/rsmcrt_amd/csrc/ws.h
+++ b/rsmcrt_amd/csrc/ws.h
@@ -2,6 +2,7 @@
 #include <hip/hip_runtime.h>
 #include <stdint.h>
 
+#include "invoxel.h"
 #include "lean.h"
 
 namespace smcrt {
@@ -24,6 +25,10 @@
 #ifndef SMCRT_WS_START_CELLS
 #define SMCRT_WS_START_CELLS 1
 #endif
+#ifndef SMCRT_WS_INVOXEL_LDS
+#define SMCRT_WS_INVOXEL_LDS 0
+#endif
+constexpr uint32_t WS_NO_VOX = 0xFFFFFFFFu;
 constexpr int WS_WAVES = SMCRT_WS_WAVES;
 constexpr int WS_THREADS = 64 * WS_WAVES;
 constexpr int WS_PW = SMCRT_WS_PHOTON_WAVES;
@@ -49,6 +54,10 @@
   uint32_t busy[WS_NPL];
   uint32_t lu[3][WS_NPL];
   uint32_t wctr[WS_WAVES][LC_N];
+#if SMCRT_WS_INVOXEL_LDS
+  double iv_acc[WS_NPL];
+  uint32_t iv_vox[WS_NPL];
+#endif
   double ev_dir[3][WS_NPL];
   double ev_cached[WS_NPL];
   double ev_tau[WS_NPL];
@@ -108,7 +117,7 @@
 #define WST(i) do {} while (0)
 #endif
 
-template <bool LDS_FACES, int GM, bool XF, uint32_t SL>
+template <bool LDS_FACES, int GM, bool XF, uint32_t SL, bool IV>
 __global__ __launch_bounds__(WS_THREADS) __attribute__((amdgpu_waves_per_eu(4))) void ws_kernel(
     KParams K, const smcrt_sdf_node* __restrict__ nodes, const ProgOp* __restrict__ prog,
     const KCold* __restrict__ C) {
@@ -145,6 +154,10 @@
   for (uint32_t i = threadIdx.x; i < WS_NPL; i += WS_THREADS) {
     sh->busy[i] = 0;
     sh->lu[0][i] = sh->lu[1][i] = sh->lu[2][i] = 0;
+#if SMCRT_WS_INVOXEL_LDS
+    sh->iv_acc[i] = 0.0;
+    sh->iv_vox[i] = WS_NO_VOX;
+#endif
   }
   for (uint32_t i = threadIdx.x; i < WS_RING; i += WS_THREADS) sh->meta[i] = 0;
   for (uint32_t i = threadIdx.x; i < WS_EQ; i += WS_THREADS) sh->evq[i] = 0;
@@ -157,7 +170,7 @@
   __syncthreads();
 
   uint32_t w_iters = 0, w_sdf = 0, w_dep = 0, hazards = 0;
-  uint32_t r_upd = 0, r_scat = 0, r_tau = 0, r_abs = 0;
+  uint32_t r_upd = 0, r_scat = 0, r_tau = 0, r_abs = 0, r_inv = 0;
 #ifdef SMCRT_DIAG
   uint64_t wd[WD_N - WD_WITERS] = {};
   uint64_t tprev = __builtin_amdgcn_s_memtime();
@@ -173,6 +186,24 @@
     const double ex0 = 2.0 * K.xmax - mx0, ey0 = 2.0 * K.ymax - my0, ez0 = 2.0 * K.zmax - mz0;
     const bool defer_all = (K.lean_debug & 3u) == 2u;
     bool drop_event = (K.lean_debug & 4u) && blockIdx.x == 0 && pl == 0;
+    const bool invoxel_on = IV && K.ws_invoxel != 0 && (K.flags & SMCRT_FLAG_PATHLENGTH) != 0;
+#if SMCRT_WS_INVOXEL_LDS
+#define WS_IV_ACC (sh->iv_acc[pl])
+#define WS_IV_VOX (sh->iv_vox[pl])
+#else
+    double iv_acc = 0.0;
+    uint32_t iv_vox = WS_NO_VOX;
+#define WS_IV_ACC iv_acc
+#define WS_IV_VOX iv_vox
+#endif
+    auto iv_flush = [&]() {
+      const uint32_t av = WS_IV_VOX;
+      if (av != WS_NO_VOX) {
+        atomic_add_nr(C->jmean + av, WS_IV_ACC);
+        WS_IV_ACC = 0.0;
+        WS_IV_VOX = WS_NO_VOX;
+      }
+    };
     uint64_t wait_t0 = 0;
     const size_t xs = (size_t)gridDim.x * WS_NPL;
     double* const X = XF ? C->lane_scratch + (size_t)blockIdx.x * WS_NPL + pl : nullptr;
@@ -395,12 +426,43 @@
         bool push = false, sync = false;
         V3 old = v3(0.0, 0.0, 0.0);
         const uint32_t slot = P.seq;
-        if (P.has(LF_REQ) && !(ws_busy(sh, pl) & (1u << slot))) {
+        bool inv = false;
+        int32_t ci = -1, cj = -1, ck = -1;
+        if constexpr (IV) {
+          if (P.has(LF_REQ)) {
+            old = v3(P.pos.x + K.xmax, P.pos.y + K.ymax, P.pos.z + K.zmax);
+            ci = cell_of<GM>(old.x, K.nx, K.xmax, K.inv2x, K.fex);
+            cj = cell_of<GM>(old.y, K.ny, K.ymax, K.inv2y, K.fey);
+            ck = cell_of<GM>(old.z, K.nz, K.zmax, K.inv2z, K.fez);
+            if (invoxel_on && ci != -1 && cj != -1 && ck != -1)
+              inv = invoxel_segment(old.x, old.y, old.z, P.dir.x, P.dir.y, P.dir.z, P.d,
+                                    face<GM>(xf, P.dir.x > 0.0 ? ci : ci - 1, K.fex),
+                                    face<GM>(yf, P.dir.y > 0.0 ? cj : cj - 1, K.fey),
+                                    face<GM>(zf, P.dir.z > 0.0 ? ck : ck - 1, K.fez));
+          }
+        }
+        if (inv) {
           ++r_upd;
-          old = v3(P.pos.x + K.xmax, P.pos.y + K.ymax, P.pos.z + K.zmax);
-          const int32_t ci = cell_of<GM>(old.x, K.nx, K.xmax, K.inv2x, K.fex),
-                        cj = cell_of<GM>(old.y, K.ny, K.ymax, K.inv2y, K.fey),
-                        ck = cell_of<GM>(old.z, K.nz, K.zmax, K.inv2z, K.fez);
+          ++r_inv;
+          const uint32_t vox = lin(K, ci, cj, ck);
+          if (WS_IV_VOX != vox) {
+            iv_flush();
+            WS_IV_VOX = vox;
+          }
+          WS_IV_ACC = WS_IV_ACC + (double)(float)P.d;
+          if (P.has(LF_MOVE_FWD)) P.pos = P.pos + smul(P.d, P.dir);
+          else if (P.has(LF_MOVE_BACK)) P.pos = P.pos - smul(P.d, P.dir);
+          P.clr(LF_REQ | LF_MOVE_FWD | LF_MOVE_BACK);
+          P.xcell = ci; P.ycell = cj; P.zcell = ck;
+          P.set(LF_CELLS);
+        } else if (P.has(LF_REQ) && !(ws_busy(sh, pl) & (1u << slot))) {
+          ++r_upd;
+          if constexpr (!IV) {
+            old = v3(P.pos.x + K.xmax, P.pos.y + K.ymax, P.pos.z + K.zmax);
+            ci = cell_of<GM>(old.x, K.nx, K.xmax, K.inv2x, K.fex);
+            cj = cell_of<GM>(old.y, K.ny, K.ymax, K.inv2y, K.fey);
+            ck = cell_of<GM>(old.z, K.nz, K.zmax, K.inv2z, K.fez);
+          }
           if (P.has(LF_MOVE_FWD)) P.pos = P.pos + smul(P.d, P.dir);
           else if (P.has(LF_MOVE_BACK)) P.pos = P.pos - smul(P.d, P.dir);
           P.clr(LF_REQ | LF_MOVE_FWD | LF_MOVE_BACK);
@@ -658,6 +720,7 @@
             else if (WLU(LL_STATUS) == 0) { WLU(LL_STATUS) = 2; ws_count(sh, LC_ESCAPED); }
             ws_count(sh, LC_PHOTONS);
             atomicAdd(&sh->wctr[wv][LC_DRAWS], P.rng.draws);
+            iv_flush();
 #ifdef SMCRT_DIAG
             if (C->done_time)
               C->done_time[(((uint64_t)P.rng.pid_hi << 32) | P.rng.pid_lo) - C->done_base] = __builtin_amdgcn_s_memrealtime();
@@ -698,6 +761,9 @@
       }
       WST(WD_TP_P8);
     }
+    iv_flush();
+#undef WS_IV_ACC
+#undef WS_IV_VOX
 #undef WLU
     if (lane_id == 0) atomicSub(&sh->alive, 1u);
   } else if (wv < WS_PW + WS_EW) {
@@ -955,17 +1021,18 @@
     unsigned long long* const counters = C->counters;
     const uint32_t hz = wave_sum_u32(hazards);
     const uint32_t n_upd = wave_sum_u32(r_upd), n_scat = wave_sum_u32(r_scat), n_tau = wave_sum_u32(r_tau),
-                   n_abs = wave_sum_u32(r_abs);
+                   n_abs = wave_sum_u32(r_abs), n_inv = wave_sum_u32(r_inv);
     if (lane_id == 0) {
       if (hz) {
         atomicAdd(C->dep_ctl + 5, hz);
         atomicAdd(C->lean_hazards, (unsigned long long)hz);
       }
       if (C->dep_ctl && n_upd) atomicAdd(C->dep_ctl + 6, n_upd);
+      if (n_inv) atomicAdd(C->invoxel_segs, (unsigned long long)n_inv);
       if (counters) {
         const uint32_t* c = sh->wctr[wv];
         const uint32_t v[SMCRT_NCOUNTERS] = {c[LC_PHOTONS], c[LC_RETRIES], n_scat,        n_abs,          w_sdf,
-                                             w_dep,         n_upd,         n_tau,          c[LC_FRES],     c[LC_REFL],
+                                             w_dep + n_inv, n_upd,         n_tau,          c[LC_FRES],     c[LC_REFL],
                                              c[LC_BABORT],  c[LC_FAULTS] + hz, c[LC_DRAWS], c[LC_HITS],   c[LC_ESCAPED],
                                              w_iters};
         for (int i = 0; i < SMCRT_NCOUNTERS; ++i)
diff --git a/rsmcrt_amd/engine.py b/rsmcrt_amd/engine.py
--- a/rsmcrt_amd/engine.py
+++ b/rsmcrt_amd/engine.py
@@ -243,6 +243,13 @@
                 "lean_launches": t.lean_launches, "far_steps": t.far_steps,
                 "fold_cu_ms": t.fold_cu_ms, "lean_hazards": t.lean_hazards}
 
+    def invoxel_segments(self) -> int:
+        fn = load_library().smcrt_scene_invoxel_segments
+        fn.argtypes = [C.c_void_p, C.POINTER(C.c_int64)]
+        n = C.c_int64()
+        _check(fn(self._h, C.byref(n)))
+        return n.value
+
 
 def pack_layout(grid, n_det_bins: int, fields: int) -> abi.PackLayout:
     lay = abi.PackLayout()
```
